# jneem/nnnoiseless

Hardware: AMD Instinct MI355X
Metric: 480-sample frames/sec (whole node) at N concurrent streams (higher is better)
Workload: dtype f32; 1 GPU; configs[2]: 65536 concurrent streams on one GPU, built-in weights.rnn, GRU as batched MFMA GEMM, synthetic 48 kHz sine+noise, 48 frame(s) per stream per step; parity=oracle pinned by the reference's golden pair (built-in model), model=built-in weights.rnn, boundary_format=f32 planar (process_frame's own), streams_per_gpu=65536, streams_total=65536, inputs_ready=True, schedule=stages, lanes=2, parallelism=streams sharded x1, one process per GPU, no data-path collective

## Files before the change

### include/nnn_batch.h

```cpp
#ifndef NNN_BATCH_H
#define NNN_BATCH_H

#include <stddef.h>
#include <stdint.h>

#ifdef __cplusplus
extern "C" {
#endif

typedef struct nnn_batch nnn_batch;
#ifndef RNNOISE_H
typedef struct RNNModel RNNModel;
#endif

#define NNN_FRAME_SIZE 480

RNNModel *nnn_model_from_bytes(const uint8_t *bytes, size_t len);
RNNModel *nnn_model_default(void);
long nnn_convert_rnnoise_text(const char *text, size_t len, uint8_t *out, size_t cap);
RNNModel *nnn_model_from_rnnoise_text(const char *text, size_t len);
void nnn_model_free(RNNModel *m);
RNNModel *nnn_model_clone(const RNNModel *m);
void nnn_model_shape(const RNNModel *m, int32_t shape[12]);

nnn_batch *nnn_batch_create(const RNNModel *model, int n_streams, int device);
nnn_batch *nnn_batch_create_grouped(const RNNModel *const *models, const int *group_streams, int n_groups, int device);
typedef struct nnn_batch_opts {
    int max_group_frames;
    int reserved[7];
} nnn_batch_opts;
nnn_batch *nnn_batch_create_opts(const RNNModel *const *models, const int *group_streams, int n_groups, int device,
                                 const nnn_batch_opts *opts);
int nnn_batch_max_group_frames(const nnn_batch *b);
size_t nnn_batch_device_bytes(const nnn_batch *b);
void nnn_batch_destroy(nnn_batch *b);
int nnn_batch_num_streams(const nnn_batch *b);
int nnn_batch_reset(nnn_batch *b);

nnn_batch *nnn_batch_clone(nnn_batch *b);
size_t nnn_batch_state_bytes(const nnn_batch *b);
int nnn_batch_save_state(nnn_batch *b, void *host_dst, size_t dst_bytes);
int nnn_batch_load_state(nnn_batch *b, const void *host_src, size_t src_bytes);

#define NNN_STREAM_STATE_BYTES 11232
#define NNN_STREAM_STATE_VERSION 1
#define NNN_STREAM_STATE_MAGIC 0x3153534Eu
#define NNN_STREAM_STATE_OFF_MAGIC 0
#define NNN_STREAM_STATE_OFF_VERSION 4
#define NNN_STREAM_STATE_OFF_SIZE 8
#define NNN_STREAM_STATE_OFF_GRU_SIZES 12
#define NNN_STREAM_STATE_OFF_MEM_ID 24
#define NNN_STREAM_STATE_OFF_LAST_PERIOD 28
#define NNN_STREAM_STATE_OFF_LAST_GAIN 32
#define NNN_STREAM_STATE_OFF_MEM_HP_X 36
#define NNN_STREAM_STATE_OFF_INPUT_MEM 64
#define NNN_STREAM_STATE_OFF_SYNTHESIS_MEM 6976
#define NNN_STREAM_STATE_OFF_CEPSTRAL_MEM 8896
#define NNN_STREAM_STATE_OFF_LASTG 9600
#define NNN_STREAM_STATE_OFF_VAD_GRU 9696
#define NNN_STREAM_STATE_OFF_NOISE_GRU 10208
#define NNN_STREAM_STATE_OFF_DENOISE_GRU 10720
int nnn_batch_reset_streams(nnn_batch *b, const int *streams, int n);
int nnn_batch_export_streams(nnn_batch *b, const int *streams, int n, void *host_dst, size_t dst_bytes);
int nnn_batch_import_streams(nnn_batch *b, const int *streams, int n, const void *host_src, size_t src_bytes);
int nnn_batch_export_streams_device(nnn_batch *b, const int *streams, int n, void *d_dst, void *hip_stream);
int nnn_batch_import_streams_device(nnn_batch *b, const int *streams, int n, const void *d_src, void *hip_stream);

int nnn_batch_hold_streams(nnn_batch *b, const int *streams, int n);
int nnn_batch_resume_streams(nnn_batch *b, const int *streams, int n);
int nnn_batch_num_held(const nnn_batch *b);
int nnn_batch_held_mask(const nnn_batch *b, uint8_t *held, size_t n);

int nnn_batch_set_gain_floor(nnn_batch *b, const int *streams, int n, const float *floors, int bands);
int nnn_batch_get_gain_floor(nnn_batch *b, const int *streams, int n, float *floors );
int nnn_batch_num_floored(const nnn_batch *b);

enum nnn_link_mode { NNN_LINK_OFF = 0, NNN_LINK_MAX = 1, NNN_LINK_MIN = 2 };
int nnn_batch_set_channel_link(nnn_batch *b, int channels, int mode);
int nnn_batch_get_channel_link(const nnn_batch *b, int *channels, int *mode);

int nnn_batch_process_device(nnn_batch *b, const float *d_in, float *d_out, float *d_vad, int n_frames,
                             size_t stream_stride, size_t frame_stride, void *hip_stream);
int nnn_batch_process_host(nnn_batch *b, const float *in, float *out, float *vad, int n_frames,
                           size_t stream_stride, size_t frame_stride);
void *nnn_host_alloc(size_t bytes);
void nnn_host_free(void *p);

enum nnn_pcm_format { NNN_PCM_F32 = 0, NNN_PCM_I16 = 1, NNN_PCM_F32_UNIT = 2 };
typedef struct nnn_pcm_layout {
    int format;
    int channels;
    int discard_first;
    int reserved;
    size_t group_stride;
    size_t frame_stride;
} nnn_pcm_layout;
int nnn_batch_process_pcm_device(nnn_batch *b, const void *d_in, void *d_out, float *d_vad, int n_frames,
                                 const nnn_pcm_layout *layout, void *hip_stream);
int nnn_batch_process_pcm_host(nnn_batch *b, const void *in, void *out, float *vad, int n_frames,
                               const nnn_pcm_layout *layout);
int nnn_batch_analyze_device(nnn_batch *b, const void *d_in, float *d_features, int32_t *d_silence, int n_frames,
                             const nnn_pcm_layout *layout, void *hip_stream);
int nnn_batch_synthesize_device(nnn_batch *b, const float *d_gains, const float *d_vad, void *d_out, int n_frames,
                                const nnn_pcm_layout *layout, void *hip_stream);
int nnn_batch_analyze_host(nnn_batch *b, const void *in, float *features, int32_t *silence, int n_frames, const nnn_pcm_layout *layout);
int nnn_batch_synthesize_host(nnn_batch *b, const float *gains, const float *vad, void *out, int n_frames, const nnn_pcm_layout *layout);
int nnn_batch_pending_frames(const nnn_batch *b);
int nnn_batch_vad_device(nnn_batch *b, const void *d_in, float *d_vad, int n_frames, const nnn_pcm_layout *layout, void *hip_stream);
int nnn_batch_vad_host(nnn_batch *b, const void *in, float *vad, int n_frames, const nnn_pcm_layout *layout);
int nnn_batch_network_device(nnn_batch *b, const float *d_features, const int32_t *d_silence, float *d_gains, float *d_vad, int n_frames,
                             void *hip_stream);
int nnn_batch_network_host(nnn_batch *b, const float *features, const int32_t *silence, float *gains, float *vad, int n_frames);
int nnn_batch_synchronize(nnn_batch *b);
int nnn_batch_fault(const nnn_batch *b);
int nnn_batch_debug_withhold_flag(nnn_batch *b, int frames_ahead);
int nnn_batch_debug_schedule(nnn_batch *b, int n_frames, int32_t *out, size_t cap);
int nnn_batch_debug_host_plan(nnn_batch *b, int n_frames, const nnn_pcm_layout *layout, int has_vad, int64_t out[8]);

enum nnn_tap {
    NNN_TAP_FILTERED = 0,
    NNN_TAP_XLP,
    NNN_TAP_AC,
    NNN_TAP_LPC2,
    NNN_TAP_XCORR1,
    NNN_TAP_BEST1,
    NNN_TAP_XCORR2C,
    NNN_TAP_PITCH_SEARCH,
    NNN_TAP_PITCH,
    NNN_TAP_PITCH_GAIN,
    NNN_TAP_X,
    NNN_TAP_P,
    NNN_TAP_EX, NNN_TAP_EP, NNN_TAP_EXP,
    NNN_TAP_FEATURES,
    NNN_TAP_SILENCE,
    NNN_TAP_G_RAW,
    NNN_TAP_G,
    NNN_TAP_VAD,
    NNN_TAP_BRANCH,
    NNN_TAP_COUNT
};
int nnn_tap_info(int tap, int *len, int *is_int);
int nnn_batch_set_taps(nnn_batch *b, int on);
int nnn_batch_read_tap(nnn_batch *b, int tap, void *host_dst, size_t dst_bytes);

#define NNN_FRAME_LOG_WORDS 24
int nnn_batch_set_frame_log(nnn_batch *b, void *d_log, size_t frames);

int nnn_batch_set_profiling(nnn_batch *b, int on);
int nnn_batch_num_kernels(void);
const char *nnn_batch_kernel_name(int k);
int nnn_batch_read_kernel_times(nnn_batch *b, double *total_ms, int64_t *launches, int n);

int nnn_batch_read_stamps(nnn_batch *b, long long *dst64);

int nnn_batch_set_graph(nnn_batch *b, int on);
int nnn_batch_set_pipeline(nnn_batch *b, int on);
int nnn_batch_set_inputs_ready(nnn_batch *b, int on);
int nnn_batch_set_back_end(nnn_batch *b, int mode);
int nnn_batch_set_schedule(nnn_batch *b, int mode, int lanes);

int nnn_debug_activations(int device, int act, const float *x, float *y, int n);

int nnn_device_local_cpulist(int device, char *buf, size_t cap);

const char *nnn_last_error(void);

#ifdef __cplusplus
}
#endif
#endif
```

### nnnoiseless_amd/__init__.py

```python
import ctypes as C
import os

import numpy as np


from . import _ffi
from .build import LIB_PATH, build_library

FRAME_SIZE = 480
FREQ_SIZE = 481
NB_BANDS = 22
NB_FEATURES = 42
from ._ffi import STREAM_STATE_BYTES, STREAM_STATE_VERSION, stream_state_field

_lib = None


def attenuation_limit_db(db):
    return 10.0 ** (-float(db) / 20.0)


def library():
    global _lib
    if _lib is None:
        import os
        import sys
        t = sys.modules.get("torch")
        if t is not None:
            try:
                if t.cuda.is_available():
                    t.cuda.init()
            except Exception:
                pass
        _lib = _ffi.Library(os.environ.get("NNN_LIBRARY", LIB_PATH))
    return _lib


class _Pinned:

    def __init__(self, lib, nbytes):
        self._lib, self.nbytes = lib, int(nbytes)
        self.ptr = lib.L.nnn_host_alloc(self.nbytes)
        if not self.ptr:
            raise MemoryError("nnnoiseless_amd: " + lib.error())

    def __del__(self):
        if getattr(self, "ptr", None):
            self._lib.L.nnn_host_free(self.ptr)
            self.ptr = None


def pinned_empty(shape, dtype=np.float32, lib=None):
    lib = lib or library()
    dt = np.dtype(dtype)
    n = int(np.prod(shape))
    own = _Pinned(lib, max(1, n * dt.itemsize))
    buf = (C.c_char * own.nbytes).from_address(own.ptr)
    buf._owner = own
    return np.frombuffer(buf, dtype=dt, count=n).reshape(shape)


class RnnModel:

    def __init__(self, handle, lib):
        self._h, self._lib = handle, lib

    @classmethod
    def from_bytes(cls, data, lib=None):
        lib = lib or library()
        data = bytes(data)
        h = lib.L.nnn_model_from_bytes(data, len(data))
        return cls(h, lib) if h else None

    from_static_bytes = from_bytes

    @classmethod
    def from_rnnoise_text(cls, text, lib=None):
        lib = lib or library()
        data = text.encode() if isinstance(text, str) else bytes(text)
        h = lib.L.nnn_model_from_rnnoise_text(data, len(data))
        return cls(h, lib) if h else None

    @classmethod
    def default(cls, lib=None):
        lib = lib or library()
        return cls(lib.L.nnn_model_default(), lib)

    def clone(self):
        h = self._lib.L.nnn_model_clone(self._h)
        if not h:
            raise RuntimeError(self._lib.error())
        return RnnModel(h, self._lib)

    __copy__ = clone

    def shape(self):
        s = (C.c_int32 * 12)()
        self._lib.L.nnn_model_shape(self._h, s)
        return list(s)

    def __del__(self):
        if getattr(self, "_h", None):
            self._lib.L.nnn_model_free(self._h)
            self._h = None


class BatchDenoiser:

    def __init__(self, n_streams, model=None, device=0, lib=None, groups=None, taps=False, max_group_frames=None, _handle=None):
        self._lib = lib or library()
        self._model = model
        self.n_streams = int(n_streams)
        self.frames_done = 0
        if _handle is not None:
            self._h = _handle
            return
        if max_group_frames is not None and int(max_group_frames) < 1:
            raise ValueError("max_group_frames must be at least 1")
        if groups or max_group_frames is not None:
            groups_ = groups or [(model, self.n_streams)]
            if sum(n for _, n in groups_) != self.n_streams:
                raise ValueError("group sizes must add up to n_streams")
            if groups:
                self._model = [m for m, _ in groups_]
            hs = (C.c_void_p * len(groups_))(*[m._h if m is not None else None for m, _ in groups_])
            ns = (C.c_int * len(groups_))(*[int(n) for _, n in groups_])
            if max_group_frames is not None:
                opts = _ffi.BatchOpts(max_group_frames=int(max_group_frames))
                self._h = self._lib.L.nnn_batch_create_opts(hs, ns, len(groups_), device, C.byref(opts))
            else:
                self._h = self._lib.L.nnn_batch_create_grouped(hs, ns, len(groups_), device)
        else:
            self._h = self._lib.L.nnn_batch_create(model._h if model is not None else None, self.n_streams, device)
        if not self._h:
            raise RuntimeError("nnnoiseless_amd: " + self._lib.error())
        if taps:
            self.set_taps(True)

    def device_bytes(self):
        return int(self._lib.L.nnn_batch_device_bytes(self._h))

    def max_group_frames(self):
        return int(self._lib.L.nnn_batch_max_group_frames(self._h))

    def clone(self):
        h = self._lib.L.nnn_batch_clone(self._h)
        if not h:
            raise RuntimeError("nnnoiseless_amd: " + self._lib.error())
        c = BatchDenoiser(self.n_streams, model=self._model, lib=self._lib, _handle=h)
        c.frames_done = self.frames_done
        return c

    def save_state(self):
        buf = np.empty(self._lib.L.nnn_batch_state_bytes(self._h), np.uint8)
        self._lib.check(self._lib.L.nnn_batch_save_state(self._h, _ffi.ptr(buf), buf.nbytes))
        return buf.tobytes()

    def load_state(self, data):
        buf = np.frombuffer(data, np.uint8)
        self._lib.check(self._lib.L.nnn_batch_load_state(self._h, _ffi.ptr(buf), buf.nbytes))

    def reset_streams(self, idx):
        a, p = _ffi.stream_list(idx)
        self._lib.check(self._lib.L.nnn_batch_reset_streams(self._h, p, a.size))

    def export_streams(self, idx):
        a, p = _ffi.stream_list(idx)
        out = np.zeros((a.size, STREAM_STATE_BYTES), np.uint8)
        self._lib.check(self._lib.L.nnn_batch_export_streams(self._h, p, a.size, _ffi.ptr(out), out.nbytes))
        return out

    def import_streams(self, idx, records):
        a, p = _ffi.stream_list(idx)
        r = _ffi.stream_records(records, a.size)
        self._lib.check(self._lib.L.nnn_batch_import_streams(self._h, p, a.size, _ffi.ptr(r), r.nbytes))

    def hold_streams(self, idx):
        a, p = _ffi.stream_list(idx)
        self._lib.check(self._lib.L.nnn_batch_hold_streams(self._h, p, a.size))

    def resume_streams(self, idx):
        a, p = _ffi.stream_list(idx)
        self._lib.check(self._lib.L.nnn_batch_resume_streams(self._h, p, a.size))

    def held(self):
        m = np.zeros(self.n_streams, np.uint8)
        self._lib.check(self._lib.L.nnn_batch_held_mask(self._h, _ffi.ptr(m), m.size))
        return m.astype(bool)

    def num_held(self):
        return int(self._lib.L.nnn_batch_num_held(self._h))

    def set_gain_floor(self, idx, floors):
        a, p = _ffi.stream_list(idx)
        f, bands = _ffi.gain_floors(floors, a.size)
        self._lib.check(self._lib.L.nnn_batch_set_gain_floor(self._h, p, a.size, f.ctypes.data_as(C.POINTER(C.c_float)), bands))

    def gain_floor(self, idx=None):
        a, p = _ffi.stream_list(range(self.n_streams) if idx is None else idx)
        out = np.zeros((a.size, NB_BANDS), np.float32)
        self._lib.check(self._lib.L.nnn_batch_get_gain_floor(self._h, p, a.size, out.ctypes.data_as(C.POINTER(C.c_float))))
        return out

    def num_floored(self):
        return int(self._lib.L.nnn_batch_num_floored(self._h))

    def set_channel_link(self, channels, mode="max"):
        self._lib.check(self._lib.L.nnn_batch_set_channel_link(self._h, int(channels), _ffi.link_mode(mode)))

    def channel_link(self):
        ch, md = C.c_int32(0), C.c_int32(0)
        self._lib.check(self._lib.L.nnn_batch_get_channel_link(self._h, C.byref(ch), C.byref(md)))
        return ch.value, _ffi.link_mode_name(md.value)

    def export_streams_device(self, idx, d_dst, hip_stream=0):
        a, p = _ffi.stream_list(idx)
        self._lib.check(self._lib.L.nnn_batch_export_streams_device(self._h, p, a.size, d_dst, hip_stream))

    def import_streams_device(self, idx, d_src, hip_stream=0):
        a, p = _ffi.stream_list(idx)
        self._lib.check(self._lib.L.nnn_batch_import_streams_device(self._h, p, a.size, d_src, hip_stream))

    def set_taps(self, on):
        self._lib.check(self._lib.L.nnn_batch_set_taps(self._h, int(on)))

    def set_schedule(self, mode, lanes=0):
        self._lib.check(self._lib.L.nnn_batch_set_schedule(self._h, {"seq": 0, "lanes": 1, "stages": 2}[mode], int(lanes)))

    def process(self, x, out=None, vad=None):
        x = _ffi.as_f32(x)
        if x.ndim != 3 or x.shape[0] != self.n_streams or x.shape[2] != FRAME_SIZE:
            raise ValueError(f"process needs x of shape [{self.n_streams}, n_frames, {FRAME_SIZE}], got {x.shape}")
        S, T, F = x.shape
        out = np.empty_like(x) if out is None else out
        vad = np.empty((T, S), np.float32) if vad is None else vad
        if not (isinstance(out, np.ndarray) and out.shape == x.shape and out.dtype == np.float32 and out.flags.c_contiguous and out.flags.writeable):
            raise ValueError("process: `out` must be a writable C-contiguous float32 array of x's shape")
        if not (isinstance(vad, np.ndarray) and vad.shape == (T, S) and vad.dtype == np.float32 and vad.flags.c_contiguous and vad.flags.writeable):
            raise ValueError("process: `vad` must be a writable C-contiguous float32 array of shape [n_frames, n_streams]")
        self._lib.check(self._lib.L.nnn_batch_process_host(self._h, _ffi.ptr(x), _ffi.ptr(out), _ffi.ptr(vad), T,
                                                           T * FRAME_SIZE, FRAME_SIZE))
        self.frames_done += T
        return out, vad

    def process_pcm(self, x, fmt, channels=1, discard_first=False, out=None, vad=None):
        x = np.ascontiguousarray(x, dtype=_ffi.PCM_DTYPE[fmt])
        if x.ndim != 3 or x.shape[2] != channels or x.shape[0] * channels != self.n_streams or x.shape[1] % FRAME_SIZE:
            raise ValueError(f"process_pcm needs x of shape [n_streams / channels, n_frames * {FRAME_SIZE}, channels], got {x.shape}")
        G, N, Cc = x.shape
        T = N // FRAME_SIZE
        out = np.zeros_like(x) if out is None else out
        vad = np.empty((T, self.n_streams), np.float32) if vad is None else vad
        if not (isinstance(out, np.ndarray) and out.shape == x.shape and out.dtype == x.dtype and out.flags.c_contiguous and out.flags.writeable):
            raise ValueError("process_pcm: `out` must be a writable C-contiguous array of x's shape and dtype")
        if not (isinstance(vad, np.ndarray) and vad.shape == (T, self.n_streams) and vad.dtype == np.float32 and vad.flags.c_contiguous and vad.flags.writeable):
            raise ValueError("process_pcm: `vad` must be a writable C-contiguous float32 array of shape [n_frames, n_streams]")
        L = _ffi.PcmLayout(fmt, channels, int(bool(discard_first)), 0, N * channels, FRAME_SIZE * channels)
        fresh = self.frames_done == 0
        self._lib.check(self._lib.L.nnn_batch_process_pcm_host(self._h, _ffi.ptr(x), _ffi.ptr(out), _ffi.ptr(vad), T, C.byref(L)))
        self.frames_done += T
        n_out = T - 1 if (discard_first and fresh) else T
        return out[:, :n_out * FRAME_SIZE], vad

    def process_device(self, d_in, d_out, d_vad, n_frames, stream_stride, frame_stride, hip_stream=0):
        self._lib.check(self._lib.L.nnn_batch_process_device(self._h, d_in, d_out, d_vad, n_frames, stream_stride,
                                                             frame_stride, hip_stream))
        self.frames_done += n_frames

    def process_pcm_device(self, d_in, d_out, d_vad, n_frames, fmt, channels, group_stride, frame_stride, discard_first=False,
                           hip_stream=0):
        L = _ffi.PcmLayout(fmt, channels, int(bool(discard_first)), 0, group_stride, frame_stride)
        self._lib.check(self._lib.L.nnn_batch_process_pcm_device(self._h, d_in, d_out, d_vad, n_frames, C.byref(L), hip_stream))
        self.frames_done += n_frames

    def _pcm_shape(self, what, x, fmt, channels):
        if fmt is None:
            x = _ffi.as_f32(x)
            if x.ndim != 3 or x.shape[0] != self.n_streams or x.shape[2] != FRAME_SIZE:
                raise ValueError(f"{what} needs audio of shape [{self.n_streams}, n_frames, {FRAME_SIZE}], got {x.shape}")
            return x, _ffi.PCM_F32, 1, x.shape[1], x.shape[1] * FRAME_SIZE
        x = np.ascontiguousarray(x, dtype=_ffi.PCM_DTYPE[fmt])
        if x.ndim != 3 or x.shape[2] != channels or x.shape[0] * channels != self.n_streams or x.shape[1] % FRAME_SIZE:
            raise ValueError(f"{what} needs audio of shape [n_streams / channels, n_frames * {FRAME_SIZE}, channels], got {x.shape}")
        return x, fmt, channels, x.shape[1] // FRAME_SIZE, x.shape[1] * channels

    def analyze(self, x, fmt=None, channels=1, features=None, silence=None):
        x, fmt, channels, T, gstride = self._pcm_shape("analyze", x, fmt, channels)
        S = self.n_streams
        features = np.zeros((T, S, NB_FEATURES), np.float32) if features is None else features
        silence = np.zeros((T, S), np.int32) if silence is None else silence
        for a, shp, dt, name in ((features, (T, S, NB_FEATURES), np.float32, "features"), (silence, (T, S), np.int32, "silence")):
            if not (isinstance(a, np.ndarray) and a.shape == shp and a.dtype == dt and a.flags.c_contiguous and a.flags.writeable):
                raise ValueError(f"analyze: `{name}` must be a writable C-contiguous {np.dtype(dt).name} array of shape {list(shp)}")
        L = _ffi.PcmLayout(fmt, channels, 0, 0, gstride, FRAME_SIZE * channels)
        self._lib.check(self._lib.L.nnn_batch_analyze_host(self._h, _ffi.ptr(x), _ffi.ptr(features), _ffi.ptr(silence), T, C.byref(L)))
        return features, silence

    def synthesize(self, gains, vad=None, fmt=None, channels=1, discard_first=False, out=None):
        gains = _ffi.as_f32(gains)
        S = self.n_streams
        if gains.ndim != 3 or gains.shape[1:] != (S, NB_BANDS):
            raise ValueError(f"synthesize needs gains of shape [n_frames, {S}, {NB_BANDS}], got {gains.shape}")
        T = gains.shape[0]
        if vad is not None:
            vad = _ffi.as_f32(vad)
            if vad.shape != (T, S):
                raise ValueError(f"synthesize: `vad` must have shape [{T}, {S}], got {vad.shape}")
        if fmt is None:
            fmt_, channels, shape, dt = _ffi.PCM_F32, 1, (S, T, FRAME_SIZE), np.float32
        else:
            if channels < 1 or S % channels:
                raise ValueError("n_streams must be a multiple of channels")
            fmt_, shape, dt = fmt, (S // channels, T * FRAME_SIZE, channels), _ffi.PCM_DTYPE[fmt]
        out = np.zeros(shape, dt) if out is None else out
        if not (isinstance(out, np.ndarray) and out.shape == shape and out.dtype == dt and out.flags.c_contiguous and out.flags.writeable):
            raise ValueError(f"synthesize: `out` must be a writable C-contiguous {np.dtype(dt).name} array of shape {list(shape)}")
        L = _ffi.PcmLayout(fmt_, channels, int(bool(discard_first)), 0, T * FRAME_SIZE * channels, FRAME_SIZE * channels)
        fresh = self.frames_done == 0
        self._lib.check(self._lib.L.nnn_batch_synthesize_host(self._h, _ffi.ptr(gains), _ffi.ptr(vad), _ffi.ptr(out), T, C.byref(L)))
        self.frames_done += T
        if fmt is None:
            return out
        return out[:, :(T - 1 if (discard_first and fresh) else T) * FRAME_SIZE]

    def analyze_device(self, d_in, d_features, d_silence, n_frames, fmt, channels, group_stride, frame_stride, hip_stream=0):
        L = _ffi.PcmLayout(fmt, channels, 0, 0, group_stride, frame_stride)
        self._lib.check(self._lib.L.nnn_batch_analyze_device(self._h, d_in, d_features, d_silence, n_frames, C.byref(L), hip_stream))

    def synthesize_device(self, d_gains, d_vad, d_out, n_frames, fmt, channels, group_stride, frame_stride, discard_first=False, hip_stream=0):
        L = _ffi.PcmLayout(fmt, channels, int(bool(discard_first)), 0, group_stride, frame_stride)
        self._lib.check(self._lib.L.nnn_batch_synthesize_device(self._h, d_gains, d_vad, d_out, n_frames, C.byref(L), hip_stream))
        self.frames_done += n_frames

    def pending_frames(self):
        return int(self._lib.L.nnn_batch_pending_frames(self._h))

    def vad(self, x, fmt=None, channels=1, vad=None):
        x, fmt, channels, T, gstride = self._pcm_shape("vad", x, fmt, channels)
        S = self.n_streams
        vad = np.zeros((T, S), np.float32) if vad is None else vad
        if not (isinstance(vad, np.ndarray) and vad.shape == (T, S) and vad.dtype == np.float32 and vad.flags.c_contiguous and vad.flags.writeable):
            raise ValueError(f"vad: `vad` must be a writable C-contiguous float32 array of shape [{T}, {S}]")
        L = _ffi.PcmLayout(fmt, channels, 0, 0, gstride, FRAME_SIZE * channels)
        self._lib.check(self._lib.L.nnn_batch_vad_host(self._h, _ffi.ptr(x), _ffi.ptr(vad), T, C.byref(L)))
        self.frames_done += T
        return vad

    def vad_device(self, d_in, d_vad, n_frames, fmt, channels, group_stride, frame_stride, hip_stream=0):
        L = _ffi.PcmLayout(fmt, channels, 0, 0, group_stride, frame_stride)
        self._lib.check(self._lib.L.nnn_batch_vad_device(self._h, d_in, d_vad, n_frames, C.byref(L), hip_stream))
        self.frames_done += n_frames

    def network(self, features, silence=None, gains=None, vad=None):
        features = _ffi.as_f32(features)
        S = self.n_streams
        if features.ndim != 3 or features.shape[0] < 1 or features.shape[1:] != (S, NB_FEATURES):
            raise ValueError(f"network needs features of shape [n_frames >= 1, {S}, {NB_FEATURES}], got {features.shape}")
        T = features.shape[0]
        if silence is not None:
            silence = np.ascontiguousarray(silence, dtype=np.int32)
            if silence.shape != (T, S):
                raise ValueError(f"network: `silence` must have shape [{T}, {S}], got {silence.shape}")
        gains = np.zeros((T, S, NB_BANDS), np.float32) if gains is None else gains
        vad = np.zeros((T, S), np.float32) if vad is None else vad
        for a, shp, name in ((gains, (T, S, NB_BANDS), "gains"), (vad, (T, S), "vad")):
            if not (isinstance(a, np.ndarray) and a.shape == shp and a.dtype == np.float32 and a.flags.c_contiguous and a.flags.writeable):
                raise ValueError(f"network: `{name}` must be a writable C-contiguous float32 array of shape {list(shp)}")
        self._lib.check(self._lib.L.nnn_batch_network_host(self._h, _ffi.ptr(features), _ffi.ptr(silence), _ffi.ptr(gains), _ffi.ptr(vad), T))
        return gains, vad

    def network_device(self, d_features, d_silence, d_gains, d_vad, n_frames, hip_stream=0):
        self._lib.check(self._lib.L.nnn_batch_network_device(self._h, d_features, d_silence, d_gains, d_vad, n_frames, hip_stream))

    def synchronize(self):
        self._lib.check(self._lib.L.nnn_batch_synchronize(self._h))

    def reset(self):
        self._lib.check(self._lib.L.nnn_batch_reset(self._h))
        self.frames_done = 0

    def tap(self, name):
        t = _ffi.TAPS.index(name)
        ln, isint = C.c_int(), C.c_int()
        self._lib.check(self._lib.L.nnn_tap_info(t, C.byref(ln), C.byref(isint)))
        a = np.empty((self.n_streams, ln.value), np.int32 if isint.value else np.float32)
        self._lib.check(self._lib.L.nnn_batch_read_tap(self._h, t, _ffi.ptr(a), a.nbytes))
        return a

    def set_profiling(self, on):
        self._lib.check(self._lib.L.nnn_batch_set_profiling(self._h, int(on)))

    def set_graph(self, on):
        self._lib.check(self._lib.L.nnn_batch_set_graph(self._h, int(on)))

    def set_back_end(self, mode):
        self._lib.check(self._lib.L.nnn_batch_set_back_end(self._h, int(mode)))

    def set_pipeline(self, on):
        self._lib.check(self._lib.L.nnn_batch_set_pipeline(self._h, int(on)))

    def set_inputs_ready(self, on):
        self._lib.check(self._lib.L.nnn_batch_set_inputs_ready(self._h, int(on)))

    def set_frame_log(self, d_log, frames):
        self._lib.check(self._lib.L.nnn_batch_set_frame_log(self._h, d_log, int(frames)))

    def fault(self):
        fn = getattr(self._lib.L, "nnn_batch_fault", None)
        return bool(fn(self._h)) if fn else False

    def kernel_times(self):
        n = self._lib.L.nnn_batch_num_kernels()
        ms = (C.c_double * n)()
        cnt = (C.c_int64 * n)()
        self._lib.check(self._lib.L.nnn_batch_read_kernel_times(self._h, ms, cnt, n))
        return {self._lib.L.nnn_batch_kernel_name(k).decode(): (ms[k], cnt[k]) for k in range(n)}

    def close(self):
        if getattr(self, "_h", None):
            self._lib.L.nnn_batch_destroy(self._h)
            self._h = None

    __del__ = close


class DenoiseState:

    FRAME_SIZE = FRAME_SIZE

    def __init__(self, model=None, device=0, lib=None, _batch=None):
        self._b = _batch if _batch is not None else BatchDenoiser(1, model, device, lib, max_group_frames=1)

    def clone(self):
        return DenoiseState(_batch=self._b.clone())

    def export_state(self):
        return self._b.export_streams([0])[0]

    @classmethod
    def from_state(cls, record, model=None, device=0, lib=None):
        st = cls(model, device=device, lib=lib)
        st._b.import_streams([0], np.asarray(record, np.uint8).reshape(1, -1))
        return st

    @classmethod
    def new(cls, **kw):
        return cls(None, **kw)

    @classmethod
    def from_model(cls, model, **kw):
        return cls(model, **kw)

    with_model = from_model

    def process_frame(self, output, input):
        input = _ffi.as_f32(input)
        if input.shape != (FRAME_SIZE,) or output.shape != (FRAME_SIZE,):
            raise ValueError("process_frame needs slices of length DenoiseState.FRAME_SIZE")
        out, vad = self._b.process(input.reshape(1, 1, FRAME_SIZE))
        output[:] = out[0, 0]
        return float(vad[0, 0])


from .node import NodeDenoiser
```

### nnnoiseless_amd/_ffi.py

```python
import ctypes as C
import os

import numpy as np

FRAME_SIZE = 480

TAPS = ["filtered", "xlp", "ac", "lpc2", "xcorr1", "best1", "xcorr2c", "pitch_search", "pitch", "pitch_gain",
        "X", "P", "ex", "ep", "exp", "features", "silence", "g_raw", "g", "vad", "branch"]

BATCH_SYMBOLS = [
    "nnn_model_from_bytes", "nnn_model_default", "nnn_model_free", "nnn_model_clone", "nnn_model_shape",
    "nnn_convert_rnnoise_text", "nnn_model_from_rnnoise_text",
    "nnn_batch_create", "nnn_batch_create_grouped", "nnn_batch_destroy", "nnn_batch_num_streams", "nnn_batch_reset",
    "nnn_batch_process_device", "nnn_batch_process_host", "nnn_batch_process_pcm_device", "nnn_batch_process_pcm_host",
    "nnn_batch_synchronize", "nnn_batch_clone", "nnn_batch_state_bytes", "nnn_batch_save_state", "nnn_batch_load_state",
    "nnn_batch_set_taps", "nnn_batch_set_schedule", "nnn_batch_set_inputs_ready", "nnn_debug_activations",
    "nnn_tap_info", "nnn_batch_read_tap", "nnn_batch_set_profiling", "nnn_batch_num_kernels",
    "nnn_batch_kernel_name", "nnn_batch_read_kernel_times", "nnn_batch_set_graph", "nnn_batch_set_pipeline", "nnn_batch_read_stamps",
    "nnn_host_alloc", "nnn_host_free", "nnn_last_error", "nnn_batch_fault", "nnn_batch_debug_withhold_flag", "nnn_batch_debug_schedule", "nnn_batch_debug_host_plan", "nnn_batch_set_frame_log",
    "nnn_batch_create_opts", "nnn_batch_max_group_frames", "nnn_batch_device_bytes", "nnn_batch_set_back_end", "nnn_device_local_cpulist",
    "nnn_batch_reset_streams", "nnn_batch_export_streams", "nnn_batch_import_streams", "nnn_batch_export_streams_device",
    "nnn_batch_import_streams_device", "nnn_batch_hold_streams", "nnn_batch_resume_streams", "nnn_batch_num_held", "nnn_batch_held_mask",
    "nnn_batch_analyze_device", "nnn_batch_synthesize_device", "nnn_batch_analyze_host", "nnn_batch_synthesize_host", "nnn_batch_pending_frames",
    "nnn_batch_vad_device", "nnn_batch_vad_host", "nnn_batch_network_device", "nnn_batch_network_host",
    "nnn_batch_set_gain_floor", "nnn_batch_get_gain_floor", "nnn_batch_num_floored",
    "nnn_batch_set_channel_link", "nnn_batch_get_channel_link",
]
TRAIN_SYMBOLS = [
    "nnn_train_create", "nnn_train_destroy", "nnn_train_reset", "nnn_train_process_device", "nnn_train_process_host",
]
RESAMPLE_SYMBOLS = [
    "nnn_resampler_create", "nnn_resampler_destroy", "nnn_resampler_reset", "nnn_resampler_max_output",
    "nnn_resampler_process_device", "nnn_resampler_process_host",
]
RATE_SYMBOLS = [
    "nnn_rate_create", "nnn_rate_destroy", "nnn_rate_reset", "nnn_rate_reset_streams", "nnn_rate_max_output", "nnn_rate_max_frames",
    "nnn_rate_carried", "nnn_rate_process_device", "nnn_rate_process_host", "nnn_rate_debug_tables",
]
PACK_SYMBOLS = [
    "nnn_pack_create", "nnn_pack_destroy", "nnn_pack_plan", "nnn_pack_run_device", "nnn_pack_run_host", "nnn_pack_last_summary",
    "nnn_pack_debug_kernels",
]
SIM_SYMBOLS = [
    "nnn_sim_create", "nnn_sim_destroy", "nnn_sim_load", "nnn_sim_adopt_device", "nnn_sim_set_params", "nnn_sim_get_params", "nnn_sim_reset",
    "nnn_sim_process_device", "nnn_sim_process_host", "nnn_sim_signals_device", "nnn_sim_signals_host", "nnn_sim_fault", "nnn_sim_debug_kernel",
]
FIT_SYMBOLS = [
    "nnn_fit_create", "nnn_fit_destroy", "nnn_fit_get", "nnn_fit_set", "nnn_fit_get_step", "nnn_fit_set_step", "nnn_fit_get_settings",
    "nnn_fit_set_settings", "nnn_fit_export_rnn", "nnn_fit_forward_device", "nnn_fit_loss_device", "nnn_fit_grad_device", "nnn_fit_step",
    "nnn_fit_losses", "nnn_fit_forward_host", "nnn_fit_loss_host", "nnn_fit_grad_host", "nnn_fit_debug_recurrence",
]
SCORE_SYMBOLS = [
    "nnn_score_create", "nnn_score_destroy", "nnn_score_set_delay", "nnn_score_get_delay", "nnn_score_reset", "nnn_score_accumulate_device",
    "nnn_score_accumulate_host", "nnn_score_totals", "nnn_score_totals_device",
]
SCORE_MAX_DELAY, SCORE_SUMS = 960, 4
GATE_SYMBOLS = [
    "nnn_gate_create", "nnn_gate_destroy", "nnn_gate_set_params", "nnn_gate_get_params", "nnn_gate_reset", "nnn_gate_apply_device",
    "nnn_gate_apply_pcm_device", "nnn_gate_apply_host", "nnn_gate_state_bytes", "nnn_gate_export_streams", "nnn_gate_import_streams",
]
GATE_MAX_LOOKBACK, GATE_MAX_GRACE, GATE_NEVER = 8, 6000, 0x7fffffff
GATE_STATE_BYTES, GATE_STATE_VERSION, GATE_STATE_MAGIC = 48 + 8 * 480 * 4, 1, 0x3147564E
GATE_PARAMS_DTYPE = np.dtype([("threshold", "<f4"), ("grace", "<i4"), ("lookback", "<i4"), ("level", "<f4")])
GATE_STATE_DTYPE = np.dtype([("magic", "<u4"), ("version", "<u4"), ("size", "<u4"), ("threshold", "<f4"), ("grace", "<i4"), ("lookback", "<i4"),
                             ("level", "<f4"), ("since", "<i4"), ("was_open", "<u4"), ("zero", "<u4", 3), ("history", "<f4", (8, 480))])
FIT_PARAMS, FIT_RNN_BYTES, FIT_TILE = 87503, 87521, 4
FIT_SEL_PARAMS, FIT_SEL_GRAD, FIT_SEL_ADAM_M, FIT_SEL_ADAM_V = 0, 1, 2, 3
FIT_TENSORS = {
    "input_dense.W": (0, (42, 24)), "input_dense.b": (1008, (24,)),
    "vad_gru.W": (1032, (24, 72)), "vad_gru.U": (2760, (24, 72)), "vad_gru.b": (4488, (72,)),
    "noise_gru.W": (4560, (90, 144)), "noise_gru.U": (17520, (48, 144)), "noise_gru.b": (24432, (144,)),
    "denoise_gru.W": (24576, (114, 288)), "denoise_gru.U": (57408, (96, 288)), "denoise_gru.b": (85056, (288,)),
    "denoise_output.W": (85344, (96, 22)), "denoise_output.b": (87456, (22,)),
    "vad_output.W": (87478, (24, 1)), "vad_output.b": (87502, (1,)),
}
NODE_SYMBOLS = [
    "nnn_node_create", "nnn_node_destroy", "nnn_node_num_streams", "nnn_node_num_shards", "nnn_node_shard", "nnn_node_batch", "nnn_node_reset",
    "nnn_node_process_host", "nnn_node_process_pcm_host", "nnn_node_process_device", "nnn_node_process_device_streams", "nnn_node_synchronize",
    "nnn_node_fault", "nnn_node_shard_cpus", "nnn_node_reset_streams", "nnn_node_export_streams", "nnn_node_import_streams",
    "nnn_node_hold_streams", "nnn_node_resume_streams", "nnn_node_num_held",
    "nnn_node_set_gain_floor", "nnn_node_get_gain_floor", "nnn_node_num_floored",
    "nnn_node_set_channel_link", "nnn_node_get_channel_link",
]
RNNOISE_SYMBOLS = [
    "rnnoise_get_frame_size", "rnnoise_get_size", "rnnoise_init", "rnnoise_create", "rnnoise_destroy",
    "rnnoise_process_frame", "rnnoise_model_from_file", "rnnoise_model_free",
]


PCM_F32, PCM_I16, PCM_F32_UNIT = 0, 1, 2
PACK_I24, PACK_I32, PACK_F32_WAV = 16, 17, 18
PACK_ELEM_BYTES = {PCM_F32: 4, PCM_I16: 2, PACK_I24: 3, PACK_I32: 4, PACK_F32_WAV: 4}
LINK_OFF, LINK_MAX, LINK_MIN = 0, 1, 2
LINK_MODES = {"off": LINK_OFF, "max": LINK_MAX, "min": LINK_MIN}

STREAM_STATE_BYTES = 11232
STREAM_STATE_VERSION = 1
STREAM_STATE_MAGIC = 0x3153534E
STREAM_STATE_FIELDS = {
    "magic": (0, np.uint32, 1), "version": (4, np.uint32, 1), "size": (8, np.uint32, 1), "gru_sizes": (12, np.int32, 3),
    "mem_id": (24, np.int32, 1), "last_period": (28, np.int32, 1), "last_gain": (32, np.float32, 1), "mem_hp_x": (36, np.float32, 2),
    "input_mem": (64, np.float32, 1728), "synthesis_mem": (6976, np.float32, 480), "cepstral_mem": (8896, np.float32, 176),
    "lastg": (9600, np.float32, 22), "vad_gru": (9696, np.float32, 128), "noise_gru": (10208, np.float32, 128),
    "denoise_gru": (10720, np.float32, 128),
}


def stream_state_field(records, name):
    off, dt, cnt = STREAM_STATE_FIELDS[name]
    r = np.ascontiguousarray(records, dtype=np.uint8)
    a = r[..., off:off + cnt * np.dtype(dt).itemsize].view(dt)
    return a.reshape(r.shape[:-1] + (cnt,))
PCM_DTYPE = {PCM_F32: np.float32, PCM_I16: np.int16, PCM_F32_UNIT: np.float32}


class PcmLayout(C.Structure):
    _fields_ = [("format", C.c_int), ("channels", C.c_int), ("discard_first", C.c_int), ("reserved", C.c_int),
                ("group_stride", C.c_size_t), ("frame_stride", C.c_size_t)]


class PackFile(C.Structure):
    _fields_ = [("in_off", C.c_uint64), ("n_frames_samples", C.c_uint64), ("out_off", C.c_uint64), ("vad_off", C.c_uint64)]


class SimParams(C.Structure):
    _fields_ = [("signal_gain", C.c_float), ("noise_gain", C.c_float), ("sig_a", C.c_float * 2), ("sig_b", C.c_float * 2),
                ("noise_a", C.c_float * 2), ("noise_b", C.c_float * 2), ("band_lp", C.c_int32)]


SIM_PARAMS_DTYPE = np.dtype([("signal_gain", "<f4"), ("noise_gain", "<f4"), ("sig_a", "<f4", 2), ("sig_b", "<f4", 2),
                             ("noise_a", "<f4", 2), ("noise_b", "<f4", 2), ("band_lp", "<i4")])


class FitSettings(C.Structure):
    _fields_ = [("lr", C.c_float), ("beta1", C.c_float), ("beta2", C.c_float), ("epsilon", C.c_float), ("reg", C.c_float), ("clip", C.c_float)]


class FitRows(C.Structure):
    _fields_ = [("rows", C.c_void_p), ("frame_stride", C.c_size_t), ("seq_stride", C.c_size_t), ("w", C.c_void_p),
                ("w_frame_stride", C.c_size_t), ("w_seq_stride", C.c_size_t), ("n_seq", C.c_int), ("window", C.c_int)]


class BatchOpts(C.Structure):
    _fields_ = [("max_group_frames", C.c_int), ("reserved", C.c_int * 7)]


class Library:

    def __init__(self, path):
        if not os.path.exists(path):
            raise RuntimeError(
                f"nnnoiseless_amd: HIP library not found at {path}. Build it with "
                "`python -c 'import __graft_entry__ as g; g.build()'` (needs hipcc); there is no CPU fallback.")
        self.path = path
        L = self.L = C.CDLL(path)
        vp, sz, i32 = C.c_void_p, C.c_size_t, C.c_int
        L.nnn_model_from_bytes.restype = vp
        L.nnn_model_from_bytes.argtypes = [C.c_char_p, sz]
        L.nnn_model_default.restype = vp
        L.nnn_model_free.argtypes = [vp]
        L.nnn_model_clone.restype = vp
        L.nnn_model_clone.argtypes = [vp]
        L.nnn_model_shape.argtypes = [vp, C.POINTER(C.c_int32)]
        L.nnn_convert_rnnoise_text.restype = C.c_long
        L.nnn_convert_rnnoise_text.argtypes = [C.c_char_p, sz, vp, sz]
        L.nnn_model_from_rnnoise_text.restype = vp
        L.nnn_model_from_rnnoise_text.argtypes = [C.c_char_p, sz]
        L.nnn_batch_create_grouped.restype = vp
        L.nnn_batch_create_grouped.argtypes = [C.POINTER(vp), C.POINTER(i32), i32, i32]
        L.nnn_batch_create.restype = vp
        L.nnn_batch_create.argtypes = [vp, i32, i32]
        L.nnn_batch_destroy.argtypes = [vp]
        L.nnn_batch_num_streams.argtypes = [vp]
        L.nnn_batch_reset.argtypes = [vp]
        L.nnn_batch_process_device.argtypes = [vp, vp, vp, vp, i32, sz, sz, vp]
        L.nnn_batch_process_host.argtypes = [vp, vp, vp, vp, i32, sz, sz]
        L.nnn_batch_process_pcm_device.argtypes = [vp, vp, vp, vp, i32, C.POINTER(PcmLayout), vp]
        L.nnn_batch_process_pcm_host.argtypes = [vp, vp, vp, vp, i32, C.POINTER(PcmLayout)]
        L.nnn_batch_synchronize.argtypes = [vp]
        L.nnn_host_alloc.restype = vp
        L.nnn_host_alloc.argtypes = [sz]
        L.nnn_host_free.restype = None
        L.nnn_host_free.argtypes = [vp]
        L.nnn_tap_info.argtypes = [i32, C.POINTER(i32), C.POINTER(i32)]
        L.nnn_batch_read_tap.argtypes = [vp, i32, vp, sz]
        L.nnn_batch_set_profiling.argtypes = [vp, i32]
        L.nnn_batch_kernel_name.restype = C.c_char_p
        L.nnn_batch_kernel_name.argtypes = [i32]
        L.nnn_batch_read_kernel_times.argtypes = [vp, C.POINTER(C.c_double), C.POINTER(C.c_int64), i32]
        L.nnn_batch_set_graph.argtypes = [vp, i32]
        L.nnn_batch_clone.restype = vp
        L.nnn_batch_clone.argtypes = [vp]
        L.nnn_batch_state_bytes.restype = sz
        L.nnn_batch_state_bytes.argtypes = [vp]
        L.nnn_batch_save_state.argtypes = [vp, vp, sz]
        L.nnn_batch_load_state.argtypes = [vp, vp, sz]
        L.nnn_batch_set_taps.argtypes = [vp, i32]
        L.nnn_batch_set_schedule.argtypes = [vp, i32, i32]
        L.nnn_debug_activations.argtypes = [i32, i32, vp, vp, i32]
        L.nnn_batch_set_pipeline.argtypes = [vp, i32]
        L.nnn_batch_set_inputs_ready.argtypes = [vp, i32]
        for name, at in (("nnn_batch_set_frame_log", [vp, vp, sz]), ("nnn_batch_fault", [vp]), ("nnn_batch_debug_withhold_flag", [vp, i32]),
                         ("nnn_batch_debug_schedule", [vp, i32, C.POINTER(C.c_int32), sz]),
                         ("nnn_batch_debug_host_plan", [vp, i32, C.POINTER(PcmLayout), i32, C.POINTER(C.c_int64)]),
                         ("nnn_batch_create_opts", [C.POINTER(vp), C.POINTER(i32), i32, i32, C.POINTER(BatchOpts)]),
                         ("nnn_batch_max_group_frames", [vp]), ("nnn_batch_device_bytes", [vp]), ("nnn_batch_set_back_end", [vp, i32])):
            if hasattr(L, name):
                getattr(L, name).argtypes = at
        if hasattr(L, "nnn_batch_create_opts"):
            L.nnn_batch_create_opts.restype = vp
            L.nnn_batch_device_bytes.restype = sz
        if hasattr(L, "nnn_batch_reset_streams"):
            ip = C.POINTER(i32)
            L.nnn_batch_reset_streams.argtypes = [vp, ip, i32]
            L.nnn_batch_export_streams.argtypes = [vp, ip, i32, vp, sz]
            L.nnn_batch_import_streams.argtypes = [vp, ip, i32, vp, sz]
            L.nnn_batch_export_streams_device.argtypes = [vp, ip, i32, vp, vp]
            L.nnn_batch_import_streams_device.argtypes = [vp, ip, i32, vp, vp]
        if hasattr(L, "nnn_batch_hold_streams"):
            ip = C.POINTER(i32)
            L.nnn_batch_hold_streams.argtypes = [vp, ip, i32]
            L.nnn_batch_resume_streams.argtypes = [vp, ip, i32]
            L.nnn_batch_num_held.argtypes = [vp]
            L.nnn_batch_held_mask.argtypes = [vp, vp, sz]
        if hasattr(L, "nnn_batch_analyze_device"):
            lp = C.POINTER(PcmLayout)
            L.nnn_batch_analyze_device.argtypes = [vp, vp, vp, vp, i32, lp, vp]
            L.nnn_batch_synthesize_device.argtypes = [vp, vp, vp, vp, i32, lp, vp]
            L.nnn_batch_analyze_host.argtypes = [vp, vp, vp, vp, i32, lp]
            L.nnn_batch_synthesize_host.argtypes = [vp, vp, vp, vp, i32, lp]
            L.nnn_batch_pending_frames.argtypes = [vp]
        if hasattr(L, "nnn_batch_vad_device"):
            L.nnn_batch_vad_device.argtypes = [vp, vp, vp, i32, C.POINTER(PcmLayout), vp]
            L.nnn_batch_vad_host.argtypes = [vp, vp, vp, i32, C.POINTER(PcmLayout)]
        if hasattr(L, "nnn_batch_network_device"):
            L.nnn_batch_network_device.argtypes = [vp, vp, vp, vp, vp, i32, vp]
            L.nnn_batch_network_host.argtypes = [vp, vp, vp, vp, vp, i32]
        if hasattr(L, "nnn_batch_set_gain_floor"):
            ip, fp = C.POINTER(i32), C.POINTER(C.c_float)
            L.nnn_batch_set_gain_floor.argtypes = [vp, ip, i32, fp, i32]
            L.nnn_batch_get_gain_floor.argtypes = [vp, ip, i32, fp]
            L.nnn_batch_num_floored.argtypes = [vp]
        for name in ("nnn_batch_set_channel_link", "nnn_node_set_channel_link"):
            if hasattr(L, name):
                getattr(L, name).argtypes = [vp, i32, i32]
                getattr(L, name.replace("_set_", "_get_")).argtypes = [vp, C.POINTER(i32), C.POINTER(i32)]
        if hasattr(L, "nnn_node_set_gain_floor"):
            ip, fp = C.POINTER(i32), C.POINTER(C.c_float)
            L.nnn_node_set_gain_floor.argtypes = [vp, ip, i32, fp, i32]
            L.nnn_node_get_gain_floor.argtypes = [vp, ip, i32, fp]
            L.nnn_node_num_floored.argtypes = [vp]
        if hasattr(L, "nnn_node_hold_streams"):
            ip = C.POINTER(i32)
            L.nnn_node_hold_streams.argtypes = [vp, ip, i32]
            L.nnn_node_resume_streams.argtypes = [vp, ip, i32]
            L.nnn_node_num_held.argtypes = [vp]
        if hasattr(L, "nnn_node_reset_streams"):
            ip = C.POINTER(i32)
            L.nnn_node_reset_streams.argtypes = [vp, ip, i32]
            L.nnn_node_export_streams.argtypes = [vp, ip, i32, vp, sz]
            L.nnn_node_import_streams.argtypes = [vp, ip, i32, vp, sz]
        if hasattr(L, "nnn_node_create"):
            L.nnn_node_create.restype = vp
            L.nnn_node_create.argtypes = [vp, i32, C.POINTER(i32), i32, C.POINTER(BatchOpts)]
            L.nnn_node_destroy.argtypes = [vp]
            L.nnn_node_num_streams.argtypes = [vp]
            L.nnn_node_num_shards.argtypes = [vp]
            L.nnn_node_shard.argtypes = [vp, i32, C.POINTER(i32), C.POINTER(i32), C.POINTER(i32)]
            L.nnn_node_batch.restype = vp
            L.nnn_node_batch.argtypes = [vp, i32]
            L.nnn_node_reset.argtypes = [vp]
            L.nnn_node_process_host.argtypes = [vp, vp, vp, vp, i32, sz, sz]
            L.nnn_node_process_pcm_host.argtypes = [vp, vp, vp, vp, i32, C.POINTER(PcmLayout)]
            L.nnn_node_process_device.argtypes = [vp, C.POINTER(vp), C.POINTER(vp), C.POINTER(vp), i32, sz, sz]
            L.nnn_node_process_device_streams.argtypes = [vp, C.POINTER(vp), C.POINTER(vp), C.POINTER(vp), C.POINTER(vp), i32, i32, sz, sz]
            L.nnn_node_shard_cpus.restype = C.c_char_p
            L.nnn_node_shard_cpus.argtypes = [vp, i32]
            L.nnn_node_synchronize.argtypes = [vp]
            L.nnn_node_fault.argtypes = [vp]
        L.nnn_train_create.restype = vp
        L.nnn_train_create.argtypes = [i32, i32]
        L.nnn_train_destroy.argtypes = [vp]
        L.nnn_train_reset.argtypes = [vp]
        L.nnn_train_process_device.argtypes = [vp, vp, vp, vp, vp, vp, vp, i32, sz, sz, vp]
        L.nnn_train_process_host.argtypes = [vp, vp, vp, vp, vp, vp, vp, i32]
        L.nnn_resampler_create.restype = vp
        L.nnn_resampler_create.argtypes = [i32, C.c_double, i32]
        L.nnn_resampler_destroy.argtypes = [vp]
        L.nnn_resampler_reset.argtypes = [vp]
        L.nnn_resampler_max_output.restype = C.c_long
        L.nnn_resampler_max_output.argtypes = [vp, C.c_long]
        L.nnn_resampler_process_device.argtypes = [vp, vp, C.c_long, sz, vp, C.c_long, sz, C.POINTER(C.c_long), vp]
        L.nnn_resampler_process_host.argtypes = [vp, vp, C.c_long, vp, C.c_long, C.POINTER(C.c_long)]
        if hasattr(L, "nnn_rate_create"):
            lp = C.POINTER(C.c_long)
            L.nnn_rate_create.restype = vp
            L.nnn_rate_create.argtypes = [vp, C.c_double, C.c_long]
            L.nnn_rate_destroy.restype = None
            L.nnn_rate_destroy.argtypes = [vp]
            L.nnn_rate_reset.argtypes = [vp]
            L.nnn_rate_reset_streams.argtypes = [vp, C.POINTER(i32), i32]
            L.nnn_rate_max_output.restype = C.c_long
            L.nnn_rate_max_output.argtypes = [vp, C.c_long]
            L.nnn_rate_max_frames.argtypes = [vp, C.c_long]
            L.nnn_rate_carried.restype = C.c_long
            L.nnn_rate_carried.argtypes = [vp]
            L.nnn_rate_process_device.argtypes = [vp, vp, C.c_long, sz, vp, C.c_long, sz, lp, vp, i32, C.POINTER(i32), i32, vp]
            L.nnn_rate_process_host.argtypes = [vp, vp, C.c_long, vp, C.c_long, lp, vp, i32, C.POINTER(i32), i32]
            L.nnn_rate_debug_tables.argtypes = [vp, lp, C.POINTER(C.c_double)]
        if hasattr(L, "nnn_pack_create"):
            u64, fp_ = C.c_uint64, C.POINTER(PackFile)
            L.nnn_pack_create.restype = vp
            L.nnn_pack_create.argtypes = [vp, i32, i32]
            L.nnn_pack_destroy.restype = None
            L.nnn_pack_destroy.argtypes = [vp]
            L.nnn_pack_plan.argtypes = [i32, i32, C.POINTER(u64), i32, C.POINTER(C.c_int32), C.POINTER(C.c_int32), C.POINTER(C.c_int64)]
            L.nnn_pack_run_device.argtypes = [vp, vp, u64, i32, vp, u64, i32, vp, u64, fp_, i32, vp]
            L.nnn_pack_run_host.argtypes = [vp, vp, u64, i32, vp, u64, i32, vp, u64, fp_, i32]
            L.nnn_pack_last_summary.argtypes = [vp, C.POINTER(C.c_int64)]
            L.nnn_pack_debug_kernels.argtypes = [vp, i32, vp, i32, vp, i32, i32, i32, vp]
        if hasattr(L, "nnn_sim_create"):
            u64, ip = C.c_uint64, C.POINTER(i32)
            L.nnn_sim_create.restype = vp
            L.nnn_sim_create.argtypes = [vp]
            L.nnn_sim_destroy.restype = None
            L.nnn_sim_destroy.argtypes = [vp]
            L.nnn_sim_load.argtypes = [vp, i32, vp, u64]
            L.nnn_sim_adopt_device.argtypes = [vp, i32, vp, u64]
            L.nnn_sim_set_params.argtypes = [vp, ip, i32, vp]
            L.nnn_sim_get_params.argtypes = [vp, ip, i32, vp]
            L.nnn_sim_reset.argtypes = [vp]
            L.nnn_sim_process_device.argtypes = [vp, vp, vp, vp, i32, vp]
            L.nnn_sim_process_host.argtypes = [vp, vp, vp, vp, i32]
            L.nnn_sim_signals_device.argtypes = [vp, vp, vp, vp, vp, vp, vp, vp, i32, sz, sz, vp]
            L.nnn_sim_signals_host.argtypes = [vp, vp, vp, vp, vp, vp, vp, vp, i32]
            L.nnn_sim_fault.argtypes = [vp]
            L.nnn_sim_debug_kernel.argtypes = [vp, vp, vp, i32, i32, vp]
        if hasattr(L, "nnn_fit_create"):
            rp, fp = C.POINTER(FitRows), C.POINTER(C.c_float)
            L.nnn_fit_create.restype = vp
            L.nnn_fit_create.argtypes = [C.c_char_p, sz, i32, i32, i32]
            L.nnn_fit_destroy.restype = None
            L.nnn_fit_destroy.argtypes = [vp]
            L.nnn_fit_get.argtypes = [vp, i32, vp]
            L.nnn_fit_set.argtypes = [vp, i32, vp]
            L.nnn_fit_get_step.argtypes = [vp, C.POINTER(C.c_int64)]
            L.nnn_fit_set_step.argtypes = [vp, C.c_int64]
            L.nnn_fit_get_settings.argtypes = [vp, C.POINTER(FitSettings)]
            L.nnn_fit_set_settings.argtypes = [vp, C.POINTER(FitSettings)]
            L.nnn_fit_export_rnn.argtypes = [vp, vp, sz]
            L.nnn_fit_forward_device.argtypes = [vp, rp, vp, vp, vp]
            L.nnn_fit_loss_device.argtypes = [vp, rp, vp]
            L.nnn_fit_grad_device.argtypes = [vp, rp, vp]
            L.nnn_fit_step.argtypes = [vp, vp]
            L.nnn_fit_losses.argtypes = [vp, fp]
            L.nnn_fit_forward_host.argtypes = [vp, vp, i32, i32, vp, vp]
            L.nnn_fit_loss_host.argtypes = [vp, vp, vp, i32, i32]
            L.nnn_fit_grad_host.argtypes = [vp, vp, vp, i32, i32]
            L.nnn_fit_debug_recurrence.argtypes = [vp, i32, i32, i32, i32, i32, vp]
        if hasattr(L, "nnn_score_create"):
            ip = C.POINTER(i32)
            L.nnn_score_create.restype = vp
            L.nnn_score_create.argtypes = [i32, i32, i32]
            L.nnn_score_destroy.restype = None
            L.nnn_score_destroy.argtypes = [vp]
            L.nnn_score_set_delay.argtypes = [vp, ip, i32, vp]
            L.nnn_score_get_delay.argtypes = [vp, ip, i32, vp]
            L.nnn_score_reset.argtypes = [vp, ip, i32]
            L.nnn_score_accumulate_device.argtypes = [vp, vp, vp, vp, vp, i32, sz, sz, vp]
            L.nnn_score_accumulate_host.argtypes = [vp, vp, vp, vp, vp, i32]
            L.nnn_score_totals.argtypes = [vp, vp, vp]
            L.nnn_score_totals_device.argtypes = [vp, vp, vp, vp]
        if hasattr(L, "nnn_gate_create"):
            ip = C.POINTER(i32)
            L.nnn_gate_create.restype = vp
            L.nnn_gate_create.argtypes = [i32, i32, i32]
            L.nnn_gate_destroy.restype = None
            L.nnn_gate_destroy.argtypes = [vp]
            L.nnn_gate_set_params.argtypes = [vp, ip, i32, vp]
            L.nnn_gate_get_params.argtypes = [vp, ip, i32, vp]
            L.nnn_gate_reset.argtypes = [vp, ip, i32]
            L.nnn_gate_apply_device.argtypes = [vp, vp, vp, vp, vp, vp, i32, sz, sz, vp]
            L.nnn_gate_apply_pcm_device.argtypes = [vp, vp, vp, vp, vp, vp, i32, C.POINTER(PcmLayout), vp]
            L.nnn_gate_apply_host.argtypes = [vp, vp, vp, vp, vp, vp, i32]
            L.nnn_gate_state_bytes.restype = sz
            L.nnn_gate_state_bytes.argtypes = [vp]
            L.nnn_gate_export_streams.argtypes = [vp, ip, i32, vp, sz]
            L.nnn_gate_import_streams.argtypes = [vp, ip, i32, vp, sz]
        L.nnn_last_error.restype = C.c_char_p
        L.rnnoise_create.restype = vp
        L.rnnoise_create.argtypes = [vp]
        L.rnnoise_destroy.argtypes = [vp]
        L.rnnoise_process_frame.restype = C.c_float
        L.rnnoise_process_frame.argtypes = [vp, vp, vp]
        L.rnnoise_model_free.argtypes = [vp]

    def error(self):
        return self.L.nnn_last_error().decode()

    def check(self, rc):
        if rc != 0:
            raise RuntimeError("nnnoiseless_amd: " + self.error())


def ptr(a):
    return None if a is None else a.ctypes.data_as(C.c_void_p)


def as_f32(a):
    return np.ascontiguousarray(a, dtype=np.float32)


def stream_list(idx):
    a = np.ascontiguousarray(np.asarray(idx, dtype=np.int64).reshape(-1))
    if a.size and (a.min() < -2**31 or a.max() >= 2**31):
        raise ValueError("stream index out of int32 range")
    a = a.astype(np.int32)
    return a, a.ctypes.data_as(C.POINTER(C.c_int))


def stream_records(records, n):
    r = np.ascontiguousarray(records, dtype=np.uint8)
    if r.size != n * STREAM_STATE_BYTES:
        raise ValueError(f"need {n} records of {STREAM_STATE_BYTES} bytes, got {r.size} bytes")
    return r.reshape(n, STREAM_STATE_BYTES)


def gain_floors(floors, n):
    f = np.asarray(floors, dtype=np.float32)
    if f.ndim == 0:
        f = np.full(n, f, np.float32)
    if f.shape == (n,):
        return np.ascontiguousarray(f), 1
    if f.shape == (n, 22):
        return np.ascontiguousarray(f), 22
    raise ValueError(f"floors must be a scalar, [{n}] or [{n}, 22], got shape {f.shape}")


def link_mode(mode):
    if isinstance(mode, str):
        if mode not in LINK_MODES:
            raise ValueError(f"link mode must be one of {sorted(LINK_MODES)}, got {mode!r}")
        return LINK_MODES[mode]
    return int(mode)


def link_mode_name(mode):
    return {v: k for k, v in LINK_MODES.items()}[int(mode)]
```

### nnnoiseless_amd/csrc/nnn_batch_core.hip

```cpp
#pragma once

static thread_local std::string g_err;
static std::recursive_mutex g_rt_mu;
constexpr int MARK_DEVICES = 64;
static std::atomic<uint64_t> g_call_mark[MARK_DEVICES];
static std::atomic<uint64_t> g_next_batch_id{1};
#define NNN_RT_LOCK std::lock_guard<std::recursive_mutex> rt_lock_(g_rt_mu)
extern "C" const char *nnn_last_error(void) { return g_err.c_str(); }
extern "C" int nnn_device_local_cpulist(int device, char *buf, size_t cap)
{
    if (!buf || cap < 2) return 1;
    buf[0] = 0;
    char id[64] = {0};
    if (hipDeviceGetPCIBusId(id, (int)sizeof(id), device) != hipSuccess || !id[0]) return 1;
    for (char *p = id; *p; p++)
        if (*p >= 'A' && *p <= 'F') *p = (char)(*p - 'A' + 'a');
    char path[160];
    snprintf(path, sizeof(path), "/sys/bus/pci/devices/%s/local_cpulist", id);
    FILE *f = fopen(path, "r");
    if (!f) return 1;
    const bool ok = fgets(buf, (int)cap, f) != nullptr;
    fclose(f);
    if (!ok) { buf[0] = 0; return 1; }
    for (char *p = buf; *p; p++)
        if (*p == '\n' || *p == '\r') *p = 0;
    return buf[0] ? 0 : 1;
}
static int fail(const char *fmt, ...)
{
    char buf[512];
    va_list ap;
    va_start(ap, fmt);
    vsnprintf(buf, sizeof(buf), fmt, ap);
    va_end(ap);
    g_err = buf;
    return 1;
}
int nnn_set_error(const char *msg) { return fail("%s", msg); }
#define HIPCHK(expr)                                                                       \
    do {                                                                                   \
        hipError_t e_ = (expr);                                                            \
        if (e_ != hipSuccess) return fail("%s failed: %s", #expr, hipGetErrorString(e_));  \
    } while (0)


static const char *knob(const char *name) { return getenv(name); }
#ifdef NNN_DEV_KNOBS
static const char *dev_knob(const char *name) { return getenv(name); }
#else
static const char *dev_knob(const char *) { return nullptr; }
#endif

enum KernelId { K_HP, K_LPC, K_PITCH, K_FFT_XP, K_RNN, K_SYNTH, K_BACK, K_COUNT };
static const char *kKernelNames[K_COUNT] = {"k_hp", "k_lpc", "k_pitch", "k_fft_xp", "k_rnn", "k_synth", "k_back"};

enum Stage { ST_HP, ST_PITCH, ST_FFT, ST_RNN, ST_SYN, ST_COUNT };
enum SplitStage { ST_FEAT = ST_COUNT, ST_GAINS, ST_FFT_FEAT, ST_VAD };
struct SplitIo {
    float *features = nullptr;
    int *silence = nullptr;
    const float *gains = nullptr;
    const float *vad = nullptr;
};
constexpr int NSTREAMS = 5;
constexpr int EVR = 16;
enum SchedMode { SCHED_SEQ = 0, SCHED_LANES = 1, SCHED_STAGES = 2 };
constexpr int AUTO_BIG = 16384;
constexpr long long HANDOFF_TICKS = 10000ll * 100000ll;

struct Paths {
    int sched = SCHED_LANES;
    bool sched_auto = true;
    int n_lanes = 1;
    int host_chunk = -1;
    int wf_min_g = 0;
    int rnn_rows = 0;
    int hp_split = -1;
    int lpc_head = -1;
    int pitch_chain = 1;
    int hp_tpb = 0;
    int x_rides = -1;
    int lpc_wide = -1;
    int lpc_fc = 0;
    int back_mode = -1;
    bool use_pipeline = true;
    bool inputs_ready = false;
};
static Paths read_paths()
{
    Paths p;
    if (const char *e = knob("NNN_HOST_CHUNK")) p.host_chunk = atoi(e);
    if (const char *e = knob("NNN_RNN_WF_MIN_G")) p.wf_min_g = atoi(e);
    if (const char *e = knob("NNN_HP_SPLIT")) p.hp_split = atoi(e);
    if (const char *e = dev_knob("NNN_HP_TPB")) p.hp_tpb = atoi(e);
    if (const char *e = knob("NNN_LPC_HEAD")) p.lpc_head = atoi(e);
    if (const char *e = dev_knob("NNN_X_RIDES")) p.x_rides = atoi(e);
    if (const char *e = knob("NNN_PITCH_CHAIN")) p.pitch_chain = atoi(e);
    if (const char *e = dev_knob("NNN_LPC_WIDE")) p.lpc_wide = atoi(e);
    if (const char *e = dev_knob("NNN_LPC_FC")) p.lpc_fc = atoi(e);
    if (const char *e = knob("NNN_SCHED")) {
        if (!strcmp(e, "seq")) p.sched = SCHED_SEQ;
        else if (!strcmp(e, "lanes")) p.sched = SCHED_LANES;
        else if (!strcmp(e, "stages")) p.sched = SCHED_STAGES;
        p.sched_auto = false;
    }
    if (const char *e = knob("NNN_LANES")) {
        const int v = atoi(e);
        if (v >= 1 && v <= NSTREAMS - 1) p.n_lanes = v;
        p.sched_auto = false;
    }
    if (const char *e = knob("NNN_RNN_ROWS")) {
        const int v = atoi(e);
        if (v == 16 || v == 32) p.rnn_rows = v;
    }
    return p;
}

enum BackEnd { BACK_UNFUSED = 0, BACK_RNN_ALONE = 1, BACK_FUSED = 2 };
enum RnnKernel : uint8_t { RK_BACK, RK_WF_BUILTIN, RK_WF_ANY, RK_PLAIN };
struct GroupPlan {
    int g = 0;
    BackEnd back = BACK_UNFUSED;
    int hp = 0;
    bool held = false;
    bool floor = false;
    bool link = false;
    bool head = false;
    bool lpc_in_pitch = false;
    int lpc_fc = 0;
    bool chain = false;
    bool riders = false;
    uint8_t *rnn = nullptr;
};

enum MemKind : uint8_t { MEM_DEVICE, MEM_PINNED, MEM_MAPPED };
template <class T> struct GrowBuf {
    T *p = nullptr;
    size_t cap = 0;
    MemKind kind = MEM_DEVICE;
    int release()
    {
        if (p) HIPCHK(kind == MEM_DEVICE ? hipFree(p) : hipHostFree(p));
        p = nullptr, cap = 0;
        return 0;
    }
    hipError_t alloc(size_t n) { return kind == MEM_DEVICE ? hipMalloc((void **)&p, n) : hipHostMalloc((void **)&p, n, kind == MEM_MAPPED ? hipHostMallocMapped : 0); }
};

struct nnn_batch {
    Buffers b[NSET];
    ModelDims md;
    struct ModelGroup {
        RnnPlan plan;
        const uint4 *wq = nullptr;
        const float *fpar = nullptr;
        size_t rnn_lds = 0;
        bool wf = false;
        bool shape_builtin = false;
        WfPlan wp;
        size_t wf_lds = 0;
        int rows = 32;
        int tile0 = 0, ntiles = 0;
        size_t back_lds = 0, rnn16_lds = 0;
        BkActs acts = {};
        int vad_rows = 0, vad_mb = 0;
        size_t vad_lds = 0;
        int net_rows = 0;
        size_t net_lds = 0;
    };
    Paths paths;
    Paths created;
    GroupPlan plan;
    std::vector<ModelGroup> groups;
    std::vector<RNNModel> models;
    std::vector<int> group_streams;
    int device = 0;
    int S = 0, S_pad = 0, NT = 0;
    uint64_t frame_count = 0;
    int depth = 1;
    int gmax = GROUP;
    int nset = GROUP, nslot = slots_for(GROUP, 1);
    size_t device_bytes = 0;
    uint64_t group_count = 0;
    int last_set = 0;
    std::vector<void *> allocs;
    std::vector<std::pair<void *, size_t>> state_bufs;
    GrowBuf<char> stage;
    GrowBuf<float> stage_vad;
    std::vector<char> stage_host;
    GrowBuf<char> zc_host{nullptr, 0, MEM_MAPPED};
    char *zc_dev = nullptr;
    hipStream_t copy_in = nullptr, copy_out = nullptr;
    std::vector<hipEvent_t> ev_up, ev_run;
    GrowBuf<StepParams> sp_tab;
    hipStream_t stream = nullptr;
    hipStream_t pool[NSTREAMS] = {};
    hipEvent_t ev[2][ST_COUNT][EVR] = {};
    hipEvent_t ev_done[2] = {};
    bool have_done[2] = {false, false};
    bool prev_pipe = false;
    hipStream_t prev_st = nullptr;
    uint64_t prev_frame0 = 0;
    int prev_par = 0;
    std::vector<int> prev_first;
    volatile int *fault_host = nullptr;
    unsigned tickets = 0;
    unsigned *frame_log = nullptr;
    size_t frame_log_left = 0;
    uint64_t id = 0, other_seen_us = 0;
    bool beside_others = false;
    bool host_call = false;
    hipEvent_t ev_in = nullptr;
    hipEvent_t ev_last = nullptr;
    hipStream_t last_stream = nullptr;
    bool have_last = false;
    uint64_t call_count = 0;
    bool taps_alloc = false;
    bool profiling = false;
    std::vector<hipEvent_t> evp;
    std::vector<int> evp_kernel;
    double k_ms[K_COUNT] = {0};
    int64_t k_launches[K_COUNT] = {0};
    int *ss_dims = nullptr;
    int *ss_flag = nullptr;
    volatile int *ss_bad_host = nullptr;
    int *ss_bad_dev = nullptr;
    GrowBuf<int> ss_idx;
    GrowBuf<int> ss_idx_pin{nullptr, 0, MEM_PINNED};
    hipEvent_t ev_ss_idx = nullptr;
    bool ss_idx_busy = false;
    GrowBuf<char> ss_stage;
    unsigned *park = nullptr;
    unsigned long long *live = nullptr;
    std::vector<uint8_t> held;
    int n_held = 0;
    float *gfloor = nullptr;
    std::vector<float> gfloor_host;
    int n_floored = 0;
    GrowBuf<char> fl_stage;
    GrowBuf<char> fl_pin{nullptr, 0, MEM_PINNED};
    hipEvent_t ev_fl = nullptr;
    bool fl_busy = false;
    int link_ch = 1, link_mode = 0;
    int pending = 0, pending_set0 = 0, pending_slot = 0;
    GrowBuf<float> split_stage;
};

static int refuse_pending(const nnn_batch *h, const char *what)
{
    if (!h || !h->pending) return 0;
    return fail("%s refused: %d frames are pending (analysed by nnn_batch_analyze_* and not yet synthesised); "
                "nnn_batch_synthesize_* of the same n_frames comes first (nnn_batch_reset drops them)", what, h->pending);
}

extern "C" int nnn_batch_fault(const nnn_batch *h) { return h && h->fault_host && *h->fault_host ? 1 : 0; }
static int report_fault(const nnn_batch *h)
{
    if (!nnn_batch_fault(h)) return 0;
    return fail("a pitch workgroup gave up waiting for the previous frame's result (frame hand-off flag never set): the state of the "
                "affected streams is invalid from that frame on; nnn_batch_reset or nnn_batch_load_state clears the condition "
                "(NNN_PITCH_CHAIN=0 runs the frames of a group in a loop instead of side by side)");
}

static int quiesce(nnn_batch *h)
{
    HIPCHK(hipSetDevice(h->device));
    if (h->have_last) HIPCHK(hipEventSynchronize(h->ev_last));
    HIPCHK(hipStreamSynchronize(h->stream));
    for (int i = 0; i < NSTREAMS; i++)
        if (h->pool[i]) HIPCHK(hipStreamSynchronize(h->pool[i]));
    return 0;
}

template <class A, class B = char> static int grow(nnn_batch *h, bool drain, GrowBuf<A> &a, size_t a_bytes, size_t cap, GrowBuf<B> *b = nullptr, size_t b_bytes = 0)
{
    NNN_RT_LOCK;
    if (int rc = drain ? quiesce(h) : 0) return rc;
    if (int rc = a.release()) return rc;
    if (int rc = b ? b->release() : 0) return rc;
    HIPCHK(a.alloc(a_bytes));
    if (b) HIPCHK(b->alloc(b_bytes));
    a.cap = cap;
    if (b) b->cap = cap;
    return 0;
}

template <class T> static hipError_t dalloc(nnn_batch *h, T **p, size_t count, bool is_state)
{
    size_t bytes = count * sizeof(T);
    hipError_t e = hipMalloc((void **)p, bytes ? bytes : 4);
    if (e != hipSuccess) return e;
    h->allocs.push_back(*p);
    h->device_bytes += bytes ? bytes : 4;
    e = hipMemset(*p, 0, bytes);
    if (is_state) h->state_bufs.push_back({(void *)*p, bytes});
    return e;
}
template <class T> static hipError_t upload(nnn_batch *h, const T **p, const std::vector<T> &v)
{
    T *d = nullptr;
    hipError_t e = dalloc(h, &d, v.size(), false);
    if (e != hipSuccess) return e;
    *p = d;
    return hipMemcpy(d, v.data(), v.size() * sizeof(T), hipMemcpyHostToDevice);
}

extern "C" void *nnn_host_alloc(size_t bytes)
{
    void *p = nullptr;
    if (hipHostMalloc(&p, bytes ? bytes : 1, hipHostMallocDefault) != hipSuccess) {
        fail("nnn_host_alloc: %zu bytes of page-locked memory not available", bytes);
        return nullptr;
    }
    return p;
}
extern "C" void nnn_host_free(void *p)
{
    if (p) hipHostFree(p);
}
```

### nnnoiseless_amd/csrc/nnn_batch_create.hip

```cpp
#pragma once

static void make_tables(std::vector<float> &window, std::vector<float> &dct, std::vector<float2> &tw,
                        std::vector<float> &tansig, std::vector<float> &bin_frac, std::vector<int> &bin_band, float &wnorm)
{
    const double pi = 3.14159265358979323846;
    window.resize(WINDOW);
    for (int i = 0; i < FRAME; i++) {
        double s = sin(0.5 * pi * ((double)i + 0.5) / (double)FRAME);
        float w = (float)sin(0.5 * pi * s * s);
        window[i] = w;
        window[WINDOW - 1 - i] = w;
    }
    float acc = 0.0f;
    for (int i = 0; i < WINDOW; i++) acc += window[i] * window[i];
    wnorm = 1.0f / acc;
    dct.resize(NB * NB);
    for (int i = 0; i < NB; i++)
        for (int j = 0; j < NB; j++) {
            float v = (float)cos(((double)i + 0.5) * (double)j * pi / (double)NB);
            if (j == 0) v *= sqrtf(0.5f);
            dct[i * NB + j] = v;
        }
    tw.resize(WINDOW);
    for (int k = 0; k < WINDOW; k++) {
        tw[k].x = (float)cos(-2.0 * pi * k / (double)WINDOW);
        tw[k].y = (float)sin(-2.0 * pi * k / (double)WINDOW);
    }
    tansig.resize(201);
    for (int i = 0; i <= 200; i++) tansig[i] = (float)(floor(tanh(0.04 * (double)i) * 1e6 + 0.5) / 1e6);
    tansig[70] = 0.992631f;
    tansig[170] = 0.999997f;
    tansig[190] = 1.000000f;
    const int *E = kEbandHost;
    bin_frac.assign(400, 0.0f);
    bin_band.assign(400, 0);
    for (int i = 0; i < NB - 1; i++) {
        int band_size = (E[i + 1] - E[i]) << 2;
        for (int j = 0; j < band_size; j++) {
            bin_frac[(E[i] << 2) + j] = (float)j / (float)band_size;
            bin_band[(E[i] << 2) + j] = i;
        }
    }
}

extern "C" void nnn_batch_destroy(nnn_batch *h)
{
    if (!h) return;
    NNN_RT_LOCK;
    hipSetDevice(h->device);
    hipDeviceSynchronize();
    for (int p = 0; p < 2; p++) {
        for (int s = 0; s < ST_COUNT; s++)
            for (int i = 0; i < EVR; i++)
                if (h->ev[p][s][i]) hipEventDestroy(h->ev[p][s][i]);
        if (h->ev_done[p]) hipEventDestroy(h->ev_done[p]);
    }
    if (h->ev_in) hipEventDestroy(h->ev_in);
    if (h->ev_last) hipEventDestroy(h->ev_last);
    for (hipEvent_t e : h->evp) hipEventDestroy(e);
    for (void *p : h->allocs) hipFree(p);
    if (h->fault_host) hipHostFree((void *)h->fault_host);
    h->sp_tab.release();
    for (hipEvent_t e : h->ev_up) hipEventDestroy(e);
    for (hipEvent_t e : h->ev_run) hipEventDestroy(e);
    if (h->copy_in) hipStreamDestroy(h->copy_in);
    if (h->copy_out) hipStreamDestroy(h->copy_out);
    h->stage.release();
    h->stage_vad.release();
    h->split_stage.release();
    h->zc_host.release();
    if (h->ss_dims) hipFree(h->ss_dims);
    if (h->ss_flag) hipFree(h->ss_flag);
    if (h->ss_bad_host) hipHostFree((void *)h->ss_bad_host);
    h->ss_idx.release();
    h->ss_idx_pin.release();
    if (h->ev_ss_idx) hipEventDestroy(h->ev_ss_idx);
    h->ss_stage.release();
    h->fl_stage.release();
    h->fl_pin.release();
    if (h->ev_fl) hipEventDestroy(h->ev_fl);
    delete[] h->plan.rnn;
    for (int i = 0; i < NSTREAMS; i++)
        if (h->pool[i]) hipStreamDestroy(h->pool[i]);
    if (h->stream) hipStreamDestroy(h->stream);
    delete h;
}

constexpr size_t kLdsMax = 160 * 1024;
constexpr int RNN_SMALL_BATCH_BLOCKS = 128;

static nnn_batch::ModelGroup plan_model_group(const RnnPlan &pl, int ntiles, const Paths &paths)
{
    nnn_batch::ModelGroup G;
    G.plan = pl;
    G.ntiles = ntiles;
    G.rows = 0;
    for (int rows = 32; rows >= 16 && !G.rows; rows /= 2)
        if ((size_t)rnn_lds(G.plan, rows).total <= kLdsMax) G.rows = rows;
    if (!G.rows) return G;
    while (G.rows > 16 && G.ntiles * (TILE / G.rows) < RNN_SMALL_BATCH_BLOCKS) G.rows /= 2;
    if (paths.rnn_rows && (size_t)rnn_lds(G.plan, paths.rnn_rows).total <= kLdsMax) G.rows = paths.rnn_rows;
    G.rnn_lds = (size_t)rnn_lds(G.plan, G.rows).total;
    for (int half = 2; half >= 1 && !G.vad_rows; half--)
        for (int rows = TILE; rows >= 16 && !G.vad_rows; rows /= 2)
            if ((size_t)vad_lds(vad_plan_view(G.plan), rows).total <= kLdsMax / half && vad_gru_mb(G.plan, rows)) G.vad_rows = rows;
    if (G.vad_rows) {
        G.vad_mb = vad_gru_mb(G.plan, G.vad_rows);
        G.vad_lds = (size_t)vad_lds(vad_plan_view(G.plan), G.vad_rows).total;
    }
    G.net_rows = paths.rnn_rows && (size_t)net_lds(G.plan, paths.rnn_rows).total <= kLdsMax ? paths.rnn_rows : 16;
    G.net_lds = (size_t)net_lds(G.plan, G.net_rows).total;
    G.wp = wf_plan_of(G.plan);
    G.wf_lds = (size_t)wf_lds(G.wp).total;
    {
        constexpr RnnPlan cls = BkShapeBuiltin::plan();
        const bool shape_ok = pl.dense.n == cls.dense.n && pl.vad.n == cls.vad.n && pl.noise.n == cls.noise.n && pl.dn.n == cls.dn.n;
        G.shape_builtin = shape_ok;
        const size_t fb = (size_t)back_lds(G.plan, true).total, rb = (size_t)back_lds(G.plan, false).total;
        G.back_lds = shape_ok && fb <= kLdsMax ? fb : 0;
        G.rnn16_lds = shape_ok && rb <= kLdsMax ? rb : 0;
        G.acts = BkActs{G.plan.dense.act, G.plan.vad.act, G.plan.noise.act, G.plan.dn.act, G.plan.out.act, G.plan.act_vo};
    }
    G.wf = !paths.rnn_rows && G.plan.dense.nb <= 2 && G.plan.vad.nb <= 2 && G.plan.noise.nb <= 3 && G.plan.dn.nb <= 6 && G.plan.vad.rec.ksteps <= WF_KS_REC &&
           G.plan.noise.rec.ksteps <= WF_KS_REC && G.plan.dn.rec.ksteps <= WF_KS_REC && G.wf_lds <= kLdsMax;
    return G;
}

static int create_check_args(nnn_batch *h, const int *group_streams, int n_groups, int device, int gmax, int &n_streams)
{
    h->gmax = gmax < 1 ? 1 : (gmax > GROUP ? GROUP : gmax);
    n_streams = 0;
    for (int g = 0; g < n_groups; g++) {
        if (group_streams[g] <= 0) return fail("group %d: stream count must be positive", g);
        if (g + 1 < n_groups && group_streams[g] % TILE) return fail("group %d: every group but the last must be a multiple of %d streams", g, TILE);
        n_streams += group_streams[g];
    }
    int ndev = 0;
    HIPCHK(hipGetDeviceCount(&ndev));
    if (device < 0 || device >= ndev) return fail("no HIP device %d (found %d)", device, ndev);
    if (device >= MARK_DEVICES) return fail("device %d: the library keeps per-device call marks for devices 0 .. %d only", device, MARK_DEVICES - 1);
    HIPCHK(hipSetDevice(device));
    h->device = device;
    return 0;
}
static int create_streams_and_events(nnn_batch *h)
{
    HIPCHK(hipStreamCreateWithFlags(&h->stream, hipStreamNonBlocking));
    HIPCHK(hipEventCreateWithFlags(&h->ev_in, hipEventDisableTiming));
    HIPCHK(hipEventCreateWithFlags(&h->ev_last, hipEventDisableTiming));
    for (int p = 0; p < 2; p++) {
        for (int s = 0; s < ST_COUNT; s++)
            for (int i = 0; i < EVR; i++) HIPCHK(hipEventCreateWithFlags(&h->ev[p][s][i], hipEventDisableTiming));
        HIPCHK(hipEventCreateWithFlags(&h->ev_done[p], hipEventDisableTiming));
    }
    return 0;
}
static int create_model_groups(nnn_batch *h, const RNNModel *const *models, const int *group_streams, int n_groups, const Paths &paths,
                               std::vector<std::vector<uint16_t>> &wqs, std::vector<std::vector<float>> &fpars)
{
    wqs.resize(n_groups);
    fpars.resize(n_groups);
    h->groups.resize(n_groups);
    h->group_streams.assign(group_streams, group_streams + n_groups);
    memset(&h->md, 0, sizeof(h->md));
    for (int g = 0, tile0 = 0; g < n_groups; g++) {
        const RNNModel *model = models ? models[g] : nullptr;
        RNNModel *own = nullptr;
        if (!model) {
            size_t len;
            const uint8_t *w = nnn_builtin_weights(&len);
            own = nnn_model_parse(w, len);
            if (!own) return fail("built-in weights failed to parse");
            model = own;
        }
        h->models.push_back(*model);
        RnnPlan plan;
        ModelDims md;
        nnn_model_pack(*model, wqs[g], fpars[g], plan, md);
        delete own;
        nnn_batch::ModelGroup &G = h->groups[g];
        G = plan_model_group(plan, (group_streams[g] + TILE - 1) / TILE, paths);
        if (!G.rows) return fail("model too large for the RNN kernel's LDS operand matrices");
        G.tile0 = tile0;
        tile0 += G.ntiles;
        h->md.nd = md.nd > h->md.nd ? md.nd : h->md.nd;
        h->md.nv = md.nv > h->md.nv ? md.nv : h->md.nv;
        h->md.nn = md.nn > h->md.nn ? md.nn : h->md.nn;
        h->md.ndn = md.ndn > h->md.ndn ? md.ndn : h->md.ndn;
    }
    h->plan.rnn = new uint8_t[n_groups]();
    return 0;
}
static int create_state_arrays(nnn_batch *h)
{
    const size_t Sp = (size_t)h->S_pad;
    const ModelDims &md = h->md;
    Buffers &b = h->b[0];
    memset(&b, 0, sizeof(b));
    b.S = h->S; b.S_pad = h->S_pad; b.NT = h->NT;
    b.nslot = h->nslot;
    b.gru_v_w = md.nv; b.gru_n_w = md.nn; b.gru_dn_w = md.ndn;
    HIPCHK(dalloc(h, &b.hist, Sp * hist_stride(h->nslot), true));
    HIPCHK(dalloc(h, &b.hp_mem, Sp * 2, true));
    HIPCHK(dalloc(h, &b.hp_last, Sp, true));
    HIPCHK(dalloc(h, &b.dec, Sp * dec_len(h->nslot), true));
    HIPCHK(dalloc(h, &b.xlp0, Sp * h->nslot, true));
    HIPCHK(dalloc(h, &b.lpc_head, (size_t)h->NT * 5 * TILE, false));
    HIPCHK(dalloc(h, &b.lpc, Sp * h->nslot * 10, false));
    HIPCHK(dalloc(h, &b.ceps_mem, Sp * CEPS_MEM * NB, true));
    HIPCHK(dalloc(h, &b.mem_id, Sp, true));
    HIPCHK(dalloc(h, &b.synth_mem, Sp * FRAME, true));
    HIPCHK(dalloc(h, &b.lastg, Sp * NB, true));
    HIPCHK(dalloc(h, &b.last_period, Sp, true));
    HIPCHK(dalloc(h, &b.last_gain, Sp, true));
    HIPCHK(dalloc(h, &b.gru_v, Sp * md.nv, true));
    HIPCHK(dalloc(h, &b.gru_n, Sp * md.nn, true));
    HIPCHK(dalloc(h, &b.gru_dn, Sp * md.ndn, true));
    HIPCHK(dalloc(h, &b.stamps, 64, false));
    {
        void *hp = nullptr, *dp = nullptr;
        HIPCHK(hipHostMalloc(&hp, sizeof(int), hipHostMallocMapped));
        *(volatile int *)hp = 0;
        HIPCHK(hipHostGetDevicePointer(&dp, hp, 0));
        h->fault_host = (volatile int *)hp;
        b.fault = (int *)dp;
    }
    HIPCHK(dalloc(h, &b.ticket, 1, false));
    b.handoff_ticks = HANDOFF_TICKS;
    return grow(h, false, h->sp_tab, 2 * 64 * sizeof(StepParams), 64);
}
static int create_tables(nnn_batch *h, const std::vector<std::vector<uint16_t>> &wqs, const std::vector<std::vector<float>> &fpars)
{
    Buffers &b = h->b[0];
    std::vector<float> window, dct, tansig, bin_frac;
    std::vector<float2> tw;
    std::vector<int> bin_band;
    make_tables(window, dct, tw, tansig, bin_frac, bin_band, b.wnorm);
    HIPCHK(upload(h, &b.window, window));
    {
        std::vector<float> wa(WINDOW), ws(WINDOW);
        for (int i = 0; i < WINDOW; i++) { wa[i] = window[i] * 0.5f; ws[i] = window[i] * 0.5f; }
        HIPCHK(upload(h, &b.window_a, wa));
        HIPCHK(upload(h, &b.window_s, ws));
    }
    HIPCHK(upload(h, &b.dct, dct));
    HIPCHK(upload(h, &b.tw960, tw));
    HIPCHK(upload(h, &b.tansig, tansig));
    HIPCHK(upload(h, &b.bin_frac, bin_frac));
    HIPCHK(upload(h, &b.bin_band, bin_band));
    {
        const int *E = kEbandHost;
        std::vector<int> seg(192, 0);
        int ns = 0;
        for (int i = 0; i < NB - 1; i++) {
            int k = E[i] << 2, end = E[i + 1] << 2;
            const int need = (end - k + 7) / 8;
            if (need > 16) return fail("band interval too long for a row of lanes");
            if ((ns & 15) + need > 16) ns = (ns + 15) & ~15;
            seg[128 + i] = ns;
            while (k < end) {
                int c = end - k < 8 ? end - k : 8;
                if (ns >= 64) return fail("band segmentation overflow");
                seg[ns] = k;
                seg[64 + ns] = c;
                ns++;
                k += c;
            }
            seg[160 + i] = ns - seg[128 + i];
        }
        if (ns > 64) return fail("band segmentation overflow");
        HIPCHK(upload(h, &b.seg, seg));
        std::vector<FftLds> img(1);
        fft_tables_image(img[0], tw.data(), bin_frac.data(), bin_band.data(), seg.data(), dct.data());
        const FftLds *dimg = nullptr;
        HIPCHK(upload(h, &dimg, img));
        b.fft_img = dimg;
    }
    for (size_t g = 0; g < h->groups.size(); g++) {
        const uint16_t *dq = nullptr;
        HIPCHK(upload(h, &dq, wqs[g]));
        h->groups[g].wq = (const uint4 *)dq;
        HIPCHK(upload(h, &h->groups[g].fpar, fpars[g]));
    }
    return 0;
}
#define NNN_ALLOC_ONE(name, len) HIPCHK(dalloc(h, &h->b[0].name, (size_t)h->S_pad * (size_t)(len) * h->nset, false));
#define NNN_ALLOC_SETS(FIELDS)                                                              \
    do {                                                                                    \
        FIELDS(NNN_ALLOC_ONE)                                                               \
        for (int set = 1; set < h->nset; set++) h->b[set] = frame_view(h->b[0], set);       \
    } while (0)
static int create_scratch_sets(nnn_batch *h)
{
    NNN_ALLOC_SETS(NNN_WORK_FIELDS);
    h->state_bufs.push_back({(void *)h->b[0].pflag, (size_t)h->S_pad * h->nset * sizeof(int)});
    return 0;
}
static int raise_lds_limits()
{
    for (const void *k : big_lds_kernels()) HIPCHK(hipFuncSetAttribute(k, hipFuncAttributeMaxDynamicSharedMemorySize, (int)kLdsMax));
    return 0;
}

static int create_impl(nnn_batch *h, const RNNModel *const *models, const int *group_streams, int n_groups, int device, int gmax, const Paths &paths)
{
    int n_streams = 0;
    if (int rc = create_check_args(h, group_streams, n_groups, device, gmax, n_streams)) return rc;
    if (int rc = create_streams_and_events(h)) return rc;
    h->paths = h->created = paths;
    h->depth = (paths.n_lanes >= 2 || paths.sched == SCHED_STAGES || (paths.sched_auto && (n_streams + TILE - 1) / TILE * TILE > AUTO_BIG)) ? DEPTH : 1;
    h->nset = h->depth * h->gmax;
    h->nslot = slots_for(h->gmax, h->depth);
    h->S = n_streams;
    h->S_pad = (n_streams + TILE - 1) / TILE * TILE;
    h->NT = h->S_pad / TILE;
    std::vector<std::vector<uint16_t>> wqs;
    std::vector<std::vector<float>> fpars;
    if (int rc = create_model_groups(h, models, group_streams, n_groups, paths, wqs, fpars)) return rc;
    if (int rc = create_state_arrays(h)) return rc;
    if (int rc = create_tables(h, wqs, fpars)) return rc;
    if (int rc = create_scratch_sets(h)) return rc;
    if (int rc = raise_lds_limits()) return rc;
    HIPCHK(hipDeviceSynchronize());
    h->id = g_next_batch_id.fetch_add(1) & 0xFFFFFu;
    if (!h->id) h->id = g_next_batch_id.fetch_add(1) & 0xFFFFFu;
    return 0;
}

static nnn_batch *create_batch(const RNNModel *const *models, const int *group_streams, int n_groups, int device, int gmax, const Paths &paths)
{
    NNN_RT_LOCK;
    nnn_batch *h = new nnn_batch();
    if (create_impl(h, models, group_streams, n_groups, device, gmax, paths) != 0) {
        std::string keep = g_err;
        nnn_batch_destroy(h);
        g_err = keep;
        return nullptr;
    }
    return h;
}

extern "C" nnn_batch *nnn_batch_create_opts(const RNNModel *const *models, const int *group_streams, int n_groups, int device,
                                             const nnn_batch_opts *opts)
{
    if (n_groups <= 0 || !group_streams) {
        fail("need at least one group of streams");
        return nullptr;
    }
    int gmax = GROUP;
    if (opts) {
        for (int r : opts->reserved)
            if (r != 0) {
                fail("nnn_batch_opts.reserved must be zero");
                return nullptr;
            }
        if (opts->max_group_frames < 0) {
            fail("nnn_batch_opts.max_group_frames must not be negative");
            return nullptr;
        }
        if (opts->max_group_frames > GROUP) {
            fail("nnn_batch_opts.max_group_frames must not exceed %d (the kernels' longest frame group)", GROUP);
            return nullptr;
        }
        if (opts->max_group_frames > 0) gmax = opts->max_group_frames;
    }
    return create_batch(models, group_streams, n_groups, device, gmax, read_paths());
}

extern "C" nnn_batch *nnn_batch_create_grouped(const RNNModel *const *models, const int *group_streams, int n_groups, int device)
{
    return nnn_batch_create_opts(models, group_streams, n_groups, device, nullptr);
}

extern "C" int nnn_batch_max_group_frames(const nnn_batch *h) { return h ? h->gmax : 0; }
extern "C" size_t nnn_batch_device_bytes(const nnn_batch *h) { return h ? h->device_bytes : 0; }

extern "C" nnn_batch *nnn_batch_create(const RNNModel *model, int n_streams, int device)
{
    if (n_streams <= 0) {
        fail("n_streams must be positive");
        return nullptr;
    }
    return nnn_batch_create_grouped(&model, &n_streams, 1, device);
}

extern "C" int nnn_batch_num_streams(const nnn_batch *h) { return h ? h->S : 0; }

extern "C" int nnn_batch_synchronize(nnn_batch *h)
{
    if (!h) return fail("null batch");
    HIPCHK(hipSetDevice(h->device));
    if (h->have_last) HIPCHK(hipEventSynchronize(h->ev_last));
    HIPCHK(hipStreamSynchronize(h->stream));
    if (h->ss_bad_host && *h->ss_bad_host) {
        *h->ss_bad_host = 0;
        return fail("nnn_batch_import_streams_device: a record did not match its target stream (magic, version, size or GRU sizes); "
                    "that import wrote nothing");
    }
    return report_fault(h);
}

extern "C" int nnn_batch_reset(nnn_batch *h)
{
    NNN_RT_LOCK;
    if (!h) return fail("null batch");
    if (int rc = quiesce(h)) return rc;
    for (auto &sb : h->state_bufs) HIPCHK(hipMemset(sb.first, 0, sb.second));
    if (int rc = hold_release_all(h)) return rc;
    HIPCHK(hipDeviceSynchronize());
    *h->fault_host = 0;
    h->frame_count = 0;
    h->group_count = 0;
    h->last_set = 0;
    h->prev_pipe = false;
    h->pending = 0;
    return 0;
}
```

### nnnoiseless_amd/csrc/nnn_batch_debug.hip

```cpp
#pragma once

struct TapDesc { int len; int is_int; int layout;  int sub_ofs; int sub_len; int needs_taps; };
static int last_slot(const nnn_batch *h) { return h ? (int)((h->frame_count + h->nslot - 1) % h->nslot) : 0; }
static bool tap_desc(const nnn_batch *h, int tap, TapDesc &d, const void **ptr)
{
    const Buffers *b = h ? &h->b[h->last_set] : nullptr;
#define TP(field) (b ? (const void *)b->field : nullptr)
    switch (tap) {
    case NNN_TAP_FILTERED: d = {FRAME, 0, 3, 0, FRAME, 0}; *ptr = TP(hist); return true;
    case NNN_TAP_XLP: d = {XLP, 0, 0, 0, XLP, 1}; *ptr = TP(xlp_ti); return true;
    case NNN_TAP_AC: d = {5, 0, 0, last_slot(h) * 10, (h ? h->nslot : 0) * 10, 0}; *ptr = TP(lpc); return true;
    case NNN_TAP_LPC2: d = {5, 0, 0, last_slot(h) * 10 + 5, (h ? h->nslot : 0) * 10, 0}; *ptr = TP(lpc); return true;
    case NNN_TAP_XCORR1: d = {NLAG1, 0, 0, 0, NLAG1, 1}; *ptr = TP(xc1); return true;
    case NNN_TAP_BEST1: d = {2, 1, 0, 0, 2, 1}; *ptr = TP(best1); return true;
    case NNN_TAP_XCORR2C: d = {10, 0, 0, 0, 10, 1}; *ptr = TP(xc2); return true;
    case NNN_TAP_PITCH_SEARCH: d = {1, 1, 0, 0, 1, 1}; *ptr = TP(psearch); return true;
    case NNN_TAP_PITCH: d = {1, 1, 0, 0, 1, 0}; *ptr = TP(pitch); return true;
    case NNN_TAP_PITCH_GAIN: d = {1, 0, 0, 0, 1, 0}; *ptr = TP(pgain); return true;
    case NNN_TAP_X: d = {2 * FREQ, 0, 2, 0, 2 * FREQ, 1}; *ptr = TP(X); return true;
    case NNN_TAP_P: d = {2 * FREQ, 0, 4, 0, 2 * FREQ, 1}; *ptr = TP(P); return true;
    case NNN_TAP_EX: d = {NB, 0, 0, 0, NB, 0}; *ptr = TP(ex); return true;
    case NNN_TAP_EP: d = {NB, 0, 0, 0, NB, 0}; *ptr = TP(ep); return true;
    case NNN_TAP_EXP: d = {NB, 0, 0, 0, NB, 0}; *ptr = TP(exp_); return true;
    case NNN_TAP_FEATURES: d = {NFEAT, 0, 0, 0, NFEAT, 1}; *ptr = TP(feat); return true;
    case NNN_TAP_SILENCE: d = {1, 1, 0, 0, 1, 0}; *ptr = TP(silence); return true;
    case NNN_TAP_G_RAW: d = {NB, 0, 0, 0, NB, 0}; *ptr = TP(g_raw); return true;
    case NNN_TAP_G: d = {NB, 0, 0, 0, NB, 0}; *ptr = TP(g); return true;
    case NNN_TAP_VAD: d = {1, 0, 0, 0, 1, 0}; *ptr = TP(vad); return true;
    case NNN_TAP_BRANCH: d = {1, 1, 0, 0, 1, 0}; *ptr = TP(branch); return true;
    default: return false;
    }
#undef TP
}

extern "C" int nnn_tap_info(int tap, int *len, int *is_int)
{
    TapDesc d;
    const void *p;
    if (!tap_desc(nullptr, tap, d, &p)) return fail("unknown tap %d", tap);
    if (len) *len = d.len;
    if (is_int) *is_int = d.is_int;
    return 0;
}

extern "C" int nnn_batch_set_taps(nnn_batch *h, int on)
{
    if (!h) return fail("null batch");
    if (on && !h->taps_alloc) {
        NNN_RT_LOCK;
        if (int rc = quiesce(h)) return rc;
        NNN_ALLOC_SETS(NNN_TAP_FIELDS);
        h->taps_alloc = true;
        HIPCHK(hipDeviceSynchronize());
    }
    for (int set = 0; set < h->nset; set++) h->b[set].taps = on == 2 ? 2 : (on != 0);
    return 0;
}

extern "C" int nnn_batch_read_tap(nnn_batch *h, int tap, void *host_dst, size_t dst_bytes)
{
    NNN_RT_LOCK;
    if (!h) return fail("null batch");
    TapDesc d;
    const void *p;
    if (!tap_desc(h, tap, d, &p)) return fail("unknown tap %d", tap);
    if (d.needs_taps && !h->b[0].taps) return fail("tap %d is only stored after nnn_batch_set_taps(batch, 1)", tap);
    if (dst_bytes < (size_t)h->S * d.len * 4) return fail("tap buffer too small");
    if (int rc = quiesce(h)) return rc;
    HIPCHK(hipDeviceSynchronize());
    uint32_t *dst = (uint32_t *)host_dst;
    const size_t Sp = (size_t)h->S_pad;
    if (d.layout == 0) {
        std::vector<uint32_t> tmp(Sp * d.sub_len);
        HIPCHK(hipMemcpy(tmp.data(), p, tmp.size() * 4, hipMemcpyDeviceToHost));
        for (int s = 0; s < h->S; s++)
            for (int i = 0; i < d.len; i++)
                dst[(size_t)s * d.len + i] = tmp[((size_t)(s / TILE) * d.sub_len + d.sub_ofs + i) * TILE + s % TILE];
    } else if (d.layout == 2 || d.layout == 4) {
        std::vector<uint32_t> tmp(Sp * 2 * FSTR);
        HIPCHK(hipMemcpy(tmp.data(), p, tmp.size() * 4, hipMemcpyDeviceToHost));
        for (int s = 0; s < h->S; s++)
            for (int k = 0; k < FREQ; k++) {
                const size_t at = (size_t)s * 2 * FSTR + 2 * (size_t)(d.layout == 4 ? spectrum_index_p(k) : spectrum_index(k));
                dst[(size_t)s * d.len + 2 * k] = tmp[at];
                dst[(size_t)s * d.len + 2 * k + 1] = tmp[at + 1];
            }
    } else {
        const size_t hstr = (size_t)hist_stride(h->nslot);
        std::vector<uint32_t> tmp(Sp * hstr);
        HIPCHK(hipMemcpy(tmp.data(), p, tmp.size() * 4, hipMemcpyDeviceToHost));
        int slot = last_slot(h);
        for (int s = 0; s < h->S; s++) memcpy(dst + (size_t)s * FRAME, tmp.data() + (size_t)s * hstr + slot * FRAME, FRAME * 4);
    }
    return 0;
}

extern "C" int nnn_batch_read_stamps(nnn_batch *h, long long *dst64)
{
    NNN_RT_LOCK;
    if (!h) return fail("null batch");
    HIPCHK(hipSetDevice(h->device));
    HIPCHK(hipDeviceSynchronize());
    HIPCHK(hipMemcpy(dst64, h->b[0].stamps, 64 * sizeof(long long), hipMemcpyDeviceToHost));
    return 0;
}

extern "C" int nnn_debug_activations(int device, int act, const float *x, float *y, int n)
{
    NNN_RT_LOCK;
    if (!x || !y || n < 0 || act < 0 || act > 2) return fail("bad argument");
    HIPCHK(hipSetDevice(device));
    std::vector<float> window, dct, tansig, bin_frac;
    std::vector<float2> tw;
    std::vector<int> bin_band;
    float wnorm;
    make_tables(window, dct, tw, tansig, bin_frac, bin_band, wnorm);
    float *d = nullptr;
    HIPCHK(hipMalloc((void **)&d, (size_t)(2 * n + 256) * sizeof(float)));
    float *dx = d + 256, *dy = dx + n;
    hipError_t e = hipMemcpy(d, tansig.data(), 201 * sizeof(float), hipMemcpyHostToDevice);
    if (e == hipSuccess) e = hipMemcpy(dx, x, (size_t)n * sizeof(float), hipMemcpyHostToDevice);
    if (e == hipSuccess && n) {
        hipLaunchKernelGGL(k_activation_kat, dim3((n + 255) / 256), dim3(256), 0, (hipStream_t) nullptr, (const float *)d, (const float *)dx, dy, act, n);
        e = hipDeviceSynchronize();
    }
    if (e == hipSuccess) e = hipMemcpy(y, dy, (size_t)n * sizeof(float), hipMemcpyDeviceToHost);
    hipFree(d);
    if (e != hipSuccess) return fail("activation sweep failed: %s", hipGetErrorString(e));
    return 0;
}

extern "C" int nnn_batch_set_profiling(nnn_batch *h, int on)
{
    if (!h) return fail("null batch");
    h->profiling = on != 0;
    return 0;
}
extern "C" int nnn_batch_num_kernels(void) { return K_COUNT; }
extern "C" const char *nnn_batch_kernel_name(int k) { return (k >= 0 && k < K_COUNT) ? kKernelNames[k] : ""; }
extern "C" int nnn_batch_read_kernel_times(nnn_batch *h, double *total_ms, int64_t *launches, int n)
{
    if (!h) return fail("null batch");
    for (int k = 0; k < n && k < K_COUNT; k++) {
        total_ms[k] = h->k_ms[k];
        launches[k] = h->k_launches[k];
        h->k_ms[k] = 0;
        h->k_launches[k] = 0;
    }
    return 0;
}
extern "C" int nnn_batch_set_graph(nnn_batch *h, int on)
{
    (void)on;
    if (!h) return fail("null batch");
    return 0;
}
extern "C" int nnn_batch_set_inputs_ready(nnn_batch *h, int on)
{
    if (!h) return fail("null batch");
    h->paths.inputs_ready = on != 0;
    return 0;
}
extern "C" int nnn_batch_set_frame_log(nnn_batch *h, void *d_log, size_t frames)
{
    if (!h) return fail("null batch");
    h->frame_log = (unsigned *)d_log;
    h->frame_log_left = d_log ? frames : 0;
    return 0;
}
extern "C" int nnn_batch_debug_withhold_flag(nnn_batch *h, int frames_ahead)
{
    if (!h) return fail("null batch");
    const int seq = frames_ahead < 0 ? 0 : (int)((h->frame_count + (uint64_t)frames_ahead) & 0x3fffffffu) + 1;
    for (int set = 0; set < h->nset; set++) {
        h->b[set].dbg_withhold = seq;
        h->b[set].handoff_ticks = seq ? 20000000ll : HANDOFF_TICKS;
    }
    return 0;
}
extern "C" int nnn_batch_debug_schedule(nnn_batch *h, int n_frames, int32_t *out, size_t cap)
{
    if (!h || !out) return fail("null argument");
    if (n_frames < 1) return fail("n_frames must be at least 1");
    CallPlan cp = plan_call(h, n_frames, h->stream);
    if ((size_t)n_frames > h->sp_tab.cap) cp.early_hp = false;
    const Schedule sc = plan_schedule(h, cp);
    constexpr size_t HEAD = 8, PER_NODE = 8 + 3 * MAX_WAITS;
    if (cap < HEAD + PER_NODE * sc.nodes.size()) return fail("schedule buffer too small: %zu entries needed", HEAD + PER_NODE * sc.nodes.size());
    const int32_t head[HEAD] = {(int32_t)sc.nodes.size(), (int32_t)cp.sizes.size(), cp.pipe, cp.sched, cp.lanes, sc.fill, sc.fill_after_done, sc.last_syn};
    memcpy(out, head, sizeof(head));
    out += HEAD;
    for (const Node &n : sc.nodes) {
        const int32_t v[8] = {n.stage, n.group, n.frames, n.first, n.stream, n.first_use, n.record, n.n_waits};
        memcpy(out, v, sizeof(v));
        for (int w = 0; w < MAX_WAITS; w++) {
            const Wait x = w < n.n_waits ? n.waits[w] : Wait{-1, -1, -1};
            out[8 + 3 * w] = x.origin, out[9 + 3 * w] = x.stage, out[10 + 3 * w] = x.group;
        }
        out += PER_NODE;
    }
    return 0;
}
extern "C" int nnn_batch_debug_host_plan(nnn_batch *h, int n_frames, const nnn_pcm_layout *L, int has_vad, int64_t out[8])
{
    if (!h || !out || n_frames < 1) return fail("null argument or no frames");
    if (int rc = check_layout(h, L)) return rc;
    const HostPlan p = plan_host_call(h, n_frames, *L, has_vad != 0);
    const int64_t v[8] = {p.route, p.chunk, p.n_chunks, (int64_t)p.span, (int64_t)p.vbytes, (int64_t)p.vofs, p.drop, p.vad_masked};
    memcpy(out, v, sizeof(v));
    return 0;
}
extern "C" int nnn_batch_set_back_end(nnn_batch *h, int mode)
{
    if (!h) return fail("null batch");
    if (mode < -1 || mode > 4) return fail("unknown back-end mode %d", mode);
    h->paths.back_mode = mode;
    return 0;
}
extern "C" int nnn_batch_set_pipeline(nnn_batch *h, int on)
{
    if (!h) return fail("null batch");
    h->paths.use_pipeline = on != 0;
    return 0;
}
extern "C" int nnn_batch_set_schedule(nnn_batch *h, int mode, int lanes)
{
    if (!h) return fail("null batch");
    if (mode < SCHED_SEQ || mode > SCHED_STAGES) return fail("unknown schedule %d", mode);
    h->paths.sched = mode;
    if (lanes >= 1 && lanes <= NSTREAMS - 1) h->paths.n_lanes = lanes;
    h->paths.sched_auto = false;
    return 0;
}
```

### nnnoiseless_amd/csrc/nnn_batch_launch.hip

```cpp
#pragma once

struct Launcher {
    nnn_batch *h;
    hipStream_t st;
    bool prof;
    template <class K, class... A> void go(int id, K kern, dim3 grid, dim3 block, size_t lds, A... args)
    {
        hipEvent_t e0 = nullptr, e1 = nullptr;
        if (prof) {
            hipEventCreate(&e0);
            hipEventCreate(&e1);
            hipEventRecord(e0, st);
        }
        hipLaunchKernelGGL(kern, grid, block, lds, st, args...);
        if (prof) {
            hipEventRecord(e1, st);
            h->evp.push_back(e0);
            h->evp.push_back(e1);
            h->evp_kernel.push_back(id);
        }
    }
};


static int lpc_launch(const nnn_batch *h, int g)
{
    const Paths &p = h->paths;
    const unsigned NT = (unsigned)h->NT, ug = (unsigned)g;
    if (p.lpc_wide >= 0 ? p.lpc_wide != 0 : NT * ug < 512u) return 0;
    int fc = LPC_FC;
    while (fc > 1 && NT * ((ug + fc - 1) / fc) < 2048u) fc /= 2;
    if (p.lpc_fc > 0) fc = p.lpc_fc < LPC_FC ? p.lpc_fc : LPC_FC;
    return fc;
}
static bool pitch_chained(const nnn_batch *h, int g)
{
    const int pc = h->paths.pitch_chain;
    return pc > 0 && g > 1 && (pc > 1 || (unsigned)h->S_pad / PK_SPB < 1024u);
}

static void plan_group(const nnn_batch *h, int g, GroupPlan &p)
{
    const Paths &k = h->paths;
    p.g = g;
    const int m = k.back_mode >= 0 ? k.back_mode : g > 1 ? 0 : ((h->S_pad <= 8192 && !h->beside_others) ? 1 : 3);
    const bool fused = m == 1 || m == 2, all_g = m == 2 || m == 4;
    p.back = m == 0 || (g > 1 && !all_g) ? BACK_UNFUSED : (fused ? BACK_FUSED : BACK_RNN_ALONE);
    for (const nnn_batch::ModelGroup &G : h->groups)
        if ((fused ? G.back_lds : G.rnn16_lds) == 0) p.back = BACK_UNFUSED;
    const bool split = k.hp_split >= 0 ? k.hp_split != 0 : h->NT <= 256;
    p.hp = !split ? 0 : ((k.hp_tpb ? k.hp_tpb == 2 : (g > 1 && h->NT >= 8)) ? 2 : 1);
    p.floor = h->n_floored > 0;
    p.link = h->link_ch > 1;
    p.held = h->n_held > 0;
    p.lpc_in_pitch = g == 1 && h->S_pad <= (split ? 8192 : 6144) && k.lpc_wide < 0 && k.lpc_fc == 0;
    p.head = p.lpc_in_pitch && split && k.lpc_head != 0;
    p.lpc_fc = p.lpc_in_pitch ? 0 : lpc_launch(h, g);
    p.chain = pitch_chained(h, g);
    p.riders = g == 1 && p.back == BACK_FUSED && (k.x_rides >= 0 ? k.x_rides != 0 : h->S_pad <= 8192);
    for (size_t i = 0; i < h->groups.size(); i++) {
        const nnn_batch::ModelGroup &G = h->groups[i];
        const int min_g = k.wf_min_g > 0 ? k.wf_min_g : ((G.ntiles * (TILE / WF_ROWS) >= 1024 || h->beside_others) ? 2 : 1);
        p.rnn[i] = p.back == BACK_RNN_ALONE ? RK_BACK : !(G.wf && g >= min_g) ? RK_PLAIN : G.shape_builtin ? RK_WF_BUILTIN : RK_WF_ANY;
    }
}

using RnnWfKernel = decltype(&k_rnn_wf<WfShapeAny>);
using BackKernel = decltype(&k_back<true, BkShapeBuiltin>);
using RnnPlainKernel = decltype(&k_rnn<false>);
static const RnnPlainKernel kRnnKernels[2] = {k_rnn<false>, k_rnn<true>};
static const auto kVadKernel = &k_vad;
static const auto kNetKernel = &k_net;
static const RnnWfKernel kRnnWfKernels[2] = {k_rnn_wf<WfShapeAny>, k_rnn_wf<BkShapeBuiltin>};
#define NNN_BK(F, XR, HELD, FLOOR) {k_back<F, BkShapeBuiltin, XR, HELD, FLOOR, false>, k_back<F, BkShapeBuiltin, XR, HELD, FLOOR, true>}
static const BackKernel kBackFused[2][2][2][2] = {
    {{NNN_BK(true, false, false, false), NNN_BK(true, false, false, true)}, {NNN_BK(true, false, true, false), NNN_BK(true, false, true, true)}},
    {{NNN_BK(true, true, false, false), NNN_BK(true, true, false, true)}, {NNN_BK(true, true, true, false), NNN_BK(true, true, true, true)}}};
static const BackKernel kBackRnnAlone[2][2][2] = {
    {NNN_BK(false, false, false, false), NNN_BK(false, false, false, true)},
    {NNN_BK(false, false, true, false), NNN_BK(false, false, true, true)}};
#undef NNN_BK
static std::vector<const void *> big_lds_kernels()
{
    std::vector<const void *> v;
    for (RnnPlainKernel k : kRnnKernels) v.push_back((const void *)k);
    for (RnnWfKernel k : kRnnWfKernels) v.push_back((const void *)k);
    for (const auto &by_held : kBackFused)
        for (const auto &by_floor : by_held)
            for (const auto &by_link : by_floor)
                for (BackKernel k : by_link) v.push_back((const void *)k);
    for (const auto &by_floor : kBackRnnAlone)
        for (const auto &by_link : by_floor)
            for (BackKernel k : by_link) v.push_back((const void *)k);
    v.push_back((const void *)kVadKernel);
    v.push_back((const void *)kNetKernel);
    return v;
}

static void launch_stage(nnn_batch *h, int s, int set0, const GroupPlan &p, const StepParams *sp0, hipStream_t st, bool prof, bool plain_out, const StepParams *call = nullptr, int fill = 0,
                         const SplitIo *io = nullptr)
{
    const int g = p.g;
    if (g <= 0) return;
    const unsigned NT = (unsigned)h->NT, Sp = (unsigned)h->S_pad, ug = (unsigned)g;
    const Buffers &b = h->b[set0];
    Launcher L{h, st, prof};
    switch (s) {
    case ST_HP:
        if (p.hp == 2)
            L.go(K_HP, p.held ? k_hp2<2, true> : k_hp2<2, false>, dim3((NT + 1) / 2 + (p.head ? (5 * NT + 3) / 4 : 0)), dim3(256), 0, b, sp0, g, call ? *call : StepParams{}, call ? fill : 0, p.head ? 1 : 0);
        else if (p.hp == 1)
            L.go(K_HP, p.held ? k_hp2<1, true> : k_hp2<1, false>, dim3(NT + (p.head ? (5 * NT + 1) / 2 : 0)), dim3(128), 0, b, sp0, g, call ? *call : StepParams{}, call ? fill : 0, p.head ? 1 : 0);
        else L.go(K_HP, p.held ? k_hp<true> : k_hp<false>, dim3(NT), dim3(64), 0, b, sp0, g, call ? *call : StepParams{}, call ? fill : 0);
        if (p.lpc_in_pitch) break;
        if (!p.lpc_fc) L.go(K_LPC, k_lpc_wide, dim3(NT * ug), dim3(320), 0, b, sp0, g);
        else L.go(K_LPC, k_lpc, dim3(NT * ((ug + p.lpc_fc - 1) / p.lpc_fc)), dim3(64), 0, b, sp0, g, p.lpc_fc);
        break;
    case ST_PITCH: {
        const int chain = p.chain ? 1 : 0, seq0 = (int)(h->frame_count & 0x3fffffffu) + 1;
        const unsigned grid = Sp / PK_SPB * (chain ? ug : 1u);
        if (p.lpc_in_pitch)
            L.go(K_PITCH, p.held ? k_pitch<true, true> : k_pitch<true, false>, dim3(grid + (p.riders ? Sp / 8 : 0u)), dim3(PK_T), 0, b, sp0, g, chain, seq0, h->tickets, p.head ? 2 : 1, p.riders ? (int)grid : 0);
        else
            L.go(K_PITCH, p.held ? k_pitch<false, true> : k_pitch<false, false>, dim3(grid + (p.riders ? Sp / 8 : 0u)), dim3(PK_T), 0, b, sp0, g, chain, seq0, h->tickets, 0, p.riders ? (int)grid : 0);
        if (chain) h->tickets += grid;
        break;
    }
    case ST_FFT:
        if (p.back == BACK_FUSED) {
            for (const nnn_batch::ModelGroup &G : h->groups)
                L.go(K_BACK, kBackFused[p.riders][p.held][p.floor][p.link], dim3((unsigned)(G.ntiles * (TILE / BK_ROWS))), dim3(BK_T), G.back_lds, b, sp0, G.acts, G.wq, G.fpar, G.tile0, g);
            break;
        }
        L.go(K_FFT_XP, k_fft_xp, dim3(Sp * ug / FFT_SPB), dim3(64 * FFT_SPB), 0, b, sp0, g);
        break;
    case ST_RNN:
        if (p.back == BACK_FUSED) break;
        for (size_t i = 0; i < h->groups.size(); i++) {
            const nnn_batch::ModelGroup &G = h->groups[i];
            if (p.rnn[i] == RK_BACK)
                L.go(K_RNN, kBackRnnAlone[p.held][p.floor][p.link], dim3((unsigned)(G.ntiles * (TILE / BK_ROWS))), dim3(BK_T), G.rnn16_lds, b, sp0, G.acts, G.wq, G.fpar, G.tile0, g);
            else if (p.rnn[i] == RK_WF_BUILTIN || p.rnn[i] == RK_WF_ANY)
                L.go(K_RNN, kRnnWfKernels[p.rnn[i] == RK_WF_BUILTIN], dim3((unsigned)(G.ntiles * (TILE / WF_ROWS))), dim3(64 * WF_WAVES), G.wf_lds, b, G.plan, G.wp,
                     G.wq, G.fpar, G.tile0, g);
            else
                L.go(K_RNN, kRnnKernels[p.link], dim3((unsigned)(G.ntiles * (TILE / G.rows))), dim3(64 * RNN_WAVES), G.rnn_lds, b, G.plan, G.wq, G.fpar,
                     G.tile0, G.rows, g);
        }
        break;
    case ST_SYN:
        if (p.back == BACK_FUSED) break;
        if (plain_out) L.go(K_SYNTH, k_synth<true>, dim3(Sp / FFT_SPB), dim3(64 * FFT_SPB), 0, b, sp0, g);
        else L.go(K_SYNTH, k_synth<false>, dim3(Sp / FFT_SPB), dim3(64 * FFT_SPB), 0, b, sp0, g);
        break;
    case ST_FEAT:
        hipLaunchKernelGGL(k_features, dim3(NT), dim3(64 * FEAT_WAVES), 0, st, b, g);
        hipLaunchKernelGGL(k_features_out, dim3(NT * ug), dim3(FOUT_T), 0, st, b, io->features, io->silence, g);
        break;
    case ST_GAINS:
        hipLaunchKernelGGL(k_gains_in, dim3(NT), dim3(GIN_T), 0, st, b, io->gains, io->vad, g);
        break;
    case ST_FFT_FEAT:
        if (b.taps) hipLaunchKernelGGL(k_fft_xp, dim3(Sp * ug / FFT_SPB), dim3(64 * FFT_SPB), 0, st, b, sp0, g);
        else hipLaunchKernelGGL(k_fft_feat, dim3(Sp * ug / FFT_SPB), dim3(64 * FFT_SPB), 0, st, b, sp0, g);
        break;
    case ST_VAD:
        hipLaunchKernelGGL(k_features, dim3(NT), dim3(64 * FEAT_WAVES), 0, st, b, g);
        for (const nnn_batch::ModelGroup &G : h->groups)
            hipLaunchKernelGGL(kVadKernel, dim3((unsigned)(G.ntiles * (TILE / G.vad_rows))), dim3(64 * RNN_WAVES), G.vad_lds, st, b, sp0, G.plan, G.wq,
                               G.fpar, G.tile0, G.vad_rows, G.vad_mb, g);
        break;
    }
}

static int drain_profile(nnn_batch *h)
{
    for (size_t i = 0; i < h->evp_kernel.size(); i++) {
        float ms = 0.0f;
        HIPCHK(hipEventSynchronize(h->evp[2 * i + 1]));
        HIPCHK(hipEventElapsedTime(&ms, h->evp[2 * i], h->evp[2 * i + 1]));
        h->k_ms[h->evp_kernel[i]] += ms;
        h->k_launches[h->evp_kernel[i]] += 1;
        hipEventDestroy(h->evp[2 * i]);
        hipEventDestroy(h->evp[2 * i + 1]);
    }
    h->evp.clear();
    h->evp_kernel.clear();
    return 0;
}

struct CallPlan {
    std::vector<int> sizes;
    bool pipe;
    int sched, lanes;
    bool fold_fill, early_hp, hp_after;
    bool idle;
};
static CallPlan plan_call(const nnn_batch *h, int n_frames, hipStream_t st)
{
    const Paths &k = h->paths;
    CallPlan c;
    constexpr int PIPE_MIN = 32;
    const bool auto_big = k.sched_auto && h->S_pad > AUTO_BIG;
    c.idle = h->n_held == h->S;
    c.pipe = !c.idle && k.use_pipeline && k.sched != SCHED_SEQ && !h->profiling && n_frames >= PIPE_MIN && !(auto_big && h->depth < 2);
    if (c.pipe) {
        int n = 2;
        while ((n_frames + n - 1) / n > h->gmax) n += 2;
        if (n > n_frames) n = n_frames;
        for (int i = 0; i < n; i++) c.sizes.push_back(n_frames / n + (i < n_frames % n ? 1 : 0));
    } else {
        for (int rem = n_frames; rem > 0; rem -= c.sizes.back()) c.sizes.push_back(rem < h->gmax ? rem : h->gmax);
    }
    c.sched = auto_big ? (c.sizes.size() <= 2 ? SCHED_STAGES : SCHED_LANES) : k.sched;
    c.lanes = auto_big ? 2 : k.n_lanes;
    c.fold_fill = (!c.pipe && !h->profiling) || c.idle;
    c.early_hp = c.pipe && k.inputs_ready && !h->host_call && h->prev_pipe && h->prev_st == st && c.sched == SCHED_LANES && h->pool[0];
    c.hp_after = c.sched == SCHED_LANES && c.lanes == 1 && h->S_pad >= 8192;
    return c;
}

constexpr int MAX_WAITS = 1 + 1 + 1;
static_assert(MAX_WAITS >= 1 + 1, "hp: the pitch kernel before it (hp_after) and the ring edge; rnn, synth: previous stage and previous group; fft_xp: previous stage");
enum WaitOrigin { W_THIS = 0, W_PREV = 1, W_DONE = 2 };
enum FillWhere { FILL_FOLDED = 0, FILL_CALLER = 1, FILL_POOL0 = 2 };
struct Wait { int origin, stage, group; };
struct Node {
    int stage, group, frames, first;
    int stream;
    bool first_use;
    bool record;
    bool fill;
    int n_waits;
    Wait waits[MAX_WAITS];
};
struct Schedule {
    std::vector<Node> nodes;
    int fill = FILL_FOLDED;
    bool fill_after_done = false;
    int last_syn = -1;
};

static Schedule plan_schedule(const nnn_batch *h, const CallPlan &cp)
{
    Schedule sc;
    const int n_groups = (int)cp.sizes.size(), par = (int)((h->call_count + 1) & 1);
    sc.fill = cp.early_hp ? FILL_POOL0 : (cp.fold_fill ? FILL_FOLDED : FILL_CALLER);
    sc.fill_after_done = cp.early_hp && h->have_done[par];
    if (cp.idle) return sc;
    auto stream_of = [&](int s, int k) -> int {
        if (!cp.pipe) return -1;
        if (cp.sched == SCHED_STAGES) return s == ST_HP ? 0 : (s == ST_PITCH ? 1 : (s == ST_FFT ? 2 : (s == ST_RNN ? 3 : -1)));
        return s == ST_HP ? 0 : (k % cp.lanes) - (k % cp.lanes == 0 ? 1 : 0);
    };
    auto consumers_elsewhere = [&](int s, int k) {
        const int me = stream_of(s, k);
        if (s + 1 < ST_COUNT && stream_of(s + 1, k) != me) return true;
        if ((s == ST_HP || s == ST_PITCH || s == ST_RNN || s == ST_SYN) && k + 1 < n_groups && stream_of(s, k + 1) != me) return true;
        if (s == ST_SYN) return true;
        if (cp.hp_after && s == ST_PITCH) return true;
        return false;
    };
    bool used[NSTREAMS] = {cp.early_hp};
    const int pn = (int)h->prev_first.size();
    sc.nodes.reserve((size_t)n_groups * ST_COUNT);
    for (int k = 0, t = 0; k < n_groups; t += cp.sizes[k++]) {
        const int g = cp.sizes[k];
        for (int s = 0; s < ST_COUNT; s++) {
            Node n = {};
            const int si = stream_of(s, k);
            n.stage = s, n.group = k, n.frames = g, n.first = t, n.stream = si;
            n.first_use = si >= 0 && !used[si];
            if (si >= 0) used[si] = true;
            n.fill = cp.fold_fill && k == 0 && s == ST_HP;
            n.record = cp.pipe && consumers_elsewhere(s, k);
            auto wait = [&](int origin, int ds, int dk) { n.waits[n.n_waits++] = Wait{origin, ds, dk}; };
            auto wait_for = [&](int ds, int dk) {
                if (dk < 0 || dk < k - EVR + 1) return;
                if (stream_of(ds, dk) != si) wait(W_THIS, ds, dk);
            };
            if (s > 0) wait_for(s - 1, k);
            if (s == ST_HP || s == ST_PITCH || s == ST_RNN || s == ST_SYN) wait_for(s, k - 1);
            if (s == ST_PITCH) wait_for(ST_SYN, k - h->depth);
            if (s == ST_HP && cp.hp_after) {
                if (k > 0) wait_for(ST_PITCH, k - 1);
                else if (cp.early_hp && pn > 0) wait(W_PREV, ST_PITCH, pn - 1);
            }
            if (s == ST_HP && cp.pipe) {
                const int need = t + g - 1 + 3 - h->nslot;
                int dk = -1;
                for (int j = 0; j < k; j++)
                    if (sc.nodes[(size_t)j * ST_COUNT].first <= need) dk = j;
                wait_for(ST_SYN, dk);
                if (cp.early_hp && need < 0) {
                    const long long pf = (long long)h->frame_count + need - (long long)h->prev_frame0;
                    int pj = -1;
                    for (int j = 0; j < pn; j++)
                        if (h->prev_first[j] <= pf) pj = j;
                    if (pf >= 0 && pj >= 0 && pn - pj < EVR) wait(W_PREV, ST_SYN, pj);
                    else if (h->have_done[par]) wait(W_DONE, 0, 0);
                }
            }
            sc.nodes.push_back(n);
        }
    }
    if (stream_of(ST_SYN, n_groups - 1) >= 0) sc.last_syn = n_groups - 1;
    return sc;
}
static hipEvent_t wait_event(const nnn_batch *h, int par, const Wait &w)
{
    return w.origin == W_DONE ? h->ev_done[par] : h->ev[w.origin == W_PREV ? h->prev_par : par][w.stage][w.group % EVR];
}

static int process_frames(nnn_batch *h, const void *d_in, void *d_out, float *d_vad, int n_frames, int fmt, int channels,
                          long long group_stride, long long frame_stride, int drop, void *hip_stream)
{
    HIPCHK(hipSetDevice(h->device));
    if (int rc = report_fault(h)) return rc;
    const bool plain_out = fmt == PCM_F32 && channels == 1;
    {
        const uint64_t mask = (1ull << 44) - 1;
        const uint64_t now = (uint64_t)std::chrono::duration_cast<std::chrono::microseconds>(std::chrono::steady_clock::now().time_since_epoch()).count() & mask;
        const uint64_t prev = g_call_mark[h->device].exchange((h->id << 44) | now, std::memory_order_relaxed);
        if ((prev >> 44) != h->id && (prev >> 44) != 0 && now - (prev & mask) < 5000) h->other_seen_us = now | (1ull << 63);
        h->beside_others = (h->other_seen_us >> 63) && now - (h->other_seen_us & mask) < 20000;
        if (h->beside_others) {
            static std::atomic<bool> told{false};
            if (!getenv("GPU_MAX_HW_QUEUES") && !told.exchange(true))
                fprintf(stderr, "nnnoiseless_mi355x: several batches are being driven side by side on device %d and GPU_MAX_HW_QUEUES is not set; "
                                "the HIP runtime then maps their streams onto 4 hardware queues and they largely serialise "
                                "(export GPU_MAX_HW_QUEUES=8 before the process starts -- INTEGRATION.md; any value of the variable silences this note)\n", h->device);
        }
    }
    hipError_t e;
    hipStream_t st = call_begin(h, hip_stream, e);
    if (e != hipSuccess) return fail("hipStreamWaitEvent(st, h->ev_last, 0) failed: %s", hipGetErrorString(e));
    StepParams v0;
    v0.in = (const char *)d_in;
    v0.out = (char *)d_out;
    v0.vad = d_vad;
    v0.group_stride = group_stride;
    v0.frame_stride = frame_stride;
    v0.fmt = fmt;
    v0.channels = channels;
    v0.discard = drop;
    v0.slot = (int)(h->frame_count % h->nslot);
    v0.n_streams = h->S;
    v0.log = h->frame_log_left ? h->frame_log : nullptr;
    v0.log_frames = (int)(h->frame_log_left < (size_t)n_frames ? h->frame_log_left : (size_t)n_frames);
    if (v0.log) {
        h->frame_log += (size_t)v0.log_frames * h->S * FRAME_LOG_WORDS;
        h->frame_log_left -= (size_t)v0.log_frames;
    }
    if ((size_t)n_frames > h->sp_tab.cap) {
        const size_t cap = n_frames < 64 ? 64 : (size_t)n_frames;
        if (int rc = grow(h, true, h->sp_tab, 2 * cap * sizeof(StepParams), cap)) return rc;
        h->prev_pipe = false;
    }
    const CallPlan cp = plan_call(h, n_frames, st);
    const Schedule sc = plan_schedule(h, cp);
    const int n_groups = (int)cp.sizes.size();
    h->call_count += 1;
    const int par = (int)(h->call_count & 1);
    StepParams *const tab = h->sp_tab.p + (size_t)par * h->sp_tab.cap;
    const uint64_t frame0 = h->frame_count;
    bool ok = true;
    if (sc.fill != FILL_FOLDED) {
        hipStream_t fs = sc.fill == FILL_POOL0 ? h->pool[0] : st;
        if (sc.fill_after_done) ok &= hipStreamWaitEvent(fs, h->ev_done[par], 0) == hipSuccess;
        hipLaunchKernelGGL(k_fill_params, dim3((n_frames + 63) / 64), dim3(64), 0, fs, tab, v0, n_frames, h->nslot);
    }
    if (cp.pipe) ok &= hipEventRecord(h->ev_in, st) == hipSuccess;
    size_t i = 0;
    for (int k = 0; k < n_groups; k++) {
        const int g = cp.sizes[k], set0 = (int)(h->group_count % h->depth) * h->gmax;
        plan_group(h, g, h->plan);
        for (; i < sc.nodes.size() && sc.nodes[i].group == k; i++) {
            const Node &n = sc.nodes[i];
            if (n.stream >= 0 && !h->pool[n.stream]) ok &= hipStreamCreateWithFlags(&h->pool[n.stream], hipStreamNonBlocking) == hipSuccess;
            hipStream_t ss = n.stream < 0 ? st : h->pool[n.stream];
            if (n.first_use) ok &= hipStreamWaitEvent(ss, h->ev_in, 0) == hipSuccess;
            for (int w = 0; w < n.n_waits; w++) ok &= hipStreamWaitEvent(ss, wait_event(h, par, n.waits[w]), 0) == hipSuccess;
            launch_stage(h, n.stage, set0, h->plan, tab + n.first, ss, h->profiling, plain_out, n.fill ? &v0 : nullptr, n_frames);
            if (n.record) ok &= hipEventRecord(h->ev[par][n.stage][k % EVR], ss) == hipSuccess;
        }
        h->group_count += 1;
        h->frame_count += g;
        h->last_set = set0 + g - 1;
    }
    if (sc.last_syn >= 0) ok &= hipStreamWaitEvent(st, h->ev[par][ST_SYN][sc.last_syn % EVR], 0) == hipSuccess;
    h->prev_pipe = cp.pipe;
    if (cp.pipe) {
        h->prev_st = st;
        h->prev_frame0 = frame0;
        h->prev_par = par;
        h->prev_first.clear();
        for (int k = 0; k < n_groups; k++) h->prev_first.push_back(sc.nodes[(size_t)k * ST_COUNT].first);
    }
    ok &= hipEventRecord(h->ev_done[par], st) == hipSuccess;
    h->have_done[par] = true;
    ok &= call_end(h, st) == hipSuccess;
    if (!ok) return fail("stream/event call failed while enqueueing frames: %s", hipGetErrorString(hipGetLastError()));
    HIPCHK(hipGetLastError());
    if (h->profiling) {
        HIPCHK(hipStreamSynchronize(st));
        return drain_profile(h);
    }
    return 0;
}

static int check_layout(const nnn_batch *h, const nnn_pcm_layout *L)
{
    if (!L) return fail("null layout");
    if (L->format != NNN_PCM_F32 && L->format != NNN_PCM_I16 && L->format != NNN_PCM_F32_UNIT) return fail("unknown sample format %d", L->format);
    if (L->channels < 1 || h->S % L->channels) return fail("n_streams (%d) is not a multiple of channels (%d)", h->S, L->channels);
    if (L->frame_stride < (size_t)FRAME * L->channels) return fail("frame_stride smaller than one frame of all channels");
    return 0;
}

extern "C" int nnn_batch_process_device(nnn_batch *h, const float *d_in, float *d_out, float *d_vad, int n_frames,
                                        size_t stream_stride, size_t frame_stride, void *hip_stream)
{
    if (!h) return fail("null batch");
    if (int rc = refuse_pending(h, "nnn_batch_process_device")) return rc;
    if (n_frames <= 0) return 0;
    if (!d_in || !d_out) return fail("null buffer");
    if (n_frames > 1 && frame_stride < (size_t)FRAME) return fail("frame_stride smaller than one frame");
    return process_frames(h, d_in, d_out, d_vad, n_frames, PCM_F32, 1, (long long)stream_stride * 4, (long long)frame_stride * 4, 0,
                          hip_stream);
}

extern "C" int nnn_batch_process_pcm_device(nnn_batch *h, const void *d_in, void *d_out, float *d_vad, int n_frames,
                                            const nnn_pcm_layout *L, void *hip_stream)
{
    if (!h) return fail("null batch");
    if (int rc = refuse_pending(h, "nnn_batch_process_pcm_device")) return rc;
    if (n_frames <= 0) return 0;
    if (!d_in || !d_out) return fail("null buffer");
    if (int rc = check_layout(h, L)) return rc;
    const long long e = pcm_elem_bytes(L->format);
    const int drop = (L->discard_first && h->frame_count == 0) ? 1 : 0;
    return process_frames(h, d_in, d_out, d_vad, n_frames, L->format, L->channels, (long long)L->group_stride * e,
                          (long long)L->frame_stride * e, drop, hip_stream);
}
```

### nnnoiseless_amd/csrc/nnn_rnn_wf.hip

```cpp
#pragma once

namespace nnn {

constexpr int WF_ROWS = 16, WF_WAVES = 12, WF_FS_W = 72;

struct WfGru {
    f32x4 acc[3][2];
    float zz[4], sold[4];
};
constexpr int WF_KS_REC = 3;
struct WfWeights {
    Frags<2, WF_KS_REC> zr;
    Frags<1, WF_KS_REC> h;
    float bias[3];
};
__device__ __forceinline__ void wf_load_weights(WfWeights &w, const LayerDesc &L, const uint4 *__restrict__ Wq, const float *__restrict__ fpar,
                                                int nbi, int lane)
{
    const uint4 *Brec = Wq + L.rec.wofs + (size_t)nbi * 3 * L.rec.ksteps * 64;
    load_frags<2, 0, WF_KS_REC>(w.zr, L.rec, Brec, lane);
    load_frags<1, 2, WF_KS_REC>(w.h, L.rec, Brec, lane);
    const int neuron = nbi * 16 + (lane & 15);
#pragma unroll
    for (int g = 0; g < 3; g++) w.bias[g] = neuron < L.n ? fpar[L.bias + g * L.n + neuron] : 0.0f;
}

__device__ __forceinline__ void wf_gru_a(const LayerDesc &L, const unsigned short *Ain, int in_w, const unsigned short *SP, unsigned short *RS,
                                         int sw, const uint4 *__restrict__ Wq, const WfWeights &w, const float *tab, int nbi, int lane, WfGru &u)
{
    const float scale = 1.0f / 256.0f;
    const int neuron = nbi * 16 + (lane & 15);
    const bool nvalid = neuron < L.n;
    const uint4 *Bin = Wq + L.in.wofs + (size_t)nbi * 3 * L.in.ksteps * 64;
    const uint4 *Brec = Wq + L.rec.wofs + (size_t)nbi * 3 * L.rec.ksteps * 64;
    Frags<3> f_in;
    load_frags<3, 0>(f_in, L.in, Bin, lane);
#pragma unroll
    for (int g = 0; g < 3; g++) u.acc[g][0] = f32x4{w.bias[g], w.bias[g], w.bias[g], w.bias[g]};
    const int ps = WF_ROWS * sw;
    gemm_acc<2, 1, 0, WF_KS_REC>(u.acc, SP, ps, sw, 0, L.rec, Brec, lane, w.zr);
    gemm_acc<3, 1, 0>(u.acc, Ain, WF_ROWS * in_w, in_w, 0, L.in, Bin, lane, f_in);
    const int kcols = 32 * L.rec.ksteps;
#pragma unroll
    for (int q = 0; q < 4; q++) {
        const int row = 4 * (lane >> 4) + q;
        const float so = nvalid ? load_split(SP, ps, row * sw + neuron) : 0.0f;
        u.sold[q] = so;
        u.zz[q] = sigmoid_approx(scale * u.acc[0][0][q], tab);
        const float rs = so * sigmoid_approx(scale * u.acc[1][0][q], tab);
        if (neuron < kcols) store_split(RS, ps, row * sw + neuron, rs);
        if (nbi == L.nb - 1 && neuron + 16 < kcols) store_split(RS, ps, row * sw + neuron + 16, 0.0f);
    }
}

template <class Sink>
__device__ __forceinline__ void wf_gru_b(const LayerDesc &L, const unsigned short *RS, int sw, const uint4 *__restrict__ Wq, const WfWeights &w,
                                         const float *tab, const int *live, int nbi, int lane, WfGru &u, Sink &&sink)
{
    const float scale = 1.0f / 256.0f;
    const int neuron = nbi * 16 + (lane & 15);
    const uint4 *Brec = Wq + L.rec.wofs + (size_t)nbi * 3 * L.rec.ksteps * 64;
    gemm_acc<1, 1, 2, WF_KS_REC>(u.acc, RS, WF_ROWS * sw, sw, 0, L.rec, Brec, lane, w.h);
    if (neuron < L.n) {
#pragma unroll
        for (int q = 0; q < 4; q++) {
            const int row = 4 * (lane >> 4) + q;
            const float hh = activate(L.act, scale * u.acc[2][0][q], tab);
            const float z = u.zz[q], so = u.sold[q];
            float snew = z * so + (1.0f - z) * hh;
            snew = live[row] ? snew : so;
            sink(row, neuron, snew);
        }
    }
}

struct WfFeatIn {
    float mine[7];
    int pitch, silent;
};
__device__ __forceinline__ void wf_features_load(WfWeights &w, const Buffers &b, int f, int tile, int r0, int lane)
{
    const int row = lane & 15, part = lane >> 4, trow = r0 + row;
    const float *cg = NNN_TIF(b, cn, 28, f, tile, trow);
    unsigned m[7];
#pragma unroll
    for (int i = 0; i < 7; i++) m[i] = __float_as_uint(cg[(size_t)(7 * part + i) * TILE]);
    w.zr.f[0][0] = make_uint4(m[0], m[1], m[2], m[3]);
    w.zr.f[0][1] = make_uint4(m[4], m[5], m[6], (unsigned)NNN_TIF(b, pitch, 1, f, tile, trow)[0]);
    w.h.f[0][0].x = (unsigned)NNN_TIF(b, silence, 1, f, tile, trow)[0];
}
__device__ __forceinline__ WfFeatIn wf_features_in(const WfWeights &w)
{
    WfFeatIn in;
    const uint4 a = w.zr.f[0][0], c = w.zr.f[0][1];
    in.mine[0] = __uint_as_float(a.x); in.mine[1] = __uint_as_float(a.y); in.mine[2] = __uint_as_float(a.z); in.mine[3] = __uint_as_float(a.w);
    in.mine[4] = __uint_as_float(c.x); in.mine[5] = __uint_as_float(c.y); in.mine[6] = __uint_as_float(c.z);
    in.pitch = (int)c.w;
    in.silent = (int)w.h.f[0][0].x;
    return in;
}
template <int KIND, int KB, int SRC_B, int RB, bool HALF>
__device__ __forceinline__ void wf_feature_outputs(const Buffers &b, int f, int tile, int trow, int part, bool silent, const float *cnb_l,
                                                   const float *r1_l, const float *r2_l, unsigned short *fs_l)
{
    constexpr int rm = WF_ROWS;
    if (HALF && part >= 2) return;
    const float v0 = cnb_l[SRC_B * rm];
    const float v1 = (KIND == 0 || KIND == 3) ? r1_l[RB * rm] : 0.0f;
    const float v2 = (KIND == 0 || KIND == 2 || KIND == 3) ? r2_l[RB * rm] : 0.0f;
    const float a = KIND == 0 ? v1 : (KIND == 3 ? -(2.0f * v1) : 0.0f);
    const float c = (KIND == 0 || KIND == 3) ? v2 : (KIND == 2 ? -v2 : 0.0f);
    float v = (v0 + a) + c;
    v = silent ? 0.0f : v;
    if (b.taps) NNN_TIF(b, feat, NFEAT, f, tile, trow)[(size_t)(KB + part) * TILE] = v;
    store_split(fs_l, rm * WF_FS_W, KB, v);
}

__device__ __forceinline__ void wf_features(const Buffers &b, const WfFeatIn &in, int f, int tile, int r0, int lane, float *crs, float *dc,
                                            float *cnb, unsigned short *FS, int *live_f, int &mem_id)
{
    constexpr int rm = WF_ROWS;
    const int row = lane & 15, part = lane >> 4, trow = r0 + row;
    const int pitch = in.pitch;
    const bool silent = in.silent != 0;
    NNN_STAMPW(b, 8, f == 3);
#pragma unroll
    for (int i = 0; i < 7; i++) cnb[(7 * part + i) * rm + row] = in.mine[i];
    wave_lds_sync();
    if (part == 0) live_f[row] = silent ? 0 : 1;
    const int c0 = mem_id, c1 = mem_id < 1 ? CEPS_MEM + mem_id - 1 : mem_id - 1;
    const int c2 = mem_id < 2 ? CEPS_MEM + mem_id - 2 : mem_id - 2;
    NNN_STAMPW(b, 9, f == 3);
    if (!silent) {
        float *cm = NNN_TI(b.ceps_mem, CEPS_MEM * NB, tile, trow);
        for (int k = part; k < NB; k += 4) {
            const float v = cnb[k * rm + row];
            cm[(size_t)(c0 * NB + k) * TILE] = v;
            crs[(c0 * NB + k) * rm + row] = v;
        }
        mem_id = mem_id + 1 == CEPS_MEM ? 0 : mem_id + 1;
        NNN_STAMPW(b, 10, f == 3);
        const int ia = part, ib = part + 4 < CEPS_MEM - 1 ? part + 4 : part;
        const int ja = ia < c0 ? ia : ia + 1, jb = ib < c0 ? ib : ib + 1;
        const float *ra = crs + (ja * NB) * rm + row, *rb = crs + (jb * NB) * rm + row, *nw = cnb + row;
        float da = 0.0f, db = 0.0f;
#pragma unroll
        for (int k = 0; k < NB; k++) {
            const float x = nw[k * rm];
            const float ea = x - ra[k * rm], eb = x - rb[k * rm];
            da += ea * ea;
            db += eb * eb;
        }
        dc[pair_index(ja < c0 ? ja : c0, ja < c0 ? c0 : ja) * rm + row] = da;
        if (part + 4 < CEPS_MEM - 1) dc[pair_index(jb < c0 ? jb : c0, jb < c0 ? c0 : jb) * rm + row] = db;
    }
    NNN_STAMPW(b, 11, f == 3);
    wave_lds_sync();
    {
        const float *cnb_l = cnb + part * rm + row;
        const float *r1_l = crs + (c1 * NB + part) * rm + row, *r2_l = crs + (c2 * NB + part) * rm + row;
        unsigned short *fs_l = FS + row * WF_FS_W + part;
        wf_feature_outputs<0, 0, 0, 0, false>(b, f, tile, trow, part, silent, cnb_l, r1_l, r2_l, fs_l);
        wf_feature_outputs<0, 4, 4, 4, true>(b, f, tile, trow, part, silent, cnb_l, r1_l, r2_l, fs_l);
        wf_feature_outputs<1, 6, 6, 0, false>(b, f, tile, trow, part, silent, cnb_l, r1_l, r2_l, fs_l);
        wf_feature_outputs<1, 10, 10, 0, false>(b, f, tile, trow, part, silent, cnb_l, r1_l, r2_l, fs_l);
        wf_feature_outputs<1, 14, 14, 0, false>(b, f, tile, trow, part, silent, cnb_l, r1_l, r2_l, fs_l);
        wf_feature_outputs<1, 18, 18, 0, false>(b, f, tile, trow, part, silent, cnb_l, r1_l, r2_l, fs_l);
        wf_feature_outputs<2, NB, 0, 0, false>(b, f, tile, trow, part, silent, cnb_l, r1_l, r2_l, fs_l);
        wf_feature_outputs<2, NB + 4, 4, 4, true>(b, f, tile, trow, part, silent, cnb_l, r1_l, r2_l, fs_l);
        wf_feature_outputs<3, NB + 6, 0, 0, false>(b, f, tile, trow, part, silent, cnb_l, r1_l, r2_l, fs_l);
        wf_feature_outputs<3, NB + 10, 4, 4, true>(b, f, tile, trow, part, silent, cnb_l, r1_l, r2_l, fs_l);
        wf_feature_outputs<1, NB + 12, NB, 0, false>(b, f, tile, trow, part, silent, cnb_l, r1_l, r2_l, fs_l);
        wf_feature_outputs<1, NB + 16, NB + 4, 0, true>(b, f, tile, trow, part, silent, cnb_l, r1_l, r2_l, fs_l);
    }
    NNN_STAMPW(b, 12, f == 3);
    if (part < 2) {
        float v = part == 0 ? 0.01f * ((float)pitch - 300.0f) : spectral_variability(dc, row, rm);
        v = silent ? 0.0f : v;
        if (b.taps) NNN_TIF(b, feat, NFEAT, f, tile, trow)[(size_t)(40 + part) * TILE] = v;
        store_split(FS, rm * WF_FS_W, row * WF_FS_W + 40 + part, v);
    }
    NNN_STAMPW(b, 13, f == 3);
}

template <int KS> struct WfDenseW {
    Frags<1, KS> fr;
    float bias;
};
template <int KS>
__device__ __forceinline__ void wf_dense_load(WfDenseW<KS> &w, const LayerDesc &L, const uint4 *__restrict__ Wq, const float *__restrict__ fpar,
                                              int nbi, int lane)
{
    load_frags<1, 0, KS>(w.fr, L.in, Wq + L.in.wofs + (size_t)nbi * L.in.ksteps * 64, lane);
    const int neuron = nbi * 16 + (lane & 15);
    w.bias = neuron < L.n ? fpar[L.bias + neuron] : 0.0f;
}
template <bool QUAD = false, int KS, class Sink>
__device__ __forceinline__ void wf_dense(const LayerDesc &L, const unsigned short *Ain, int in_w, const uint4 *__restrict__ Wq, const WfDenseW<KS> &w,
                                         const float *tab, int nbi, int lane, Sink &&sink)
{
    const int neuron = nbi * 16 + (lane & 15);
    const uint4 *Bnb = Wq + L.in.wofs + (size_t)nbi * L.in.ksteps * 64;
    f32x4 acc[3][2];
    acc[0][0] = f32x4{w.bias, w.bias, w.bias, w.bias};
    gemm_acc<1, 1, 0, KS>(acc, Ain, WF_ROWS * in_w, in_w, 0, L.in, Bnb, lane, w.fr);
    if (neuron < L.n) {
        if constexpr (QUAD) {
            float v[4];
#pragma unroll
            for (int q = 0; q < 4; q++) v[q] = activate(L.act, acc[0][0][q] * (1.0f / 256.0f), tab);
            sink(4 * (lane >> 4), neuron, v);
        } else {
#pragma unroll
            for (int q = 0; q < 4; q++) sink(4 * (lane >> 4) + q, neuron, activate(L.act, acc[0][0][q] * (1.0f / 256.0f), tab));
        }
    }
}

#ifndef NNN_WF_MINWAVES
#define NNN_WF_MINWAVES 3
#endif
struct WfPlan {
    int w_v, w_n, w_dn;
    int sw_v, sw_n, sw_dn;
};

__host__ __device__ constexpr WfPlan wf_plan_of(const RnnPlan &pl)
{
    return WfPlan{32 * pl.vad.in.ksteps + 8, 32 * pl.noise.in.ksteps + 8, 32 * pl.dn.in.ksteps + 8,
                  rnn_state_w(pl.vad), rnn_state_w(pl.noise), rnn_state_w(pl.dn)};
}
struct WfLds { int tab, live, Xv, Xn, Xdn, SPv, SPn, SPdn, RSv, RSn, RSdn, FS, crs, dc, cnb, total; };
__host__ __device__ constexpr WfLds wf_lds(const WfPlan &w)
{
    constexpr int plane3 = 3 * WF_ROWS * 2;
    WfLds o{};
    int at = 0;
    o.tab = lds_take(at, 256 * 4);
    o.live = lds_take(at, 8 * WF_ROWS * 4);
    o.Xv = lds_take(at, plane3 * w.w_v);
    o.Xn = lds_take(at, 2 * plane3 * w.w_n);
    o.Xdn = lds_take(at, 3 * plane3 * w.w_dn);
    o.SPv = lds_take(at, plane3 * w.sw_v);
    o.SPn = lds_take(at, plane3 * w.sw_n);
    o.SPdn = lds_take(at, plane3 * w.sw_dn);
    o.RSv = lds_take(at, plane3 * w.sw_v);
    o.RSn = lds_take(at, plane3 * w.sw_n);
    o.RSdn = lds_take(at, plane3 * w.sw_dn);
    o.FS = lds_take(at, plane3 * WF_FS_W);
    o.crs = lds_take(at, CEPS_MEM * NB * WF_ROWS * 4);
    o.dc = lds_take(at, 28 * WF_ROWS * 4);
    o.cnb = lds_take(at, 28 * WF_ROWS * 4);
    o.total = at;
    return o;
}
static_assert(wf_lds(wf_plan_of(BkShapeBuiltin::plan())).total == 127744, "k_rnn_wf's LDS for the built-in shape class");
struct WfShapeAny { static constexpr bool fixed = false; };
template <class SH> struct WfFixed { static constexpr bool value = true; };
template <> struct WfFixed<WfShapeAny> { static constexpr bool value = false; };
template <class SH>
__global__ void __launch_bounds__(64 * WF_WAVES, NNN_WF_MINWAVES) k_rnn_wf(Buffers b, RnnPlan pl_rt, WfPlan wp_rt, const uint4 *__restrict__ Wq,
                                                            const float *__restrict__ fpar, int tile0, int g)
{
    RnnPlan pl = pl_rt;
    WfPlan wp = wp_rt;
    if constexpr (WfFixed<SH>::value) {
        constexpr RnnPlan p0 = SH::plan();
        constexpr WfPlan w0 = wf_plan_of(p0);
        pl = p0;
        pl.dense.act = pl_rt.dense.act; pl.vad.act = pl_rt.vad.act; pl.noise.act = pl_rt.noise.act; pl.dn.act = pl_rt.dn.act;
        pl.out.act = pl_rt.out.act; pl.act_vo = pl_rt.act_vo;
        wp = w0;
    }
    HIP_DYNAMIC_SHARED(float, lds_raw)
    constexpr int rm = WF_ROWS;
    const int wave0 = __builtin_amdgcn_readfirstlane((int)(threadIdx.x >> 6));
    const int lane0 = threadIdx.x & 63;
    int wave = wave0, lane = lane0;
    int tile, r0;
    if (!rnn_block_rows(b, tile0, rm, tile, r0)) return;
    if (!live_any(b, tile, r0, rm)) return;
    const bool rowl = lane0 < rm;
    const int trow = r0 + (rowl ? lane0 : 0);
    NNN_STAMP(b, 50);
    const WfLds o = wf_lds(wp);
    auto planes = [&](int at) { return (unsigned short *)(lds_raw + at / 4); };
    float *tab = lds_raw + o.tab / 4;
    int *live = (int *)(lds_raw + o.live / 4);
    unsigned short *Xv = planes(o.Xv), *Xn = planes(o.Xn), *Xdn = planes(o.Xdn);
    unsigned short *SPv = planes(o.SPv), *SPn = planes(o.SPn), *SPdn = planes(o.SPdn);
    unsigned short *RSv = planes(o.RSv), *RSn = planes(o.RSn), *RSdn = planes(o.RSdn);
    unsigned short *FS = planes(o.FS);
    float *crs = lds_raw + o.crs / 4, *dc = lds_raw + o.dc / 4, *cnb = lds_raw + o.cnb / 4;
    const int cD = pl.dense.out_col, cV = pl.cV, cF = pl.cF;
    float *sv = b.gru_v + ((size_t)tile * TILE * b.gru_v_w + (size_t)r0 * pl.vad.n),
          *sn = b.gru_n + ((size_t)tile * TILE * b.gru_n_w + (size_t)r0 * pl.noise.n),
          *sdn = b.gru_dn + ((size_t)tile * TILE * b.gru_dn_w + (size_t)r0 * pl.dn.n);
    {
        uint4 *z = (uint4 *)Xv;
        const int n16 = (int)(((char *)crs - (char *)Xv) / 16);
        for (int i = (int)threadIdx.x; i < n16; i += 64 * WF_WAVES) z[i] = make_uint4(0u, 0u, 0u, 0u);
        for (int i = (int)threadIdx.x; i < 201; i += 64 * WF_WAVES) tab[i] = b.tansig[i];
        const float *cm = NNN_TI(b.ceps_mem, CEPS_MEM * NB, tile, trow);
        constexpr int PER = (CEPS_MEM * NB + WF_WAVES - 1) / WF_WAVES;
        float stg[PER];
#pragma unroll
        for (int i = 0; i < PER; i++) {
            const int r = wave + i * WF_WAVES;
            stg[i] = (rowl && r < CEPS_MEM * NB) ? cm[(size_t)r * TILE] : 0.0f;
        }
#pragma unroll
        for (int i = 0; i < PER; i++) {
            const int r = wave + i * WF_WAVES;
            if (rowl && r < CEPS_MEM * NB) crs[r * rm + lane] = stg[i];
        }
    }
    lds_barrier();
    constexpr int T = 64 * WF_WAVES;
    gru_state_io<T>(pl.vad, rm, sv, SPv, wp.sw_v, true);
    gru_state_io<T>(pl.noise, rm, sn, SPn, wp.sw_n, true);
    gru_state_io<T>(pl.dn, rm, sdn, SPdn, wp.sw_dn, true);
    if (rowl)
        for (int p = wave; p < 28; p += WF_WAVES) dc[p * rm + lane] = pair_dist(crs, p, lane, rm);
    int mem_id = wave == WF_WAVES - 1 ? NNN_TI(b.mem_id, 1, tile, r0 + (lane & 15))[0] : 0;
    const int W_N = 6, W_V = 9, W_F = 11;
    WfWeights wts;
    if (wave < W_N) wf_load_weights(wts, pl.dn, Wq, fpar, wave < pl.dn.nb ? wave : 0, lane);
    else if (wave < W_V) wf_load_weights(wts, pl.noise, Wq, fpar, wave - W_N < pl.noise.nb ? wave - W_N : 0, lane);
    else if (wave < W_F) wf_load_weights(wts, pl.vad, Wq, fpar, wave - W_V < pl.vad.nb ? wave - W_V : 0, lane);
    else wf_load_weights(wts, pl.vad, Wq, fpar, 0, lane);
    lds_barrier();
    NNN_STAMP(b, 51);
    WfGru ua;
    if (wave == WF_WAVES - 1 && g > 0) wf_features_load(wts, b, 0, tile, r0, lane);
    if (wave0 == WF_WAVES - 1) wf_setprio_high();
    for (int t = -1; t < g + 3; t++) {
        lane = launder_v(lane0);
        wave = launder_s(wave0);
        const int fv = t, fn = t - 1, fd = t - 2, fo = t - 3, ff = t + 1;
        const bool on_v = fv >= 0 && fv < g, on_n = fn >= 0 && fn < g, on_d = fd >= 0 && fd < g, on_o = fo >= 0 && fo < g,
                   on_f = ff >= 0 && ff < g;
        unsigned short *Xn_n = Xn + (fn & 1) * 3 * rm * wp.w_n;
        unsigned short *Xdn_d = Xdn + ((fd + 3) % 3) * 3 * rm * wp.w_dn;
        const int srole = wave0 == 0 ? 0 : (wave0 == 6 ? 1 : (wave0 == 9 ? 2 : (wave0 == 11 ? 3 : -1)));
        NNN_STAMPW(b, 30 + 5 * srole, t == 2 && srole >= 0);
        if (wave < W_N) {
            if (on_d && wave < pl.dn.nb) wf_gru_a(pl.dn, Xdn_d, wp.w_dn, SPdn, RSdn, wp.sw_dn, Wq, wts, tab, wave, lane, ua);
        } else if (wave < W_V) {
            if (on_n && wave - W_N < pl.noise.nb) wf_gru_a(pl.noise, Xn_n - cV, wp.w_n, SPn, RSn, wp.sw_n, Wq, wts, tab, wave - W_N, lane, ua);
        } else if (wave < W_F) {
            WfDenseW<3> dw;
            const bool mine_o = on_o && wave - W_V < pl.out.nb;
            if (on_v && wave - W_V < pl.vad.nb) wf_gru_a(pl.vad, Xv - cD, wp.w_v, SPv, RSv, wp.sw_v, Wq, wts, tab, wave - W_V, lane, ua);
            if (mine_o) {
                const int *lv = live + 16 * (fo & 7);
                wf_dense_load(dw, pl.out, Wq, fpar, wave - W_V, lane);
                wf_dense<true>(pl.out, SPdn, wp.sw_dn, Wq, dw, tab, wave - W_V, lane, [&](int lrow, int band, const float (&v)[4]) {
                    if (b.link) {
                        rnn_gain_out4(b, fo, tile, r0 + lrow, band, lv + lrow, v);
                    } else {
#pragma unroll
                        for (int q = 0; q < 4; q++) rnn_gain_out(b, fo, tile, r0 + lrow + q, band, lv[lrow + q] != 0, v[q]);
                    }
                });
            }
        } else {
            if (on_f) wf_features(b, wf_features_in(wts), ff, tile, r0, lane, crs, dc, cnb, FS, live + 16 * (ff & 7), mem_id);
            if (ff + 1 >= 0 && ff + 1 < g) wf_features_load(wts, b, ff + 1, tile, r0, lane);
        }
        NNN_STAMPW(b, 31 + 5 * srole, t == 2 && srole >= 0);
#if defined(NNN_STAMPS) && NNN_WFSTAMP_PHASE == 1
        NNN_STAMPW(b, 14 + wave0, t == 2);
#endif
        lds_barrier();
        NNN_STAMPW(b, 32 + 5 * srole, t == 2 && srole >= 0);
        if (wave < W_N) {
            WfDenseW<2> dw;
            const bool mine_d = on_f && wave < pl.dense.nb;
            if (on_d && wave < pl.dn.nb)
                wf_gru_b(pl.dn, RSdn, wp.sw_dn, Wq, wts, tab, live + 16 * (fd & 7), wave, lane, ua,
                         [&](int row, int n, float v) { store_split(SPdn, rm * wp.sw_dn, row * wp.sw_dn + n, v); });
            if (mine_d) {
                unsigned short *Xnn = Xn + (ff & 1) * 3 * rm * wp.w_n;
                wf_dense_load(dw, pl.dense, Wq, fpar, wave, lane);
                wf_dense(pl.dense, FS - cF, WF_FS_W, Wq, dw, tab, wave, lane, [&](int row, int n, float v) {
                    store_split(Xv, rm * wp.w_v, row * wp.w_v + n, v);
                    store_split(Xnn, rm * wp.w_n, row * wp.w_n + (cD - cV) + n, v);
                });
            }
        } else if (wave < W_V) {
            if (on_n && wave - W_N < pl.noise.nb) {
                unsigned short *Xd = Xdn + (fn % 3) * 3 * rm * wp.w_dn;
                wf_gru_b(pl.noise, RSn, wp.sw_n, Wq, wts, tab, live + 16 * (fn & 7), wave - W_N, lane, ua, [&](int row, int n, float v) {
                    store_split(SPn, rm * wp.sw_n, row * wp.sw_n + n, v);
                    store_split(Xd, rm * wp.w_dn, row * wp.w_dn + n, v);
                });
            }
            if (on_f) {
                unsigned short *Xnn = Xn + (ff & 1) * 3 * rm * wp.w_n, *Xd = Xdn + (ff % 3) * 3 * rm * wp.w_dn;
                for (int i = 64 * (wave - W_N) + lane; i < 3 * rm * 6; i += 64 * (W_V - W_N)) {
                    const int plx = i / (rm * 6), rem = i - plx * rm * 6, row = rem / 6, c8 = rem - row * 6;
                    const uint4 v = *(const uint4 *)(FS + (size_t)plx * rm * WF_FS_W + row * WF_FS_W + 8 * c8);
                    *(uint4 *)(Xnn + (size_t)plx * rm * wp.w_n + row * wp.w_n + (cF - cV) + 8 * c8) = v;
                    *(uint4 *)(Xd + (size_t)plx * rm * wp.w_dn + row * wp.w_dn + cF + 8 * c8) = v;
                }
            }
        } else if (wave < W_F) {
            if (on_v && wave - W_V < pl.vad.nb) {
                unsigned short *Xnn = Xn + (fv & 1) * 3 * rm * wp.w_n, *Xd = Xdn + (fv % 3) * 3 * rm * wp.w_dn;
                wf_gru_b(pl.vad, RSv, wp.sw_v, Wq, wts, tab, live + 16 * (fv & 7), wave - W_V, lane, ua, [&](int row, int n, float v) {
                    store_split(SPv, rm * wp.sw_v, row * wp.sw_v + n, v);
                    store_split(Xnn, rm * wp.w_n, row * wp.w_n + n, v);
                    store_split(Xd, rm * wp.w_dn, row * wp.w_dn + cV + n, v);
                });
            }
        } else {
            if (on_n && rowl) {
                const unsigned short *Xv1 = Xn + (fn & 1) * 3 * rm * wp.w_n;
                NNN_TIF(b, vad, 1, fn, tile, trow)[0] = rnn_vad_out(pl, fpar, Xv1, rm * wp.w_n, wp.w_n, 0, lane, live + 16 * (fn & 7), tab);
            }
        }
        NNN_STAMPW(b, 33 + 5 * srole, t == 2 && srole >= 0);
#if defined(NNN_STAMPS) && NNN_WFSTAMP_PHASE == 2
        NNN_STAMPW(b, 14 + wave0, t == 2);
#endif
        lds_barrier();
        NNN_STAMPW(b, 34 + 5 * srole, t == 2 && srole >= 0);
    }
    gru_state_io<T>(pl.vad, rm, sv, SPv, wp.sw_v, false);
    gru_state_io<T>(pl.noise, rm, sn, SPn, wp.sw_n, false);
    gru_state_io<T>(pl.dn, rm, sdn, SPdn, wp.sw_dn, false);
    if (wave0 == WF_WAVES - 1 && rowl) NNN_TI(b.mem_id, 1, tile, trow)[0] = mem_id;
    NNN_STAMP(b, 52);
}

}
```

Measured before the change: 76.10 million frames/s.

## Add 32-row variant of fused wavefront RNN kernel with unified LDS layout

Adds a templated k_rnn_wf path for the built-in model shape that processes 32 stream rows per workgroup (two 16-row MFMA blocks), using a new unified per-row LDS column layout. The 32-row form is picked automatically when the block count is large (at least 2048 blocks) or through a new NNN_WF_ROWS knob or set_wf_rows API. The aim is to reuse the loaded GRU weights across more rows per workgroup and cut per-block overhead, at the cost of more LDS and registers per block and possibly lower occupancy. The built-in 16-row path also moves to the new layout.

```diff
diff --git a/include/nnn_batch.h b/include/nnn_batch.h
--- a/include/nnn_batch.h
+++ b/include/nnn_batch.h
@@ -157,6 +157,7 @@
 int nnn_batch_set_pipeline(nnn_batch *b, int on);
 int nnn_batch_set_inputs_ready(nnn_batch *b, int on);
 int nnn_batch_set_back_end(nnn_batch *b, int mode);
+int nnn_batch_set_wf_rows(nnn_batch *b, int rows);
 int nnn_batch_set_schedule(nnn_batch *b, int mode, int lanes);
 
 int nnn_debug_activations(int device, int act, const float *x, float *y, int n);
diff --git a/nnnoiseless_amd/__init__.py b/nnnoiseless_amd/__init__.py
--- a/nnnoiseless_amd/__init__.py
+++ b/nnnoiseless_amd/__init__.py
@@ -396,6 +396,9 @@
     def set_back_end(self, mode):
         self._lib.check(self._lib.L.nnn_batch_set_back_end(self._h, int(mode)))
 
+    def set_wf_rows(self, rows):
+        self._lib.check(self._lib.L.nnn_batch_set_wf_rows(self._h, int(rows)))
+
     def set_pipeline(self, on):
         self._lib.check(self._lib.L.nnn_batch_set_pipeline(self._h, int(on)))
 
diff --git a/nnnoiseless_amd/_ffi.py b/nnnoiseless_amd/_ffi.py
--- a/nnnoiseless_amd/_ffi.py
+++ b/nnnoiseless_amd/_ffi.py
@@ -24,7 +24,7 @@
     "nnn_batch_analyze_device", "nnn_batch_synthesize_device", "nnn_batch_analyze_host", "nnn_batch_synthesize_host", "nnn_batch_pending_frames",
     "nnn_batch_vad_device", "nnn_batch_vad_host", "nnn_batch_network_device", "nnn_batch_network_host",
     "nnn_batch_set_gain_floor", "nnn_batch_get_gain_floor", "nnn_batch_num_floored",
-    "nnn_batch_set_channel_link", "nnn_batch_get_channel_link",
+    "nnn_batch_set_channel_link", "nnn_batch_get_channel_link", "nnn_batch_set_wf_rows",
 ]
 TRAIN_SYMBOLS = [
     "nnn_train_create", "nnn_train_destroy", "nnn_train_reset", "nnn_train_process_device", "nnn_train_process_host",
@@ -204,7 +204,7 @@
                          ("nnn_batch_debug_schedule", [vp, i32, C.POINTER(C.c_int32), sz]),
                          ("nnn_batch_debug_host_plan", [vp, i32, C.POINTER(PcmLayout), i32, C.POINTER(C.c_int64)]),
                          ("nnn_batch_create_opts", [C.POINTER(vp), C.POINTER(i32), i32, i32, C.POINTER(BatchOpts)]),
-                         ("nnn_batch_max_group_frames", [vp]), ("nnn_batch_device_bytes", [vp]), ("nnn_batch_set_back_end", [vp, i32])):
+                         ("nnn_batch_max_group_frames", [vp]), ("nnn_batch_device_bytes", [vp]), ("nnn_batch_set_back_end", [vp, i32]), ("nnn_batch_set_wf_rows", [vp, i32])):
             if hasattr(L, name):
                 getattr(L, name).argtypes = at
         if hasattr(L, "nnn_batch_create_opts"):
diff --git a/nnnoiseless_amd/csrc/nnn_batch_core.hip b/nnnoiseless_amd/csrc/nnn_batch_core.hip
--- a/nnnoiseless_amd/csrc/nnn_batch_core.hip
+++ b/nnnoiseless_amd/csrc/nnn_batch_core.hip
@@ -75,6 +75,7 @@
     int host_chunk = -1;
     int wf_min_g = 0;
     int rnn_rows = 0;
+    int wf_rows = 0;
     int hp_split = -1;
     int lpc_head = -1;
     int pitch_chain = 1;
@@ -113,11 +114,15 @@
         const int v = atoi(e);
         if (v == 16 || v == 32) p.rnn_rows = v;
     }
+    if (const char *e = dev_knob("NNN_WF_ROWS")) {
+        const int v = atoi(e);
+        if (v == 16 || v == 32) p.wf_rows = v;
+    }
     return p;
 }
 
 enum BackEnd { BACK_UNFUSED = 0, BACK_RNN_ALONE = 1, BACK_FUSED = 2 };
-enum RnnKernel : uint8_t { RK_BACK, RK_WF_BUILTIN, RK_WF_ANY, RK_PLAIN };
+enum RnnKernel : uint8_t { RK_BACK, RK_WF_BUILTIN, RK_WF_ANY, RK_PLAIN, RK_WF_BUILTIN32 };
 struct GroupPlan {
     int g = 0;
     BackEnd back = BACK_UNFUSED;
@@ -158,7 +163,7 @@
         bool wf = false;
         bool shape_builtin = false;
         WfPlan wp;
-        size_t wf_lds = 0;
+        size_t wf_lds = 0, wf32_lds = 0;
         int rows = 32;
         int tile0 = 0, ntiles = 0;
         size_t back_lds = 0, rnn16_lds = 0;
diff --git a/nnnoiseless_amd/csrc/nnn_batch_create.hip b/nnnoiseless_amd/csrc/nnn_batch_create.hip
--- a/nnnoiseless_amd/csrc/nnn_batch_create.hip
+++ b/nnnoiseless_amd/csrc/nnn_batch_create.hip
@@ -120,6 +120,10 @@
         G.back_lds = shape_ok && fb <= kLdsMax ? fb : 0;
         G.rnn16_lds = shape_ok && rb <= kLdsMax ? rb : 0;
         G.acts = BkActs{G.plan.dense.act, G.plan.vad.act, G.plan.noise.act, G.plan.dn.act, G.plan.out.act, G.plan.act_vo};
+    }
+    if (G.shape_builtin) {
+        G.wf_lds = (size_t)wfu_lds(wfu_cols(BkShapeBuiltin::plan()), 16).total;
+        G.wf32_lds = (size_t)wfu_lds(wfu_cols(BkShapeBuiltin::plan()), 32).total;
     }
     G.wf = !paths.rnn_rows && G.plan.dense.nb <= 2 && G.plan.vad.nb <= 2 && G.plan.noise.nb <= 3 && G.plan.dn.nb <= 6 && G.plan.vad.rec.ksteps <= WF_KS_REC &&
            G.plan.noise.rec.ksteps <= WF_KS_REC && G.plan.dn.rec.ksteps <= WF_KS_REC && G.wf_lds <= kLdsMax;
diff --git a/nnnoiseless_amd/csrc/nnn_batch_debug.hip b/nnnoiseless_amd/csrc/nnn_batch_debug.hip
--- a/nnnoiseless_amd/csrc/nnn_batch_debug.hip
+++ b/nnnoiseless_amd/csrc/nnn_batch_debug.hip
@@ -217,6 +217,13 @@
     h->paths.back_mode = mode;
     return 0;
 }
+extern "C" int nnn_batch_set_wf_rows(nnn_batch *h, int rows)
+{
+    if (!h) return fail("null batch");
+    if (rows != 0 && rows != 16 && rows != 32) return fail("k_rnn_wf has 16 or 32 rows per workgroup, not %d", rows);
+    h->paths.wf_rows = rows;
+    return 0;
+}
 extern "C" int nnn_batch_set_pipeline(nnn_batch *h, int on)
 {
     if (!h) return fail("null batch");
diff --git a/nnnoiseless_amd/csrc/nnn_batch_launch.hip b/nnnoiseless_amd/csrc/nnn_batch_launch.hip
--- a/nnnoiseless_amd/csrc/nnn_batch_launch.hip
+++ b/nnnoiseless_amd/csrc/nnn_batch_launch.hip
@@ -39,6 +39,7 @@
     return pc > 0 && g > 1 && (pc > 1 || (unsigned)h->S_pad / PK_SPB < 1024u);
 }
 
+constexpr int WF32_MIN_BLOCKS = 2048;
 static void plan_group(const nnn_batch *h, int g, GroupPlan &p)
 {
     const Paths &k = h->paths;
@@ -61,7 +62,8 @@
     for (size_t i = 0; i < h->groups.size(); i++) {
         const nnn_batch::ModelGroup &G = h->groups[i];
         const int min_g = k.wf_min_g > 0 ? k.wf_min_g : ((G.ntiles * (TILE / WF_ROWS) >= 1024 || h->beside_others) ? 2 : 1);
-        p.rnn[i] = p.back == BACK_RNN_ALONE ? RK_BACK : !(G.wf && g >= min_g) ? RK_PLAIN : G.shape_builtin ? RK_WF_BUILTIN : RK_WF_ANY;
+        const bool rows32 = G.wf32_lds && (k.wf_rows ? k.wf_rows == 32 : G.ntiles * (TILE / WF_ROWS) >= WF32_MIN_BLOCKS);
+        p.rnn[i] = p.back == BACK_RNN_ALONE ? RK_BACK : !(G.wf && g >= min_g) ? RK_PLAIN : G.shape_builtin ? (rows32 ? RK_WF_BUILTIN32 : RK_WF_BUILTIN) : RK_WF_ANY;
     }
 }
 
@@ -71,7 +73,7 @@
 static const RnnPlainKernel kRnnKernels[2] = {k_rnn<false>, k_rnn<true>};
 static const auto kVadKernel = &k_vad;
 static const auto kNetKernel = &k_net;
-static const RnnWfKernel kRnnWfKernels[2] = {k_rnn_wf<WfShapeAny>, k_rnn_wf<BkShapeBuiltin>};
+static const RnnWfKernel kRnnWfKernels[3] = {k_rnn_wf<WfShapeAny>, k_rnn_wf<BkShapeBuiltin>, k_rnn_wf<BkShapeBuiltin, 32>};
 #define NNN_BK(F, XR, HELD, FLOOR) {k_back<F, BkShapeBuiltin, XR, HELD, FLOOR, false>, k_back<F, BkShapeBuiltin, XR, HELD, FLOOR, true>}
 static const BackKernel kBackFused[2][2][2][2] = {
     {{NNN_BK(true, false, false, false), NNN_BK(true, false, false, true)}, {NNN_BK(true, false, true, false), NNN_BK(true, false, true, true)}},
@@ -140,6 +142,8 @@
             const nnn_batch::ModelGroup &G = h->groups[i];
             if (p.rnn[i] == RK_BACK)
                 L.go(K_RNN, kBackRnnAlone[p.held][p.floor][p.link], dim3((unsigned)(G.ntiles * (TILE / BK_ROWS))), dim3(BK_T), G.rnn16_lds, b, sp0, G.acts, G.wq, G.fpar, G.tile0, g);
+            else if (p.rnn[i] == RK_WF_BUILTIN32)
+                L.go(K_RNN, kRnnWfKernels[2], dim3((unsigned)(G.ntiles * (TILE / 32))), dim3(64 * WF_WAVES), G.wf32_lds, b, G.plan, G.wp, G.wq, G.fpar, G.tile0, g);
             else if (p.rnn[i] == RK_WF_BUILTIN || p.rnn[i] == RK_WF_ANY)
                 L.go(K_RNN, kRnnWfKernels[p.rnn[i] == RK_WF_BUILTIN], dim3((unsigned)(G.ntiles * (TILE / WF_ROWS))), dim3(64 * WF_WAVES), G.wf_lds, b, G.plan, G.wp,
                      G.wq, G.fpar, G.tile0, g);
diff --git a/nnnoiseless_amd/csrc/nnn_rnn_wf.hip b/nnnoiseless_amd/csrc/nnn_rnn_wf.hip
--- a/nnnoiseless_amd/csrc/nnn_rnn_wf.hip
+++ b/nnnoiseless_amd/csrc/nnn_rnn_wf.hip
@@ -1,4 +1,5 @@
 #pragma once
+#include <utility>
 
 namespace nnn {
 
@@ -78,30 +79,30 @@
     float mine[7];
     int pitch, silent;
 };
-__device__ __forceinline__ void wf_features_load(WfWeights &w, const Buffers &b, int f, int tile, int r0, int lane)
+__device__ __forceinline__ void wf_features_load(WfWeights &w, const Buffers &b, int f, int tile, int r0, int lane, int k = 0)
 {
     const int row = lane & 15, part = lane >> 4, trow = r0 + row;
     const float *cg = NNN_TIF(b, cn, 28, f, tile, trow);
     unsigned m[7];
 #pragma unroll
     for (int i = 0; i < 7; i++) m[i] = __float_as_uint(cg[(size_t)(7 * part + i) * TILE]);
-    w.zr.f[0][0] = make_uint4(m[0], m[1], m[2], m[3]);
-    w.zr.f[0][1] = make_uint4(m[4], m[5], m[6], (unsigned)NNN_TIF(b, pitch, 1, f, tile, trow)[0]);
-    w.h.f[0][0].x = (unsigned)NNN_TIF(b, silence, 1, f, tile, trow)[0];
-}
-__device__ __forceinline__ WfFeatIn wf_features_in(const WfWeights &w)
+    w.zr.f[k][0] = make_uint4(m[0], m[1], m[2], m[3]);
+    w.zr.f[k][1] = make_uint4(m[4], m[5], m[6], (unsigned)NNN_TIF(b, pitch, 1, f, tile, trow)[0]);
+    w.h.f[k][0].x = (unsigned)NNN_TIF(b, silence, 1, f, tile, trow)[0];
+}
+__device__ __forceinline__ WfFeatIn wf_features_in(const WfWeights &w, int k = 0)
 {
     WfFeatIn in;
-    const uint4 a = w.zr.f[0][0], c = w.zr.f[0][1];
+    const uint4 a = w.zr.f[k][0], c = w.zr.f[k][1];
     in.mine[0] = __uint_as_float(a.x); in.mine[1] = __uint_as_float(a.y); in.mine[2] = __uint_as_float(a.z); in.mine[3] = __uint_as_float(a.w);
     in.mine[4] = __uint_as_float(c.x); in.mine[5] = __uint_as_float(c.y); in.mine[6] = __uint_as_float(c.z);
     in.pitch = (int)c.w;
-    in.silent = (int)w.h.f[0][0].x;
+    in.silent = (int)w.h.f[k][0].x;
     return in;
 }
 template <int KIND, int KB, int SRC_B, int RB, bool HALF>
 __device__ __forceinline__ void wf_feature_outputs(const Buffers &b, int f, int tile, int trow, int part, bool silent, const float *cnb_l,
-                                                   const float *r1_l, const float *r2_l, unsigned short *fs_l)
+                                                   const float *r1_l, const float *r2_l, unsigned short *fs_l, int fs_ps)
 {
     constexpr int rm = WF_ROWS;
     if (HALF && part >= 2) return;
@@ -113,11 +114,12 @@
     float v = (v0 + a) + c;
     v = silent ? 0.0f : v;
     if (b.taps) NNN_TIF(b, feat, NFEAT, f, tile, trow)[(size_t)(KB + part) * TILE] = v;
-    store_split(fs_l, rm * WF_FS_W, KB, v);
-}
-
+    store_split(fs_l, fs_ps, KB, v);
+}
+
+template <int DIST_UNROLL = NB>
 __device__ __forceinline__ void wf_features(const Buffers &b, const WfFeatIn &in, int f, int tile, int r0, int lane, float *crs, float *dc,
-                                            float *cnb, unsigned short *FS, int *live_f, int &mem_id)
+                                            float *cnb, unsigned short *FS, int *live_f, int &mem_id, int fs_ps = WF_ROWS * WF_FS_W, int fs_w = WF_FS_W)
 {
     constexpr int rm = WF_ROWS;
     const int row = lane & 15, part = lane >> 4, trow = r0 + row;
@@ -144,7 +146,7 @@
         const int ja = ia < c0 ? ia : ia + 1, jb = ib < c0 ? ib : ib + 1;
         const float *ra = crs + (ja * NB) * rm + row, *rb = crs + (jb * NB) * rm + row, *nw = cnb + row;
         float da = 0.0f, db = 0.0f;
-#pragma unroll
+#pragma unroll DIST_UNROLL
         for (int k = 0; k < NB; k++) {
             const float x = nw[k * rm];
             const float ea = x - ra[k * rm], eb = x - rb[k * rm];
@@ -159,26 +161,26 @@
     {
         const float *cnb_l = cnb + part * rm + row;
         const float *r1_l = crs + (c1 * NB + part) * rm + row, *r2_l = crs + (c2 * NB + part) * rm + row;
-        unsigned short *fs_l = FS + row * WF_FS_W + part;
-        wf_feature_outputs<0, 0, 0, 0, false>(b, f, tile, trow, part, silent, cnb_l, r1_l, r2_l, fs_l);
-        wf_feature_outputs<0, 4, 4, 4, true>(b, f, tile, trow, part, silent, cnb_l, r1_l, r2_l, fs_l);
-        wf_feature_outputs<1, 6, 6, 0, false>(b, f, tile, trow, part, silent, cnb_l, r1_l, r2_l, fs_l);
-        wf_feature_outputs<1, 10, 10, 0, false>(b, f, tile, trow, part, silent, cnb_l, r1_l, r2_l, fs_l);
-        wf_feature_outputs<1, 14, 14, 0, false>(b, f, tile, trow, part, silent, cnb_l, r1_l, r2_l, fs_l);
-        wf_feature_outputs<1, 18, 18, 0, false>(b, f, tile, trow, part, silent, cnb_l, r1_l, r2_l, fs_l);
-        wf_feature_outputs<2, NB, 0, 0, false>(b, f, tile, trow, part, silent, cnb_l, r1_l, r2_l, fs_l);
-        wf_feature_outputs<2, NB + 4, 4, 4, true>(b, f, tile, trow, part, silent, cnb_l, r1_l, r2_l, fs_l);
-        wf_feature_outputs<3, NB + 6, 0, 0, false>(b, f, tile, trow, part, silent, cnb_l, r1_l, r2_l, fs_l);
-        wf_feature_outputs<3, NB + 10, 4, 4, true>(b, f, tile, trow, part, silent, cnb_l, r1_l, r2_l, fs_l);
-        wf_feature_outputs<1, NB + 12, NB, 0, false>(b, f, tile, trow, part, silent, cnb_l, r1_l, r2_l, fs_l);
-        wf_feature_outputs<1, NB + 16, NB + 4, 0, true>(b, f, tile, trow, part, silent, cnb_l, r1_l, r2_l, fs_l);
+        unsigned short *fs_l = FS + row * fs_w + part;
+        wf_feature_outputs<0, 0, 0, 0, false>(b, f, tile, trow, part, silent, cnb_l, r1_l, r2_l, fs_l, fs_ps);
+        wf_feature_outputs<0, 4, 4, 4, true>(b, f, tile, trow, part, silent, cnb_l, r1_l, r2_l, fs_l, fs_ps);
+        wf_feature_outputs<1, 6, 6, 0, false>(b, f, tile, trow, part, silent, cnb_l, r1_l, r2_l, fs_l, fs_ps);
+        wf_feature_outputs<1, 10, 10, 0, false>(b, f, tile, trow, part, silent, cnb_l, r1_l, r2_l, fs_l, fs_ps);
+        wf_feature_outputs<1, 14, 14, 0, false>(b, f, tile, trow, part, silent, cnb_l, r1_l, r2_l, fs_l, fs_ps);
+        wf_feature_outputs<1, 18, 18, 0, false>(b, f, tile, trow, part, silent, cnb_l, r1_l, r2_l, fs_l, fs_ps);
+        wf_feature_outputs<2, NB, 0, 0, false>(b, f, tile, trow, part, silent, cnb_l, r1_l, r2_l, fs_l, fs_ps);
+        wf_feature_outputs<2, NB + 4, 4, 4, true>(b, f, tile, trow, part, silent, cnb_l, r1_l, r2_l, fs_l, fs_ps);
+        wf_feature_outputs<3, NB + 6, 0, 0, false>(b, f, tile, trow, part, silent, cnb_l, r1_l, r2_l, fs_l, fs_ps);
+        wf_feature_outputs<3, NB + 10, 4, 4, true>(b, f, tile, trow, part, silent, cnb_l, r1_l, r2_l, fs_l, fs_ps);
+        wf_feature_outputs<1, NB + 12, NB, 0, false>(b, f, tile, trow, part, silent, cnb_l, r1_l, r2_l, fs_l, fs_ps);
+        wf_feature_outputs<1, NB + 16, NB + 4, 0, true>(b, f, tile, trow, part, silent, cnb_l, r1_l, r2_l, fs_l, fs_ps);
     }
     NNN_STAMPW(b, 12, f == 3);
     if (part < 2) {
         float v = part == 0 ? 0.01f * ((float)pitch - 300.0f) : spectral_variability(dc, row, rm);
         v = silent ? 0.0f : v;
         if (b.taps) NNN_TIF(b, feat, NFEAT, f, tile, trow)[(size_t)(40 + part) * TILE] = v;
-        store_split(FS, rm * WF_FS_W, row * WF_FS_W + 40 + part, v);
+        store_split(FS, fs_ps, row * fs_w + 40 + part, v);
     }
     NNN_STAMPW(b, 13, f == 3);
 }
@@ -258,20 +260,419 @@
 struct WfShapeAny { static constexpr bool fixed = false; };
 template <class SH> struct WfFixed { static constexpr bool value = true; };
 template <> struct WfFixed<WfShapeAny> { static constexpr bool value = false; };
-template <class SH>
-__global__ void __launch_bounds__(64 * WF_WAVES, NNN_WF_MINWAVES) k_rnn_wf(Buffers b, RnnPlan pl_rt, WfPlan wp_rt, const uint4 *__restrict__ Wq,
-                                                            const float *__restrict__ fpar, int tile0, int g)
-{
-    RnnPlan pl = pl_rt;
-    WfPlan wp = wp_rt;
-    if constexpr (WfFixed<SH>::value) {
-        constexpr RnnPlan p0 = SH::plan();
-        constexpr WfPlan w0 = wf_plan_of(p0);
-        pl = p0;
-        pl.dense.act = pl_rt.dense.act; pl.vad.act = pl_rt.vad.act; pl.noise.act = pl_rt.noise.act; pl.dn.act = pl_rt.dn.act;
-        pl.out.act = pl_rt.out.act; pl.act_vo = pl_rt.act_vo;
-        wp = w0;
-    }
+enum { WP_F, WP_D, WP_V, WP_N, WP_DN, WP_RSV, WP_RSN, WP_RSDN, WP_Z, WP_COUNT };
+constexpr int WFU_FW = 48;
+struct WfuCols { int at[WP_COUNT]; int w, row; };
+__host__ __device__ constexpr WfuCols wfu_cols(const RnnPlan &p)
+{
+    WfuCols c{};
+    int at = 0;
+    const int len[WP_COUNT] = {4 * WFU_FW, 2 * p.dense.n, 2 * p.vad.n, p.noise.n, p.dn.n, p.vad.n, p.noise.n, p.dn.n, 8};
+    for (int i = 0; i < WP_COUNT; i++) { c.at[i] = at; at += len[i]; }
+    c.w = (at / 8) % 2 ? at : at + 8;
+    c.row = 3 * c.w;
+    return c;
+}
+struct WfuSrc { int piece[4], len[4]; };
+struct WfuSeg { int piece, col; };
+__host__ __device__ constexpr WfuSeg wfu_seg(const WfuSrc &s, int c)
+{
+    for (int i = 0; i < 4; i++) {
+        if (c < s.len[i]) return WfuSeg{s.piece[i], c};
+        c -= s.len[i];
+    }
+    return WfuSeg{WP_Z, 0};
+}
+struct WfuSlots { int F, D, V; };
+template <class SH> struct WfuT {
+    static constexpr RnnPlan plan() { return SH::plan(); }
+    static constexpr WfuCols cols() { return wfu_cols(SH::plan()); }
+    static_assert(SH::plan().dense.n % 8 == 0 && SH::plan().vad.n % 8 == 0 && SH::plan().noise.n % 8 == 0 && SH::plan().dn.n % 8 == 0, "pieces are whole 8-column segments");
+    static_assert(SH::plan().cV == SH::plan().noise.n && SH::plan().cF == SH::plan().cV + SH::plan().vad.n && SH::plan().dense.out_col == SH::plan().cF + WFU_FW, "the packed weights' column order: noise, vad, features, dense");
+    struct DenseIn { static constexpr WfuSrc get() { return {{WP_F, WP_Z, WP_Z, WP_Z}, {WFU_FW, 0, 0, 0}}; } };
+    struct VadIn { static constexpr WfuSrc get() { return {{WP_D, WP_Z, WP_Z, WP_Z}, {SH::plan().dense.n, 0, 0, 0}}; } };
+    struct VadRec { static constexpr WfuSrc get() { return {{WP_V, WP_Z, WP_Z, WP_Z}, {SH::plan().vad.n, 0, 0, 0}}; } };
+    struct NoiseIn { static constexpr WfuSrc get() { return {{WP_V, WP_F, WP_D, WP_Z}, {SH::plan().vad.n, WFU_FW, SH::plan().dense.n, 0}}; } };
+    struct NoiseRec { static constexpr WfuSrc get() { return {{WP_N, WP_Z, WP_Z, WP_Z}, {SH::plan().noise.n, 0, 0, 0}}; } };
+    struct DnIn { static constexpr WfuSrc get() { return {{WP_N, WP_V, WP_F, WP_Z}, {SH::plan().noise.n, SH::plan().vad.n, WFU_FW, 0}}; } };
+    struct DnRec { static constexpr WfuSrc get() { return {{WP_DN, WP_Z, WP_Z, WP_Z}, {SH::plan().dn.n, 0, 0, 0}}; } };
+    struct RsV { static constexpr WfuSrc get() { return {{WP_RSV, WP_Z, WP_Z, WP_Z}, {SH::plan().vad.n, 0, 0, 0}}; } };
+    struct RsN { static constexpr WfuSrc get() { return {{WP_RSN, WP_Z, WP_Z, WP_Z}, {SH::plan().noise.n, 0, 0, 0}}; } };
+    struct RsDn { static constexpr WfuSrc get() { return {{WP_RSDN, WP_Z, WP_Z, WP_Z}, {SH::plan().dn.n, 0, 0, 0}}; } };
+};
+template <class F, int... I> __device__ __forceinline__ void wfu_static_for(F &&f, std::integer_sequence<int, I...>) { (f(std::integral_constant<int, I>{}), ...); }
+template <int PIECE> __device__ __forceinline__ int wfu_slot(const WfuSlots &sl)
+{
+    if constexpr (PIECE == WP_F) return sl.F;
+    else if constexpr (PIECE == WP_D) return sl.D;
+    else if constexpr (PIECE == WP_V) return sl.V;
+    else return 0;
+}
+template <class T, class SRC, int KS> __device__ __forceinline__ int wfu_col(const WfuSlots &sl, int q)
+{
+    constexpr WfuSrc S = SRC::get();
+    constexpr WfuCols C = T::cols();
+    constexpr WfuSeg s0 = wfu_seg(S, 32 * KS), s1 = wfu_seg(S, 32 * KS + 8), s2 = wfu_seg(S, 32 * KS + 16), s3 = wfu_seg(S, 32 * KS + 24);
+    constexpr int c0 = C.at[s0.piece] + s0.col, c1 = C.at[s1.piece] + s1.col, c2 = C.at[s2.piece] + s2.col, c3 = C.at[s3.piece] + s3.col;
+    if constexpr (s1.piece == s0.piece && s2.piece == s0.piece && s3.piece == s0.piece && c1 == c0 + 8 && c2 == c0 + 16 && c3 == c0 + 24) {
+        return c0 + wfu_slot<s0.piece>(sl) + 8 * q;
+    } else {
+        const int a0 = c0 + wfu_slot<s0.piece>(sl), a1 = c1 + wfu_slot<s1.piece>(sl), a2 = c2 + wfu_slot<s2.piece>(sl), a3 = c3 + wfu_slot<s3.piece>(sl);
+        return q == 0 ? a0 : (q == 1 ? a1 : (q == 2 ? a2 : a3));
+    }
+}
+template <class T, class SRC, int NG, int MB, int G0, int KST, int KSF, int KS0 = 0>
+__device__ __forceinline__ void wfu_gemm(f32x4 (&acc)[3][2], const unsigned short *Ul, const WfuSlots &sl, int lane, const Frags<NG, KSF> &fr)
+{
+    static_assert(KST <= KSF, "every k-step's fragments are in registers");
+    constexpr int W = T::cols().w, ROW = T::cols().row;
+    const int q = lane >> 4;
+    uint4 cur[3], nxt[3];
+    {
+        const unsigned short *ap = Ul + wfu_col<T, SRC, KS0>(sl, q);
+#pragma unroll
+        for (int pl = 0; pl < GPL; pl++) cur[pl] = *(const uint4 *)(ap + pl * W);
+    }
+    wfu_static_for([&](auto si) {
+        constexpr int step = decltype(si)::value, ks = step / MB, mb = step % MB;
+        if constexpr (step + 1 < KST * MB) {
+            constexpr int ks1 = (step + 1) / MB, mb1 = (step + 1) % MB;
+            const unsigned short *ap = Ul + mb1 * 16 * ROW + wfu_col<T, SRC, KS0 + ks1>(sl, q);
+#pragma unroll
+            for (int pl = 0; pl < GPL; pl++) nxt[pl] = *(const uint4 *)(ap + pl * W);
+        }
+        __builtin_amdgcn_sched_barrier(0);
+#pragma unroll
+        for (int pl = 0; pl < GPL; pl++)
+#pragma unroll
+            for (int gi = 0; gi < NG; gi++) acc[G0 + gi][mb] = mfma_16x16x32_bf16(cur[pl], fr.f[ks][gi], acc[G0 + gi][mb]);
+        __builtin_amdgcn_sched_barrier(0);
+#pragma unroll
+        for (int pl = 0; pl < GPL; pl++) cur[pl] = nxt[pl];
+    }, std::make_integer_sequence<int, KST * MB>{});
+}
+
+template <int MB> struct WfuGru {
+    f32x4 acc[3][2];
+    float zz[MB][4], sold[MB == 1 ? 4 : 1];
+    Frags<1, WF_KS_REC> h;
+};
+template <class T, class SIN, class SREC, int MB, int KIN, int KREC>
+__device__ __forceinline__ void wfu_gru_a(const LayerDesc &L, unsigned short *U, const WfuSlots &sl, int sp_col, int rs_col, unsigned on,
+                                          const uint4 *__restrict__ Wq, const WfWeights &w, const float *tab, int nbi, int lane, WfuGru<MB> &u)
+{
+    constexpr int W = T::cols().w, ROW = T::cols().row;
+    const float scale = 1.0f / 256.0f;
+    const int neuron = nbi * 16 + (lane & 15);
+    const bool nvalid = neuron < L.n;
+    const uint4 *Bin = Wq + L.in.wofs + (size_t)nbi * 3 * L.in.ksteps * 64;
+    const unsigned short *Ul = U + (lane & 15) * ROW;
+    if constexpr (MB == 1 || KIN <= 2) {
+        Frags<3, KIN> f_in;
+        load_frags<3, 0, KIN>(f_in, L.in, Bin, lane);
+#pragma unroll
+        for (int g = 0; g < 3; g++)
+#pragma unroll
+            for (int mb = 0; mb < MB; mb++) u.acc[g][mb] = f32x4{w.bias[g], w.bias[g], w.bias[g], w.bias[g]};
+        wfu_gemm<T, SREC, 2, MB, 0, KREC, WF_KS_REC>(u.acc, Ul, sl, lane, w.zr);
+        wfu_gemm<T, SIN, 3, MB, 0, KIN, KIN>(u.acc, Ul, sl, lane, f_in);
+    } else {
+        Frags<3, 1> f_ring[2];
+        auto fetch = [&](int ks) {
+#pragma unroll
+            for (int gi = 0; gi < 3; gi++) f_ring[ks & 1].f[0][gi] = Bin[(gi * L.in.ksteps + ks) * 64 + lane];
+        };
+        fetch(0);
+        fetch(1);
+#pragma unroll
+        for (int g = 0; g < 3; g++)
+#pragma unroll
+            for (int mb = 0; mb < MB; mb++) u.acc[g][mb] = f32x4{w.bias[g], w.bias[g], w.bias[g], w.bias[g]};
+        wfu_gemm<T, SREC, 2, MB, 0, KREC, WF_KS_REC>(u.acc, Ul, sl, lane, w.zr);
+        wfu_static_for([&](auto ki) {
+            constexpr int ks = decltype(ki)::value;
+            wfu_gemm<T, SIN, 3, MB, 0, 1, 1, ks>(u.acc, Ul, sl, lane, f_ring[ks & 1]);
+            if constexpr (ks + 2 < KIN) fetch(ks + 2);
+        }, std::make_integer_sequence<int, KIN>{});
+    }
+    if constexpr (MB > 1) load_frags<1, 2, WF_KS_REC>(u.h, L.rec, Wq + L.rec.wofs + (size_t)nbi * 3 * L.rec.ksteps * 64, lane);
+#pragma unroll
+    for (int mb = 0; mb < MB; mb++) {
+        if (MB > 1 && !((on >> mb) & 1u)) continue;
+#pragma unroll
+        for (int q = 0; q < 4; q++) {
+            const int row = 16 * mb + 4 * (lane >> 4) + q;
+            const float so = nvalid ? load_split(U, W, row * ROW + sp_col + neuron) : 0.0f;
+            if constexpr (MB == 1) u.sold[q] = so;
+            u.zz[mb][q] = sigmoid_approx(scale * u.acc[0][mb][q], tab);
+            const float rs = so * sigmoid_approx(scale * u.acc[1][mb][q], tab);
+            if (nvalid) store_split(U, W, row * ROW + rs_col + neuron, rs);
+        }
+    }
+}
+template <class T, class SRS, int MB, int KREC, class Sink>
+__device__ __forceinline__ void wfu_gru_b(const LayerDesc &L, const unsigned short *U, int sp_col, unsigned on, const WfWeights &w, const float *tab, const int *live,
+                                          int nbi, int lane, WfuGru<MB> &u, Sink &&sink)
+{
+    const float scale = 1.0f / 256.0f;
+    const int neuron = nbi * 16 + (lane & 15);
+    const WfuSlots none{0, 0, 0};
+    if constexpr (MB > 1) wfu_gemm<T, SRS, 1, MB, 2, KREC, WF_KS_REC>(u.acc, U + (lane & 15) * T::cols().row, none, lane, u.h);
+    else wfu_gemm<T, SRS, 1, MB, 2, KREC, WF_KS_REC>(u.acc, U + (lane & 15) * T::cols().row, none, lane, w.h);
+    if (neuron < L.n) {
+#pragma unroll
+        for (int mb = 0; mb < MB; mb++) {
+            if (MB > 1 && !((on >> mb) & 1u)) continue;
+#pragma unroll
+            for (int q = 0; q < 4; q++) {
+                const int row = 16 * mb + 4 * (lane >> 4) + q;
+                const float hh = activate(L.act, scale * u.acc[2][mb][q], tab);
+                float so;
+                if constexpr (MB == 1) so = u.sold[q];
+                else so = load_split(U, T::cols().w, row * T::cols().row + sp_col + neuron);
+                const float z = u.zz[mb][q];
+                float snew = z * so + (1.0f - z) * hh;
+                snew = live[row] ? snew : so;
+                sink(row, neuron, snew);
+            }
+        }
+    }
+}
+template <class T, class SIN, bool QUAD, int MB, int KS, class Sink>
+__device__ __forceinline__ void wfu_dense(const LayerDesc &L, const unsigned short *U, const WfuSlots &sl, unsigned on, const WfDenseW<KS> &w, const float *tab,
+                                          int nbi, int lane, Sink &&sink)
+{
+    const int neuron = nbi * 16 + (lane & 15);
+    f32x4 acc[3][2];
+#pragma unroll
+    for (int mb = 0; mb < MB; mb++) acc[0][mb] = f32x4{w.bias, w.bias, w.bias, w.bias};
+    wfu_gemm<T, SIN, 1, MB, 0, KS, KS>(acc, U + (lane & 15) * T::cols().row, sl, lane, w.fr);
+    if (neuron < L.n) {
+#pragma unroll
+        for (int mb = 0; mb < MB; mb++) {
+            if (MB > 1 && !((on >> mb) & 1u)) continue;
+            if constexpr (QUAD) {
+                float v[4];
+#pragma unroll
+                for (int q = 0; q < 4; q++) v[q] = activate(L.act, acc[0][mb][q] * (1.0f / 256.0f), tab);
+                sink(16 * mb + 4 * (lane >> 4), neuron, v);
+            } else {
+#pragma unroll
+                for (int q = 0; q < 4; q++) sink(16 * mb + 4 * (lane >> 4) + q, neuron, activate(L.act, acc[0][mb][q] * (1.0f / 256.0f), tab));
+            }
+        }
+    }
+}
+struct WfuLds { int tab, live, U, crs, dc, cnb, total; };
+__host__ __device__ constexpr WfuLds wfu_lds(const WfuCols &c, int rows)
+{
+    WfuLds o{};
+    int at = 0;
+    o.tab = lds_take(at, 256 * 4);
+    o.live = lds_take(at, 8 * rows * 4);
+    o.U = lds_take(at, rows * c.row * 2);
+    o.crs = lds_take(at, CEPS_MEM * NB * rows * 4);
+    o.dc = lds_take(at, 28 * rows * 4);
+    o.cnb = lds_take(at, 28 * rows * 4);
+    o.total = at;
+    return o;
+}
+static_assert(wfu_cols(BkShapeBuiltin::plan()).w == 616, "operand matrix of the built-in shape class: 608 columns and a pad");
+static_assert(wfu_lds(wfu_cols(BkShapeBuiltin::plan()), 16).total == 75520 && wfu_lds(wfu_cols(BkShapeBuiltin::plan()), 32).total == 150016,
+              "k_rnn_wf's LDS for the built-in shape class at 16 and 32 rows");
+
+template <class SH, int ROWS>
+__device__ __forceinline__ void wfu_run(float *lds_raw, const Buffers &b, const RnnPlan &pl_rt, const uint4 *__restrict__ Wq, const float *__restrict__ fpar, int tile0, int g)
+{
+    using T = WfuT<SH>;
+    constexpr int MB = ROWS / 16, W = T::cols().w, ROW = T::cols().row;
+    constexpr WfuCols C = T::cols();
+    constexpr RnnPlan p0 = T::plan();
+    constexpr int ND = p0.dense.n, NV = p0.vad.n;
+    static_assert(MB == 1 || MB == 2, "one or two M-tiles");
+    static_assert(p0.dense.in.ksteps == 2 && p0.out.in.ksteps <= 3 && p0.dense.nb <= 2 && p0.out.nb <= 2, "the dense units' fragment sets and waves");
+    RnnPlan pl = p0;
+    pl.dense.act = pl_rt.dense.act; pl.vad.act = pl_rt.vad.act; pl.noise.act = pl_rt.noise.act; pl.dn.act = pl_rt.dn.act;
+    pl.out.act = pl_rt.out.act; pl.act_vo = pl_rt.act_vo;
+    const int wave0 = __builtin_amdgcn_readfirstlane((int)(threadIdx.x >> 6));
+    const int lane0 = threadIdx.x & 63;
+    int wave = wave0, lane = lane0;
+    int tile, r0;
+    if (!rnn_block_rows(b, tile0, ROWS, tile, r0)) return;
+    unsigned on = 0;
+#pragma unroll
+    for (int mb = 0; mb < MB; mb++)
+        if (tile * TILE + r0 + 16 * mb < b.S && live_any(b, tile, r0 + 16 * mb, 16)) on |= 1u << mb;
+    if (!on) return;
+    const bool rowl = lane0 < ROWS;
+    const int lrow = rowl ? lane0 : 0, trow = r0 + lrow;
+    const bool row_on = rowl && ((on >> (lrow >> 4)) & 1u);
+    NNN_STAMP(b, 50);
+    constexpr WfuLds o = wfu_lds(C, ROWS);
+    float *tab = lds_raw + o.tab / 4;
+    int *live = (int *)(lds_raw + o.live / 4);
+    unsigned short *U = (unsigned short *)(lds_raw + o.U / 4);
+    float *crs = lds_raw + o.crs / 4, *dc = lds_raw + o.dc / 4, *cnb = lds_raw + o.cnb / 4;
+    constexpr int CRS_T = CEPS_MEM * NB * 16, DC_T = 28 * 16;
+    constexpr int T_ = 64 * WF_WAVES;
+    float *sv = b.gru_v + ((size_t)tile * TILE * b.gru_v_w + (size_t)r0 * pl.vad.n),
+          *sn = b.gru_n + ((size_t)tile * TILE * b.gru_n_w + (size_t)r0 * pl.noise.n),
+          *sdn = b.gru_dn + ((size_t)tile * TILE * b.gru_dn_w + (size_t)r0 * pl.dn.n);
+    auto state_io = [&](int n, float *state, int col, bool load) {
+        for (int e = (int)threadIdx.x; e < ROWS * n; e += T_) {
+            const int row = e / n, c = e - row * n;
+            if (load) store_split(U, W, row * ROW + col + c, state[e]);
+            else if ((on >> (row >> 4)) & 1u) state[e] = load_split(U, W, row * ROW + col + c);
+        }
+    };
+    {
+        uint4 *z = (uint4 *)U;
+        constexpr int n16 = ROWS * ROW * 2 / 16;
+        for (int i = (int)threadIdx.x; i < n16; i += T_) z[i] = make_uint4(0u, 0u, 0u, 0u);
+        for (int i = (int)threadIdx.x; i < 201; i += T_) tab[i] = b.tansig[i];
+        const float *cm = NNN_TI(b.ceps_mem, CEPS_MEM * NB, tile, trow);
+        constexpr int PER = (CEPS_MEM * NB + WF_WAVES - 1) / WF_WAVES;
+        float stg[PER];
+#pragma unroll
+        for (int i = 0; i < PER; i++) {
+            const int r = wave + i * WF_WAVES;
+            stg[i] = (rowl && r < CEPS_MEM * NB) ? cm[(size_t)r * TILE] : 0.0f;
+        }
+#pragma unroll
+        for (int i = 0; i < PER; i++) {
+            const int r = wave + i * WF_WAVES;
+            if (rowl && r < CEPS_MEM * NB) crs[(lrow >> 4) * CRS_T + r * 16 + (lrow & 15)] = stg[i];
+        }
+    }
+    lds_barrier();
+    state_io(pl.vad.n, sv, C.at[WP_V] + NV, true);
+    state_io(pl.noise.n, sn, C.at[WP_N], true);
+    state_io(pl.dn.n, sdn, C.at[WP_DN], true);
+    if (rowl)
+        for (int p = wave; p < 28; p += WF_WAVES) dc[(lrow >> 4) * DC_T + p * 16 + (lrow & 15)] = pair_dist(crs + (lrow >> 4) * CRS_T, p, lrow & 15, 16);
+    int mem_id[MB];
+#pragma unroll
+    for (int mb = 0; mb < MB; mb++) mem_id[mb] = wave == WF_WAVES - 1 ? NNN_TI(b.mem_id, 1, tile, r0 + 16 * mb + (lane & 15))[0] : 0;
+    const int W_N = 6, W_V = 9, W_F = 11;
+    WfWeights wts;
+    if (wave < W_N) wf_load_weights(wts, pl.dn, Wq, fpar, wave < pl.dn.nb ? wave : 0, lane);
+    else if (wave < W_V) wf_load_weights(wts, pl.noise, Wq, fpar, wave - W_N < pl.noise.nb ? wave - W_N : 0, lane);
+    else if (wave < W_F) wf_load_weights(wts, pl.vad, Wq, fpar, wave - W_V < pl.vad.nb ? wave - W_V : 0, lane);
+    else wf_load_weights(wts, pl.vad, Wq, fpar, 0, lane);
+    lds_barrier();
+    NNN_STAMP(b, 51);
+    WfuGru<MB> ua;
+    if (wave == WF_WAVES - 1 && g > 0) {
+#pragma unroll
+        for (int mb = 0; mb < MB; mb++)
+            if ((on >> mb) & 1u) wf_features_load(wts, b, 0, tile, r0 + 16 * mb, lane, mb);
+    }
+    if (wave0 == WF_WAVES - 1) wf_setprio_high();
+    for (int t = -1; t < g + 3; t++) {
+        lane = launder_v(lane0);
+        wave = launder_s(wave0);
+        const int fv = t, fn = t - 1, fd = t - 2, fo = t - 3, ff = t + 1;
+        const bool on_v = fv >= 0 && fv < g, on_n = fn >= 0 && fn < g, on_d = fd >= 0 && fd < g, on_o = fo >= 0 && fo < g,
+                   on_f = ff >= 0 && ff < g;
+        const int srole = wave0 == 0 ? 0 : (wave0 == 6 ? 1 : (wave0 == 9 ? 2 : (wave0 == 11 ? 3 : -1)));
+        NNN_STAMPW(b, 30 + 5 * srole, t == 2 && srole >= 0);
+        if (wave < W_N) {
+            const WfuSlots sl{(fd & 3) * WFU_FW, 0, (fd & 1) * NV};
+            if (on_d && wave < pl.dn.nb)
+                wfu_gru_a<T, typename T::DnIn, typename T::DnRec, MB, p0.dn.in.ksteps, p0.dn.rec.ksteps>(pl.dn, U, sl, C.at[WP_DN], C.at[WP_RSDN], on, Wq, wts, tab, wave, lane, ua);
+        } else if (wave < W_V) {
+            const WfuSlots sl{(fn & 3) * WFU_FW, (fn & 1) * ND, (fn & 1) * NV};
+            if (on_n && wave - W_N < pl.noise.nb)
+                wfu_gru_a<T, typename T::NoiseIn, typename T::NoiseRec, MB, p0.noise.in.ksteps, p0.noise.rec.ksteps>(pl.noise, U, sl, C.at[WP_N], C.at[WP_RSN], on, Wq, wts, tab, wave - W_N, lane, ua);
+        } else if (wave < W_F) {
+            WfDenseW<3> dw;
+            const bool mine_o = on_o && wave - W_V < pl.out.nb;
+            const int vprev = ((fv - 1) & 1) * NV;
+            const WfuSlots sl{0, (fv & 1) * ND, vprev};
+            if (on_v && wave - W_V < pl.vad.nb)
+                wfu_gru_a<T, typename T::VadIn, typename T::VadRec, MB, p0.vad.in.ksteps, p0.vad.rec.ksteps>(pl.vad, U, sl, C.at[WP_V] + vprev, C.at[WP_RSV], on, Wq, wts, tab, wave - W_V, lane, ua);
+            if (mine_o) {
+                const int *lv = live + ROWS * (fo & 7);
+                const WfuSlots none{0, 0, 0};
+                wf_dense_load(dw, pl.out, Wq, fpar, wave - W_V, lane);
+                wfu_dense<T, typename T::DnRec, true, MB>(pl.out, U, none, on, dw, tab, wave - W_V, lane, [&](int qrow, int band, const float (&v)[4]) {
+                    if (b.link) {
+                        rnn_gain_out4(b, fo, tile, r0 + qrow, band, lv + qrow, v);
+                    } else {
+#pragma unroll
+                        for (int q = 0; q < 4; q++) rnn_gain_out(b, fo, tile, r0 + qrow + q, band, lv[qrow + q] != 0, v[q]);
+                    }
+                });
+            }
+        } else {
+            if (on_f) {
+#pragma unroll
+                for (int mb = 0; mb < MB; mb++)
+                    if ((on >> mb) & 1u)
+                        wf_features<MB == 1 ? NB : NB / 2>(b, wf_features_in(wts, mb), ff, tile, r0 + 16 * mb, lane, crs + mb * CRS_T, dc + mb * DC_T, cnb + mb * DC_T,
+                                    U + 16 * mb * ROW + C.at[WP_F] + (ff & 3) * WFU_FW, live + ROWS * (ff & 7) + 16 * mb, mem_id[mb], W, ROW);
+            }
+            if (ff + 1 >= 0 && ff + 1 < g) {
+#pragma unroll
+                for (int mb = 0; mb < MB; mb++)
+                    if ((on >> mb) & 1u) wf_features_load(wts, b, ff + 1, tile, r0 + 16 * mb, lane, mb);
+            }
+            if constexpr (MB > 1) ua = WfuGru<MB>{};
+        }
+        NNN_STAMPW(b, 31 + 5 * srole, t == 2 && srole >= 0);
+#if defined(NNN_STAMPS) && NNN_WFSTAMP_PHASE == 1
+        NNN_STAMPW(b, 14 + wave0, t == 2);
+#endif
+        lds_barrier();
+        NNN_STAMPW(b, 32 + 5 * srole, t == 2 && srole >= 0);
+        if (wave < W_N) {
+            WfDenseW<2> dw;
+            const bool mine_d = on_f && wave < pl.dense.nb;
+            if (on_d && wave < pl.dn.nb)
+                wfu_gru_b<T, typename T::RsDn, MB, p0.dn.rec.ksteps>(pl.dn, U, C.at[WP_DN], on, wts, tab, live + ROWS * (fd & 7), wave, lane, ua,
+                                                                      [&](int row, int n, float v) { store_split(U, W, row * ROW + C.at[WP_DN] + n, v); });
+            if (mine_d) {
+                const WfuSlots sl{(ff & 3) * WFU_FW, 0, 0};
+                const int dcol = C.at[WP_D] + (ff & 1) * ND;
+                wf_dense_load(dw, pl.dense, Wq, fpar, wave, lane);
+                wfu_dense<T, typename T::DenseIn, false, MB>(pl.dense, U, sl, on, dw, tab, wave, lane,
+                                                            [&](int row, int n, float v) { store_split(U, W, row * ROW + dcol + n, v); });
+            }
+        } else if (wave < W_V) {
+            if (on_n && wave - W_N < pl.noise.nb)
+                wfu_gru_b<T, typename T::RsN, MB, p0.noise.rec.ksteps>(pl.noise, U, C.at[WP_N], on, wts, tab, live + ROWS * (fn & 7), wave - W_N, lane, ua,
+                                                                       [&](int row, int n, float v) { store_split(U, W, row * ROW + C.at[WP_N] + n, v); });
+        } else if (wave < W_F) {
+            if (on_v && wave - W_V < pl.vad.nb) {
+                const int vcol = C.at[WP_V] + (fv & 1) * NV;
+                wfu_gru_b<T, typename T::RsV, MB, p0.vad.rec.ksteps>(pl.vad, U, C.at[WP_V] + ((fv - 1) & 1) * NV, on, wts, tab, live + ROWS * (fv & 7), wave - W_V, lane, ua,
+                                                                     [&](int row, int n, float v) { store_split(U, W, row * ROW + vcol + n, v); });
+            }
+        } else {
+            if (on_n && row_on)
+                NNN_TIF(b, vad, 1, fn, tile, trow)[0] = rnn_vad_out(pl, fpar, U, W, ROW, C.at[WP_V] + (fn & 1) * NV, lrow, live + ROWS * (fn & 7), tab);
+        }
+        NNN_STAMPW(b, 33 + 5 * srole, t == 2 && srole >= 0);
+#if defined(NNN_STAMPS) && NNN_WFSTAMP_PHASE == 2
+        NNN_STAMPW(b, 14 + wave0, t == 2);
+#endif
+        lds_barrier();
+        NNN_STAMPW(b, 34 + 5 * srole, t == 2 && srole >= 0);
+    }
+    state_io(pl.vad.n, sv, C.at[WP_V] + ((g - 1) & 1) * NV, false);
+    state_io(pl.noise.n, sn, C.at[WP_N], false);
+    state_io(pl.dn.n, sdn, C.at[WP_DN], false);
+    if (wave0 == WF_WAVES - 1 && lane0 < 16) {
+#pragma unroll
+        for (int mb = 0; mb < MB; mb++)
+            if ((on >> mb) & 1u) NNN_TI(b.mem_id, 1, tile, r0 + 16 * mb + lane0)[0] = mem_id[mb];
+    }
+    NNN_STAMP(b, 52);
+}
+
+__device__ __forceinline__ void wf_run_any(const Buffers &b, const RnnPlan &pl, const WfPlan &wp, const uint4 *__restrict__ Wq, const float *__restrict__ fpar,
+                                           int tile0, int g)
+{
     HIP_DYNAMIC_SHARED(float, lds_raw)
     constexpr int rm = WF_ROWS;
     const int wave0 = __builtin_amdgcn_readfirstlane((int)(threadIdx.x >> 6));
@@ -434,4 +835,17 @@
     NNN_STAMP(b, 52);
 }
 
-}
+template <class SH, int ROWS = WF_ROWS>
+__global__ void __launch_bounds__(64 * WF_WAVES, NNN_WF_MINWAVES) k_rnn_wf(Buffers b, RnnPlan pl_rt, WfPlan wp_rt, const uint4 *__restrict__ Wq,
+                                                            const float *__restrict__ fpar, int tile0, int g)
+{
+    if constexpr (WfFixed<SH>::value) {
+        HIP_DYNAMIC_SHARED(float, lds_u)
+        wfu_run<SH, ROWS>(lds_u, b, pl_rt, Wq, fpar, tile0, g);
+    } else {
+        static_assert(ROWS == WF_ROWS, "the run-time form has 16 rows");
+        wf_run_any(b, pl_rt, wp_rt, Wq, fpar, tile0, g);
+    }
+}
+
+}
```

After: 76.66 million frames/s, median of 6. No clear change (+0.7%).
